# agwi-lab/renderformer

Measured on AMD Instinct MI355X. Metric: rendered frames/sec at 512×512, renderformer-v1.1-swin-large, 1/2/4/8 MI355X, higher is better.
Workload: dtype fp16+bf16

## Files before the change

include/rf.h:

```cpp
#ifndef RF_H
#define RF_H

#include <stdint.h>

#ifdef __cplusplus
extern "C" {
#endif

#define RF_OK 0
#define RF_ERR_INVALID 1
#define RF_ERR_LAUNCH 2
#define RF_ERR_UNSUPPORTED 3
#define RF_ERR_DEVICE 4

#define RF_ABI_VERSION 16

#define RF_EPI_BF16 0
#define RF_EPI_F32 1
#define RF_EPI_ADD_F32 2
#define RF_EPI_SWIGLU 3
#define RF_EPI_F16 4
#define RF_EPI_SWIGLU_F16 5

#define RF_DT_BF16 0
#define RF_DT_F16 1

const char* rf_last_error(void);
int rf_abi_version(void);
#define RF_BUILD_STUDY 1
int rf_build_flags(void);

int rf_device_error(void);
int rf_clear_device_error(void);
int rf_f16_range_flag(void);
int rf_clear_f16_range_flag(void);
int rf_range_word_new(void** handle);
int rf_range_word_bind(void* handle);
int rf_range_word_read(void* handle);
int rf_range_word_clear(void* handle);
int rf_range_word_free(void* handle);
int rf_debug_raise_device_error(int code, void* stream);

int rf_ktimer_arm(void);
int rf_ktimer_read(float* ms, int max_n);

int rf_gemm_bf16(const void* a, int64_t lda, const void* w, int64_t ldw, void* c, int64_t ldc,
                 const float* bias, int m, int n, int k, int epilogue, void* workspace, int64_t ws_bytes,
                 void* stream);
int64_t rf_gemm_workspace_bytes(void);
int rf_gemm_f16(const void* a, int64_t lda, const void* w, int64_t ldw, void* c, int64_t ldc,
                const float* bias, int m, int n, int k, int epilogue, void* workspace, int64_t ws_bytes,
                void* stream);
#define RF_PRENORM_SLOTS 8
int rf_prenorm(const float* x, int64_t ldx, const float* norm_w, void* xg, int64_t ldxg, float* ss, int rows,
               int dim, int operand_dtype, void* stream);
int rf_gemm_add_prenorm(const void* a, int64_t lda, const void* w, int64_t ldw, float* x, int64_t ldx, int m, int n,
                        int k, const float* norm_w, void* xg, int64_t ldxg, float* ss, int operand_dtype,
                        void* workspace, int64_t ws_bytes, void* stream);
int rf_gemm_rownorm(const void* a, int64_t lda, const void* w, int64_t ldw, void* c, int64_t ldc, int m, int n,
                    int k, int epilogue, const float* ss, int norm_dim, float eps, float* seg_ss, int seg_w,
                    int n_seg, int operand_dtype, void* workspace, int64_t ws_bytes, void* stream);
int rf_gemm_qk_rope(const void* a, int64_t lda, const void* w, int64_t ldw, void* c, int64_t ldc, int m, int n,
                    int k, const float* ss, int norm_dim, float eps, float* seg_ss, int seg_w, int n_seg,
                    const float* norm_w, const float* pos, int64_t ld_pos, int pos_div, const float* freqs,
                    int n_freqs, float q_scale, int operand_dtype, void* workspace, int64_t ws_bytes, void* stream);
int rf_row_rms_scale(void* x, int64_t ldx, int rows, int dim, const float* ss, int64_t ld_ss, float eps, float scale,
                     void* stream);
int rf_attn_fwd_qn(const void* q, int64_t ldq, const void* k, int64_t ldk, const void* v, int64_t ldv, void* o,
                   int64_t ldo, int o_dtype, const float* q_ss, int64_t ld_ss, int q_dim, float eps, float q_scale,
                   const int32_t* problems, int n_problems, int n_heads, int head_dim, void* workspace,
                   const int64_t* bounds, int grid, void* stream);
int rf_gemm_bf16_if(const int* flag, const void* a, int64_t lda, const void* w, int64_t ldw, void* c, int64_t ldc,
                    const float* bias, int m, int n, int k, int epilogue, void* workspace, int64_t ws_bytes,
                    void* stream);

int rf_gemm_mx8(const void* a, int64_t lda, const void* sa, int64_t ld_sa, const void* w, int64_t ldw, const void* sw,
                int64_t ld_sw, void* c, int64_t ldc, const float* bias, int m, int n, int k, int epilogue,
                void* stream);
int rf_quant_mx8(const void* x, int64_t ldx, int rows, int cols, void* q, int64_t ldq, void* scales, int64_t ld_s,
                 void* stream);

int rf_rmsnorm(const float* x, int64_t ldx, const float* weight, float eps, void* out, int64_t ldo,
               int rows, int dim, void* stream);
int rf_rmsnorm_f16(const float* x, int64_t ldx, const float* weight, float eps, void* out, int64_t ldo,
                   int rows, int dim, void* stream);

int rf_qk_norm_rope(const void* src, int64_t ld_src, void* dst, int64_t ld_dst, const int32_t* src_rows,
                    int rows, int dim, int n_heads, int n_seg, const float* norm_w, float eps, float seg0_scale,
                    const float* pos, int64_t ld_pos, int pos_div, const float* freqs, int n_freqs, void* stream);

int rf_qk_norm_rope_groups(const void* src, int64_t ld_src, int64_t src_gstride, void* dst, int64_t ld_dst,
                           int64_t dst_gstride, const int32_t* src_rows, int rows, int dim, int n_heads, int n_seg,
                           int n_groups, const float* norm_w, int64_t w_gstride, float eps, float seg0_scale,
                           const float* pos, int64_t ld_pos, int pos_div, const float* freqs, int n_freqs,
                           void* stream);
int rf_qk_norm_rope_groups_ilv(const void* src, int64_t ld_src, int64_t src_gstride, void* dst, int64_t ld_dst,
                               int64_t dst_gstride, const int32_t* src_rows, int rows, int dim, int n_heads, int n_seg,
                               int n_groups, const float* norm_w, int64_t w_gstride, float eps, float seg0_scale,
                               const float* pos, int64_t ld_pos, int pos_div, const float* freqs, int n_freqs,
                               void* stream);

int rf_attn_fwd(const void* q, int64_t ldq, const void* k, int64_t ldk, const void* v, int64_t ldv,
                void* o, int64_t ldo, const int32_t* problems, int n_problems, int max_q_len, int n_heads,
                int head_dim, float scale, int n_split, void* workspace, int64_t ws_rows, void* stream);
int64_t rf_attn_workspace_bytes(int64_t rows, int n_heads, int n_split);
int rf_attn_grid(void);
int rf_attn_schedule(const int32_t* problems_host, int n_problems, int n_heads, int grid, int64_t* bounds);
int rf_attn_fwd_sched(const void* q, int64_t ldq, const void* k, int64_t ldk, const void* v, int64_t ldv,
                      void* o, int64_t ldo, const int32_t* problems, int n_problems, int n_heads, int head_dim,
                      float scale, void* workspace, const int64_t* bounds, int grid, void* stream);
int rf_attn_combine(const void* workspace, int64_t ws_rows, int n_split, int n_heads, const int32_t* rows,
// ... 24 lines not shown
int rf_texture_scan(float* texture, int64_t n_rows, int channels, int patch_elems, int log_channels,
                    const int32_t* dst_row, float* coef, int64_t ldc, int* flag, void* stream);
int rf_texture_scan2(float* texture, int64_t n_rows, int channels, int patch_elems, int log_channels,
                     const int32_t* dst_row, float* coef, int64_t ldc, int* flag, int* flag_clear, void* stream);
int rf_texture_linear(const float* coef, int64_t ldc, int rows, int channels, const float* wsum,
                      const float* bias, float* out, int64_t ldo, int n, const int* flag, void* stream);

int rf_vn_encode(const float* vn, int64_t n_rows, const int32_t* dst_row, int n_freqs, void* out,
                 int64_t ldo, void* stream);
int rf_vn_encode_dt(const float* vn, int64_t n_rows, const int32_t* dst_row, int n_freqs, void* out,
                    int64_t ldo, int out_dtype, void* stream);

int rf_ray_tokens(const float* c2w, const float* fov_deg, int n_views, int res, int patch, void* out,
                  float* ray_pos, void* stream);
int rf_ray_tokens_dt(const float* c2w, const float* fov_deg, int n_views, int res, int patch, void* out,
                     float* ray_pos, int out_dtype, void* stream);

int rf_patchify_rays(const float* rays_d, int n_views, int res, int patch, void* out, void* stream);
int rf_patchify_rays_dt(const float* rays_d, int n_views, int res, int patch, void* out, int out_dtype,
                        void* stream);

int rf_scene_pos(const float* tris, const int32_t* valid_idx, const int32_t* scene_off, const float* c2w,
                 int n_scenes, int n_views, int n_reg, float* pos_out, const int32_t* set_off, int max_tris,
                 float* partials, int64_t partial_floats, void* stream);
int64_t rf_scene_pos_partials(int sets, int max_tris);

int rf_embed(float* out, int64_t ldo, const int32_t* out_rows, int rows, int dim, const float* base,
             int base_rows, const float* in0, int64_t ld0, const float* w0, float eps0, const float* in1,
             int64_t ld1, const float* w1, float eps1, void* stream);

int rf_hdr_output(const float* logits, float* out, int n, int c, int h, int w, float elu_alpha, int log_decode,
                  int channels_last, void* stream);

#define RF_CONV_PLANE_SILU 1
#define RF_CONV_SILU_OUT 2
#define RF_CONV_FINAL 4
#define RF_CONV_LOG_DECODE 8
#define RF_CONV_NCHW_OUT 16
#define RF_CONV_BORDER_BIAS 32
int rf_conv2d_bf16x3(const void* in_hi, const void* in_lo, int n_img, int hi, int wi, int cin_pad, const void* w_hi,
                     const void* w_lo, int cout, int cout_pad, int kh, int kw, int stride, int pad, const float* bias,
                     const float* res1, const float* res2, float* out, void* p_hi, void* p_lo, int p_ld, int flags,
                     const float* w_fin, const float* b_fin, int n_fin, float elu_alpha, void* workspace,
                     int64_t ws_bytes, void* stream);

int rf_deconv2d_bf16x3(const void* in_hi, const void* in_lo, int n_img, int hi, int wi, int cin_pad, const void* w_hi,
                       const void* w_lo, int cout, int k, const float* bias, float* out, void* p_hi, void* p_lo,
                       int p_ld, void* workspace, int64_t ws_bytes, void* stream);

int rf_conv2d_f16(const void* in, int n_img, int hi, int wi, int cin_pad, const void* w, int cout, int cout_pad, int kh,
                  int kw, int stride, int pad, const float* bias, const float* res1, const float* res2, float* out,
                  void* p_out, int p_ld, int flags, const float* w_fin, const float* b_fin, int n_fin, float elu_alpha,
                  void* workspace, int64_t ws_bytes, void* stream);
typedef struct {
    const void* in;
    const void* w;
    const float* bias;
    float* out;
    void* p_out;
    int n_img, hi, wi, cin_pad, cout, cout_pad, kh, kw, stride, pad, deconv_k, p_ld, flags;
} rf_conv_desc;
int rf_conv2d_f16_group(int n_conv, const rf_conv_desc* convs, void* stream);

int rf_conv1x1_f16_group(int n_conv, const void* const* in, const int* cin_pad, const void* const* w, const int* cout,
                         const int* cout_pad, const float* const* bias, void* const* p_out, const int* p_ld, int n_img,
                         int hi, int wi, void* stream);
int rf_deconv2d_f16(const void* in, int n_img, int hi, int wi, int cin_pad, const void* w, int cout, int k,
                    const float* bias, float* out, void* p_out, int p_ld, void* workspace, int64_t ws_bytes,
                    void* stream);

int rf_split_planes(const float* x, int64_t rows, int c, int64_t ldx, void* p_hi, void* p_lo, int p_ld, int silu_act,
                    void* stream);

int rf_upsample_bilinear(const float* in, int n_img, int hi, int wi, int c, float* out, int ho, int wo, void* p_hi,
                         void* p_lo, int p_ld, void* stream);

int rf_upsample_bilinear_h(const void* in, int in_ld, int n_img, int hi, int wi, int c, int ho, int wo, void* p_out,
                           int p_ld, void* stream);


typedef struct {
    const float* attn_norm;
    const void* w_qkv;
    const float* qk_norm;
    const void* w_out;
    const float* ffn_norm;
    const void* w13;
    const void* w2;
} rf_encoder_layer;

typedef struct {
    int n_layers, rows, dim, n_heads, ffn_dim;
    int operand_dtype;
    float eps;
    const rf_encoder_layer* layers;
    const float* pos;
    int64_t ld_pos;
    const float* freqs;
    int n_freqs;
    const int32_t* problems;
    int n_problems;
    const int64_t* bounds;
    int grid;
    void* workspace;
    void* gemm_ws;
    int64_t gemm_ws_bytes;
// ... 16 lines not shown
    const float* self_norm;
    const void* w_self_in;
    const float* self_qk_norm;
    const void* w_self_out;
    const float* ffn_norm;
    const void* w13;
    const void* w2;
} rf_decoder_layer;

typedef struct {
    int layer, p_ld;
    void* p_hi;
    void* p_lo;
} rf_decoder_tap;

typedef struct {
    int n_layers, rows, dim, n_heads, ffn_dim;
    int operand_dtype;
    float eps;
    const rf_decoder_layer* layers;
    const float* ctx;
    int64_t ld_ctx;
    int ctx_rows, ctx_dim;
    const float* ctx_norm;
    const void* w_kv_all;
    int kv_rows;
    const int32_t* kv_src_rows;
    const float* kv_pos;
    int64_t ld_kv_pos;
    int k_batch;
    const float* k_norm_all;
    const float* freqs;
    int n_freqs;
    const float* ray_pos;
    int64_t ld_ray_pos;
    int ray_pos_div;
    const int32_t* cross_problems;
    int n_cross;
    const int64_t* cross_bounds;
    int cross_grid;
    int swin, n_images, grid_h, grid_w, window, shift;
    const int32_t* self_problems;
    int n_self;
    const rf_decoder_tap* taps;
    int n_taps;
    void* workspace;
    void* gemm_ws;
    int64_t gemm_ws_bytes;
    void* attn_ws;
    int timer_cross;
    int qk_fused;
    const void* kv_all;
    int64_t ld_kv_all;
} rf_decoder_desc;

int rf_decoder_forward(float* x, int64_t ldx, const rf_decoder_desc* desc, void* stream);
int64_t rf_decoder_workspace_bytes(const rf_decoder_desc* desc);

int rf_scene_kv(const float* ctx, int64_t ld_ctx, int ctx_rows, int ctx_dim, const float* ctx_norm,
                const void* w_kv_all, int width, int operand_dtype, float eps, void* scratch, void* kv_all,
                int64_t ld_kv_all, void* gemm_ws, int64_t gemm_ws_bytes, void* stream);

#ifdef __cplusplus
}
#endif
#endif
```

renderformer_amd/_lib.py:

```python
from __future__ import annotations

import ctypes
import os
import threading

import torch

_HERE = os.path.dirname(os.path.abspath(__file__))
LIB_PATH = os.environ.get("RF_LIB", os.path.join(_HERE, "lib", "librfhip.so"))


def source_digest(*names: str) -> str:
    import hashlib
    h = hashlib.sha256()
    for n in names:
        with open(os.path.join(_HERE, "csrc", n), "rb") as f:
            h.update(f.read())
    return h.hexdigest()[:16]


ATTN_SOURCES = ("attention.hip", "common.h")

_P = ctypes.c_void_p
_I = ctypes.c_int
_L = ctypes.c_int64
_F = ctypes.c_float

SIGNATURES = {
    "rf_gemm_bf16": [_P, _L, _P, _L, _P, _L, _P, _I, _I, _I, _I, _P, _L, _P],
    "rf_gemm_f16": [_P, _L, _P, _L, _P, _L, _P, _I, _I, _I, _I, _P, _L, _P],
    "rf_rmsnorm_f16": [_P, _L, _P, _F, _P, _L, _I, _I, _P],
    "rf_attn_fwd_sk": [_P, _L, _P, _L, _P, _L, _P, _L, _I, _P, _I, _I, _I, _F, _P, _P, _I, _P],
    "rf_attn_fwd_dt": [_P, _L, _P, _L, _P, _L, _P, _L, _I, _I, _P, _I, _I, _I, _F, _P, _P, _I, _P],
    "rf_swin_attn_fwd_dt": [_P, _L, _P, _L, _P, _L, _P, _L, _I, _I, _I, _I, _I, _I, _I, _I, _F, _P],
    "rf_swin_attn_fwd_qkn": [_P, _L, _P, _L, _P, _L, _P, _L, _I, _I, _I, _I, _I, _I, _I, _I, _F, _P, _P, _F, _F, _P],
    "rf_rmsnorm": [_P, _L, _P, _F, _P, _L, _I, _I, _P],
    "rf_prenorm": [_P, _L, _P, _P, _L, _P, _I, _I, _I, _P],
    "rf_gemm_add_prenorm": [_P, _L, _P, _L, _P, _L, _I, _I, _I, _P, _P, _L, _P, _I, _P, _L, _P],
    "rf_gemm_rownorm": [_P, _L, _P, _L, _P, _L, _I, _I, _I, _I, _P, _I, _F, _P, _I, _I, _I, _P, _L, _P],
    "rf_gemm_qk_rope": [_P, _L, _P, _L, _P, _L, _I, _I, _I, _P, _I, _F, _P, _I, _I, _P, _P, _L, _I, _P, _I, _F, _I,
                        _P, _L, _P],
    "rf_row_rms_scale": [_P, _L, _I, _I, _P, _L, _F, _F, _P],
    "rf_attn_fwd_qn": [_P, _L, _P, _L, _P, _L, _P, _L, _I, _P, _L, _I, _F, _F, _P, _I, _I, _I, _P, _P, _I, _P],
    "rf_qk_norm_rope": [_P, _L, _P, _L, _P, _I, _I, _I, _I, _P, _F, _F, _P, _L, _I, _P, _I, _P],
    "rf_qk_norm_rope_groups": [_P, _L, _L, _P, _L, _L, _P, _I, _I, _I, _I, _I, _P, _L, _F, _F, _P, _L, _I, _P, _I,
                               _P],
    "rf_qk_norm_rope_groups_ilv": [_P, _L, _L, _P, _L, _L, _P, _I, _I, _I, _I, _I, _P, _L, _F, _F, _P, _L, _I, _P, _I,
                               _P],
    "rf_attn_fwd": [_P, _L, _P, _L, _P, _L, _P, _L, _P, _I, _I, _I, _I, _F, _I, _P, _L, _P],
    "rf_attn_fwd_sched": [_P, _L, _P, _L, _P, _L, _P, _L, _P, _I, _I, _I, _F, _P, _P, _I, _P],
    "rf_attn_schedule": [_P, _I, _I, _I, _P],
    "rf_attn_combine": [_P, _L, _I, _I, _P, _I, _P, _L, _P],
    "rf_swin_attn_fwd": [_P, _L, _P, _L, _P, _L, _P, _L, _I, _I, _I, _I, _I, _I, _I, _F, _P],
    "rf_texture_pack": [_P, _L, _I, _I, _I, _P, _P, _L, _P],
    "rf_texture_pack_if": [_P, _P, _L, _I, _I, _I, _P, _P, _L, _P],
    "rf_texture_scan": [_P, _L, _I, _I, _I, _P, _P, _L, _P, _P],
    "rf_texture_scan2": [_P, _L, _I, _I, _I, _P, _P, _L, _P, _P, _P],
    "rf_texture_linear": [_P, _L, _I, _I, _P, _P, _P, _L, _I, _P, _P],
    "rf_gemm_bf16_if": [_P, _P, _L, _P, _L, _P, _L, _P, _I, _I, _I, _I, _P, _L, _P],
    "rf_vn_encode": [_P, _L, _P, _I, _P, _L, _P],
    "rf_vn_encode_dt": [_P, _L, _P, _I, _P, _L, _I, _P],
    "rf_ray_tokens_dt": [_P, _P, _I, _I, _I, _P, _P, _I, _P],
    "rf_patchify_rays_dt": [_P, _I, _I, _I, _P, _I, _P],
    "rf_ray_tokens": [_P, _P, _I, _I, _I, _P, _P, _P],
    "rf_patchify_rays": [_P, _I, _I, _I, _P, _P],
    "rf_scene_pos": [_P, _P, _P, _P, _I, _I, _I, _P, _P, _I, _P, _L, _P],
    "rf_embed": [_P, _L, _P, _I, _I, _P, _I, _P, _L, _P, _F, _P, _L, _P, _F, _P],
    "rf_hdr_output": [_P, _P, _I, _I, _I, _I, _F, _I, _I, _P],
    "rf_conv2d_bf16x3": [_P, _P, _I, _I, _I, _I, _P, _P, _I, _I, _I, _I, _I, _I, _P, _P, _P, _P, _P, _P, _I, _I,
                         _P, _P, _I, _F, _P, _L, _P],
    "rf_deconv2d_bf16x3": [_P, _P, _I, _I, _I, _I, _P, _P, _I, _I, _P, _P, _P, _P, _I, _P, _L, _P],
    "rf_conv2d_f16": [_P, _I, _I, _I, _I, _P, _I, _I, _I, _I, _I, _I, _P, _P, _P, _P, _P, _I, _I, _P, _P, _I, _F,
                      _P, _L, _P],
    "rf_deconv2d_f16": [_P, _I, _I, _I, _I, _P, _I, _I, _P, _P, _P, _I, _P, _L, _P],
    "rf_split_planes": [_P, _L, _I, _L, _P, _P, _I, _I, _P],
    "rf_upsample_bilinear": [_P, _I, _I, _I, _I, _P, _I, _I, _P, _P, _I, _P],
    "rf_upsample_bilinear_h": [_P, _I, _I, _I, _I, _I, _I, _I, _P, _I, _P],
    "rf_conv1x1_f16_group": [_I, _P, _P, _P, _P, _P, _P, _P, _P, _I, _I, _I, _P],
    "rf_conv2d_f16_group": [_I, _P, _P],
    "rf_gemm_mx8": [_P, _L, _P, _L, _P, _L, _P, _L, _P, _L, _P, _I, _I, _I, _I, _P],
    "rf_quant_mx8": [_P, _L, _I, _I, _P, _L, _P, _L, _P],
    "rf_device_error": [],
    "rf_clear_device_error": [],
    "rf_f16_range_flag": [],
    "rf_clear_f16_range_flag": [],
    "rf_range_word_new": [_P],
    "rf_range_word_bind": [_P],
    "rf_range_word_read": [_P],
    "rf_range_word_clear": [_P],
    "rf_range_word_free": [_P],
    "rf_debug_raise_device_error": [_I, _P],
    "rf_ktimer_arm": [],
    "rf_ktimer_read": [_P, _I],
    "rf_encoder_forward": [_P, _L, _P, _P],
    "rf_decoder_forward": [_P, _L, _P, _P],
    "rf_scene_kv": [_P, _L, _I, _I, _P, _P, _I, _I, _F, _P, _P, _L, _P, _L, _P],
}
RF_ERR_DEVICE = 4

_lock = threading.Lock()
_lib = None


class EncoderLayer(ctypes.Structure):
    _fields_ = [(n, ctypes.c_void_p) for n in ("attn_norm", "w_qkv", "qk_norm", "w_out", "ffn_norm", "w13", "w2")]


class EncoderDesc(ctypes.Structure):
    _fields_ = [("n_layers", _I), ("rows", _I), ("dim", _I), ("n_heads", _I), ("ffn_dim", _I),
                ("operand_dtype", _I), ("eps", _F), ("layers", _P), ("pos", _P), ("ld_pos", _L), ("freqs", _P),
                ("n_freqs", _I), ("problems", _P), ("n_problems", _I), ("bounds", _P), ("grid", _I),
                ("workspace", _P), ("gemm_ws", _P), ("gemm_ws_bytes", _L), ("attn_ws", _P), ("timer_attn", _I),
                ("qk_fused", _I)]


class DecoderLayer(ctypes.Structure):
    _fields_ = [(n, ctypes.c_void_p) for n in ("query_norm", "w_q", "q_norm", "kv_norm", "w_kv", "k_norm", "w_out",
                                               "self_norm", "w_self_in", "self_qk_norm", "w_self_out", "ffn_norm",
                                               "w13", "w2")]


class DecoderTap(ctypes.Structure):
    _fields_ = [("layer", _I), ("p_ld", _I), ("p_hi", _P), ("p_lo", _P)]


class DecoderDesc(ctypes.Structure):
    _fields_ = [("n_layers", _I), ("rows", _I), ("dim", _I), ("n_heads", _I), ("ffn_dim", _I),
                ("operand_dtype", _I), ("eps", _F), ("layers", _P), ("ctx", _P), ("ld_ctx", _L), ("ctx_rows", _I),
                ("ctx_dim", _I), ("ctx_norm", _P), ("w_kv_all", _P), ("kv_rows", _I), ("kv_src_rows", _P),
                ("kv_pos", _P), ("ld_kv_pos", _L), ("k_batch", _I), ("k_norm_all", _P), ("freqs", _P),
                ("n_freqs", _I), ("ray_pos", _P), ("ld_ray_pos", _L), ("ray_pos_div", _I), ("cross_problems", _P),
                ("n_cross", _I), ("cross_bounds", _P), ("cross_grid", _I), ("swin", _I), ("n_images", _I),
                ("grid_h", _I), ("grid_w", _I), ("window", _I), ("shift", _I), ("self_problems", _P), ("n_self", _I),
                ("taps", _P), ("n_taps", _I), ("workspace", _P), ("gemm_ws", _P), ("gemm_ws_bytes", _L),
                ("attn_ws", _P), ("timer_cross", _I), ("qk_fused", _I), ("kv_all", _P), ("ld_kv_all", _L)]


class HipLibraryError(RuntimeError):
    pass


class DeviceError(RuntimeError):
    """A kernel reported a device-side failure (a stream-K hand-off that timed out, or a range table that does not
    fit its launch): the outputs of that launch are invalid.  ``renderformer_amd.ops.clear_device_error()``
    recovers (it drains the device, clears the error word and drops the stream-K workspaces).  Also raised by a
    deferred fp16 range check (``RenderFormer(range_check="deferred")``) that finds a frame whose fp16 operands
    overflowed."""


def load(require_device: bool = True):
    global _lib
    with _lock:
        if _lib is None:
            if not os.path.exists(LIB_PATH):
                raise HipLibraryError(
                    f"librfhip.so not found at {LIB_PATH}; build it with `python -c 'import __graft_entry__ as g; g.build()'`")
            lib = ctypes.CDLL(LIB_PATH)
            for name, args in SIGNATURES.items():
                fn = getattr(lib, name, None)
                if fn is None:
                    continue
                fn.argtypes = args
                fn.restype = ctypes.c_int
            for name, res, args in (("rf_last_error", ctypes.c_char_p, []), ("rf_abi_version", ctypes.c_int, None),
                                    ("rf_build_flags", ctypes.c_int, []),
                                    ("rf_attn_workspace_bytes", ctypes.c_int64, [_L, _I, _I]),
                                    ("rf_gemm_workspace_bytes", ctypes.c_int64, []),
                                    ("rf_scene_pos_partials", ctypes.c_int64, [_I, _I]), ("rf_attn_grid", None, []),
                                    ("rf_encoder_workspace_bytes", ctypes.c_int64, [_I, _I, _I, _I]),
                                    ("rf_decoder_workspace_bytes", ctypes.c_int64, [_P])):
                fn = getattr(lib, name, None)
                if fn is None:
                    continue
                if res is not None:
                    fn.restype = res
                if args is not None:
                    fn.argtypes = args
            _lib = lib
    if require_device and not torch.cuda.is_available():
        raise HipLibraryError("renderformer_amd needs a HIP device (MI355X); none is visible")
    return _lib


def study_build() -> bool:
    lib = load(require_device=False)
    if getattr(lib, "rf_build_flags", None) is None:
        return False
    return bool(lib.rf_build_flags() & 1)
# ... 21 lines not shown
```

renderformer_amd/csrc/common.h:

```cpp
#pragma once
#include <hip/hip_runtime.h>
#include <hip/hip_ext.h>
#include <stdint.h>

#include "../../include/rf.h"

#define RF_DEV __device__ __forceinline__

typedef uint16_t bf16_t;
typedef __attribute__((ext_vector_type(8))) __bf16 bf16x8;
typedef __attribute__((ext_vector_type(4))) __bf16 bf16x4;
typedef __attribute__((ext_vector_type(2))) _Float16 f16x2;
typedef __attribute__((ext_vector_type(8))) _Float16 f16x8;
typedef __attribute__((ext_vector_type(4))) short s16x4;
typedef __attribute__((ext_vector_type(4))) float f32x4;
typedef __attribute__((ext_vector_type(2))) float f32x2;
typedef __attribute__((ext_vector_type(16))) float f32x16;
typedef __attribute__((ext_vector_type(4))) unsigned u32x4;
typedef __attribute__((ext_vector_type(2))) unsigned u32x2;

#define LDS_PTR(T, p) ((__attribute__((address_space(3))) T*)(p))
#define GLB_PTR(T, p) ((const __attribute__((address_space(1))) T*)(p))

RF_DEV float bf16_to_f32(bf16_t v) { return __uint_as_float(((uint32_t)v) << 16); }

RF_DEV bf16_t f32_to_bf16(float f) {
    __bf16 b = (__bf16)f;
    return *reinterpret_cast<bf16_t*>(&b);
}

RF_DEV uint32_t pack_bf16x2(float lo, float hi) {
    return (uint32_t)f32_to_bf16(lo) | ((uint32_t)f32_to_bf16(hi) << 16);
}

RF_DEV uint16_t f32_to_16(float v, bool f16) {
    if (f16) {
        _Float16 h = (_Float16)v;
        return __builtin_bit_cast(uint16_t, h);
    }
    return f32_to_bf16(v);
}

RF_DEV uint32_t pack_f16x2(float lo, float hi) {
    _Float16 a = (_Float16)lo, b = (_Float16)hi;
    return (uint32_t)*reinterpret_cast<uint16_t*>(&a) | ((uint32_t)*reinterpret_cast<uint16_t*>(&b) << 16);
}

RF_DEV float f16_bits_to_f32(uint16_t b) { return (float)__builtin_bit_cast(_Float16, b); }

RF_DEV float wave_sum(float v) {
#pragma unroll
    for (int o = 32; o > 0; o >>= 1) v += __shfl_xor(v, o, 64);
    return v;
}

RF_DEV float wave_max(float v) {
#pragma unroll
    for (int o = 32; o > 0; o >>= 1) v = fmaxf(v, __shfl_xor(v, o, 64));
    return v;
}

RF_DEV void wait_vmcnt0() { asm volatile("s_waitcnt vmcnt(0)" ::: "memory"); }

RF_DEV float silu(float x) {
    return x * __builtin_amdgcn_rcpf(1.0f + __builtin_amdgcn_exp2f(x * -1.4426950408889634f));
}
RF_DEV float elu_fast(float y, float alpha) {
    return y > 0.f ? y : alpha * (__builtin_amdgcn_exp2f(y * 1.4426950408889634f) - 1.0f);
}
RF_DEV float pow10m1_fast(float y) { return __builtin_amdgcn_exp2f(y * 3.3219280948873623f) - 1.0f; }

RF_DEV void report_device_error(int* err, int code) {
    if (err) __hip_atomic_store(err, code, __ATOMIC_RELAXED, __HIP_MEMORY_SCOPE_SYSTEM);
}
RF_DEV void report_f16_range(int* w, int code) {
    if (w) __hip_atomic_store(w, code, __ATOMIC_RELAXED, __HIP_MEMORY_SCOPE_SYSTEM);
}
RF_DEV bool f16_in_range(float amax) { return amax <= 65504.0f; }
RF_DEV float amax3(float m, float a, float b) {
    return __builtin_fmaxf(__builtin_fmaxf(m, __builtin_fabsf(a)), __builtin_fabsf(b));
}
#define RF_RANGE_GEMM 1
#define RF_RANGE_RMSNORM 2
#define RF_RANGE_ATTN 4
#define RF_RANGE_CONV 8
#define RF_DEVERR_SK_GEMM 1
#define RF_DEVERR_SK_ATTN 2
#define RF_DEVERR_SK_SCHED 3
#define RF_DEVERR_SCENE_POS 4

#define RF_HD __host__ __device__ __forceinline__
struct SkLayout {
    int nwg, nx, G;
    RF_HD SkLayout(int nwg_, int64_t units) : nwg(nwg_), nx(nwg_ < 8 ? nwg_ : 8), G(1) {
        G = units < (int64_t)nx ? (int)(units > 0 ? units : 1) : nx;
    }
    RF_HD int cnt(int x) const { return (nwg - x + nx - 1) / nx; }
    RF_HD int xlo(int g) const { return (g * nx + G - 1) / G; }
    RF_HD int group_of(int x) const { return x * G / nx; }
    RF_HD int base(int g) const {
        int s = 0;
// ... 59 lines not shown
```

renderformer_amd/csrc/conv.hip:

```cpp
#include <math.h>

#include "common.h"

namespace {


RF_DEV float store_split4(bf16_t* p_hi, bf16_t* p_lo, int64_t off, float4 v, bool act) {
    float x[4] = {v.x, v.y, v.z, v.w};
    if (!p_lo) {
        if (act) {
#pragma unroll
            for (int e = 0; e < 4; ++e) x[e] = silu(x[e]);
        }
        *reinterpret_cast<uint2*>(p_hi + off) = make_uint2(pack_f16x2(x[0], x[1]), pack_f16x2(x[2], x[3]));
        return amax3(amax3(0.f, x[0], x[1]), x[2], x[3]);
    }
    uint32_t h[2], l[2];
#pragma unroll
    for (int e = 0; e < 2; ++e) {
        float a0 = x[2 * e], a1 = x[2 * e + 1];
        if (act) {
            a0 = silu(a0);
            a1 = silu(a1);
        }
// ... 9 lines not shown
__global__ __launch_bounds__(256) void split_kernel(const float* __restrict__ x, int rows, int c, int64_t ldx,
                                                    bf16_t* __restrict__ p_hi, bf16_t* __restrict__ p_lo, int p_ld,
                                                    int act, int* range) {
    const int c4 = c / 4;
    const int i = blockIdx.x * blockDim.x + threadIdx.x;
    if (i >= rows * c4) return;
    const int r32 = i / c4;
    const int64_t r = r32;
    const int cc = (i - r32 * c4) * 4;
    const float am = store_split4(p_hi, p_lo, r * p_ld + cc, *reinterpret_cast<const float4*>(x + r * ldx + cc), act);
    if (range && !f16_in_range(am)) report_f16_range(range, RF_RANGE_CONV);
}

__global__ __launch_bounds__(256) void upsample_kernel(const float* __restrict__ in, float* __restrict__ out,
                                                       bf16_t* __restrict__ p_hi, bf16_t* __restrict__ p_lo, int p_ld,
                                                       int hi, int wi, int c, int ho, int wo, float sh, float sw) {
    const int c4n = c >> 2;
    const int i = blockIdx.x * blockDim.x + threadIdx.x;
    if (i >= wo * c4n) return;
    const int row = blockIdx.y;
    const int img = row / ho, oy = row - img * ho;
    const int ox = i / c4n;
    const int cc = (i - ox * c4n) * 4;
    const float fy = sh * (float)oy, fx = sw * (float)ox;
    const int y0 = (int)fy, x0 = (int)fx;
    const int y1 = y0 + (y0 < hi - 1 ? 1 : 0), x1 = x0 + (x0 < wi - 1 ? 1 : 0);
    const float ly1 = fy - (float)y0, lx1 = fx - (float)x0;
    const float ly0 = 1.0f - ly1, lx0 = 1.0f - lx1;
    const float* base = in + (int64_t)img * hi * wi * c + cc;
    const float4 a = *reinterpret_cast<const float4*>(base + (int64_t)(y0 * wi + x0) * c);
    const float4 b = *reinterpret_cast<const float4*>(base + (int64_t)(y0 * wi + x1) * c);
    const float4 d = *reinterpret_cast<const float4*>(base + (int64_t)(y1 * wi + x0) * c);
    const float4 e = *reinterpret_cast<const float4*>(base + (int64_t)(y1 * wi + x1) * c);
    float4 r;
    r.x = ly0 * (lx0 * a.x + lx1 * b.x) + ly1 * (lx0 * d.x + lx1 * e.x);
    r.y = ly0 * (lx0 * a.y + lx1 * b.y) + ly1 * (lx0 * d.y + lx1 * e.y);
    r.z = ly0 * (lx0 * a.z + lx1 * b.z) + ly1 * (lx0 * d.z + lx1 * e.z);
    r.w = ly0 * (lx0 * a.w + lx1 * b.w) + ly1 * (lx0 * d.w + lx1 * e.w);
    const int64_t pix = (int64_t)row * wo + ox;
    if (out) *reinterpret_cast<float4*>(out + pix * c + cc) = r;
    if (p_hi) store_split4(p_hi, p_lo, pix * p_ld + cc, r, false);
}

__global__ __launch_bounds__(256) void upsample8_kernel(const float* __restrict__ in, float* __restrict__ out,
                                                        bf16_t* __restrict__ p_hi, bf16_t* __restrict__ p_lo, int p_ld,
                                                        int hi, int wi, int c, int ho, int wo, float sh, float sw) {
    const int c8n = c >> 3;
    const int i = blockIdx.x * blockDim.x + threadIdx.x;
    if (i >= wo * c8n) return;
    const int row = blockIdx.y;
    const int img = row / ho, oy = row - img * ho;
    const int ox = i / c8n;
    const int cc = (i - ox * c8n) * 8;
    const float fy = sh * (float)oy, fx = sw * (float)ox;
    const int y0 = (int)fy, x0 = (int)fx;
    const int y1 = y0 + (y0 < hi - 1 ? 1 : 0), x1 = x0 + (x0 < wi - 1 ? 1 : 0);
    const float ly1 = fy - (float)y0, lx1 = fx - (float)x0;
    const float ly0 = 1.0f - ly1, lx0 = 1.0f - lx1;
    const float* base = in + (int64_t)img * hi * wi * c + cc;
    const float4* pa = reinterpret_cast<const float4*>(base + (int64_t)(y0 * wi + x0) * c);
    const float4* pb = reinterpret_cast<const float4*>(base + (int64_t)(y0 * wi + x1) * c);
    const float4* pd = reinterpret_cast<const float4*>(base + (int64_t)(y1 * wi + x0) * c);
    const float4* pe = reinterpret_cast<const float4*>(base + (int64_t)(y1 * wi + x1) * c);
    float4 a[2], b[2], d[2], e[2], r[2];
#pragma unroll
    for (int h = 0; h < 2; ++h) {
        a[h] = pa[h];
        b[h] = pb[h];
        d[h] = pd[h];
        e[h] = pe[h];
    }
#pragma unroll
    for (int h = 0; h < 2; ++h) {
        r[h].x = ly0 * (lx0 * a[h].x + lx1 * b[h].x) + ly1 * (lx0 * d[h].x + lx1 * e[h].x);
        r[h].y = ly0 * (lx0 * a[h].y + lx1 * b[h].y) + ly1 * (lx0 * d[h].y + lx1 * e[h].y);
        r[h].z = ly0 * (lx0 * a[h].z + lx1 * b[h].z) + ly1 * (lx0 * d[h].z + lx1 * e[h].z);
        r[h].w = ly0 * (lx0 * a[h].w + lx1 * b[h].w) + ly1 * (lx0 * d[h].w + lx1 * e[h].w);
    }
    const int64_t pix = (int64_t)row * wo + ox;
    if (out) {
        float4* o = reinterpret_cast<float4*>(out + pix * c + cc);
        o[0] = r[0];
        o[1] = r[1];
    }
    if (p_hi && !p_lo) {
        *reinterpret_cast<uint4*>(p_hi + pix * p_ld + cc) =
            make_uint4(pack_f16x2(r[0].x, r[0].y), pack_f16x2(r[0].z, r[0].w), pack_f16x2(r[1].x, r[1].y),
                       pack_f16x2(r[1].z, r[1].w));
    } else if (p_hi) {
        store_split4(p_hi, p_lo, pix * p_ld + cc, r[0], false);
        store_split4(p_hi, p_lo, pix * p_ld + cc + 4, r[1], false);
    }
}

__global__ __launch_bounds__(256) void upsample8h_kernel(const uint16_t* __restrict__ in, int in_ld,
                                                         uint16_t* __restrict__ p_out, int p_ld, int hi, int wi, int c,
                                                         int ho, int wo, float sh, float sw) {
    const int c8n = c >> 3;
    const int i = blockIdx.x * blockDim.x + threadIdx.x;
    if (i >= wo * c8n) return;
    const int row = blockIdx.y;
    const int img = row / ho, oy = row - img * ho;
    const int ox = i / c8n;
    const int cc = (i - ox * c8n) * 8;
    const float fy = sh * (float)oy, fx = sw * (float)ox;
    const int y0 = (int)fy, x0 = (int)fx;
    const int y1 = y0 + (y0 < hi - 1 ? 1 : 0), x1 = x0 + (x0 < wi - 1 ? 1 : 0);
    const float ly1 = fy - (float)y0, lx1 = fx - (float)x0;
    const float ly0 = 1.0f - ly1, lx0 = 1.0f - lx1;
    const uint16_t* base = in + (int64_t)img * hi * wi * in_ld + cc;
    const uint4 qa = *reinterpret_cast<const uint4*>(base + (int64_t)(y0 * wi + x0) * in_ld);
    const uint4 qb = *reinterpret_cast<const uint4*>(base + (int64_t)(y0 * wi + x1) * in_ld);
    const uint4 qd = *reinterpret_cast<const uint4*>(base + (int64_t)(y1 * wi + x0) * in_ld);
    const uint4 qe = *reinterpret_cast<const uint4*>(base + (int64_t)(y1 * wi + x1) * in_ld);
    const uint32_t wa[4] = {qa.x, qa.y, qa.z, qa.w}, wb[4] = {qb.x, qb.y, qb.z, qb.w};
    const uint32_t wd[4] = {qd.x, qd.y, qd.z, qd.w}, we[4] = {qe.x, qe.y, qe.z, qe.w};
    uint32_t o[4];
#pragma unroll
    for (int k = 0; k < 4; ++k) {
        float r[2];
#pragma unroll
        for (int h = 0; h < 2; ++h) {
            const float a = f16_bits_to_f32((uint16_t)(wa[k] >> (16 * h))), b = f16_bits_to_f32((uint16_t)(wb[k] >> (16 * h)));
            const float d = f16_bits_to_f32((uint16_t)(wd[k] >> (16 * h))), e = f16_bits_to_f32((uint16_t)(we[k] >> (16 * h)));
            r[h] = ly0 * (lx0 * a + lx1 * b) + ly1 * (lx0 * d + lx1 * e);
        }
        o[k] = pack_f16x2(r[0], r[1]);
    }
    *reinterpret_cast<uint4*>(p_out + ((int64_t)row * wo + ox) * p_ld + cc) = make_uint4(o[0], o[1], o[2], o[3]);
}

// ... 54 lines not shown
```

renderformer_amd/csrc/gemm.hip:

```cpp
#include <algorithm>
#include <type_traits>
#include <cmath>
#include <math.h>
#include <stdio.h>
#include <stdlib.h>
#include <string.h>

#include "common.h"
#include "env.h"

namespace {

constexpr int BK = 32;
constexpr int P_F16 = 2;

enum Epi { E_BF16 = RF_EPI_BF16, E_F32 = RF_EPI_F32, E_ADD = RF_EPI_ADD_F32, E_SWIGLU = RF_EPI_SWIGLU, E_CONV = 16,
           E_ROPE = 17 };

template <int BM_, int BN_, int WGM_, int WGN_, int STAGES_, int KH_ = 1>
struct Tile {
    static constexpr int BM = BM_, BN = BN_, WGM = WGM_, WGN = WGN_, STAGES = STAGES_, KH = KH_;
    static constexpr int NWAVE = WGM * WGN, THREADS = NWAVE * 64;
    static constexpr int MW = BM / WGM, NWD = BN / WGN, TI = MW / 16, TJ = NWD / 16;
    static constexpr int APIECES = BM / 16;
    static constexpr bool ASHARE = APIECES < NWAVE;
    static constexpr int PA = ASHARE ? 1 : BM / 16 / NWAVE, PB = BN / 16 / NWAVE;
    static constexpr int A_BYTES = BM * BK * 2, B_BYTES = BN * BK * 2;
    static_assert(PA >= 1 && PB >= 1 && (ASHARE || PA * NWAVE * 16 == BM || BM == 288) && PB * NWAVE * 16 == BN,
                  "tile/wave mismatch");
    static_assert(TI >= 1 && TJ >= 2 && TJ % 2 == 0, "wave tile too small");
};

struct EngineArgs {
    const bf16_t* a;
    const bf16_t* a_lo;
    int64_t lda;
    const bf16_t* w;
    const bf16_t* w_lo;
    int64_t ldw;
    int m, n, k;
    int hi, wi, cin_pad, ho, wo, kw, stride, pad;
    uint64_t cin_m, kw_m;
    const bf16_t* zero;
    void* c;
    int64_t ldc;
    const float* bias;
    const float* res1;
    const float* res2;
    bf16_t* p_hi;
    bf16_t* p_lo;
    int p_ld;
    int cout, deconv, flags, n_fin;
    int plane_f16;
    const float* w_fin;
    const float* b_fin;
    float elu_alpha;
    float* sk_part;
    int* sk_flag;
    int sk_epoch;
    int group_m;
    const int* gate;
    int halo_lg;
    int* err;
    int spin;
    uint64_t* stamps;
    const uint8_t* sa;
    const uint8_t* sw;
    int ld_sa, ld_sw;
    int persist;
    int l2pf;
    int out_f16;
    int* range;
    bf16_t* xg;
    int64_t ldxg;
    const float* norm_g;
    float* ss_out;
    int xg_f16;
    const float* rs_part;
    float rs_n, rs_eps;
    float* seg_ss;
    int seg_w, seg_n;
    const float* rope_pos;
    int64_t rope_ld;
    int rope_div;
    const float* rope_freqs;
    int rope_nf;
    const float* rope_g;
    float rope_qscale;
};

constexpr int PN_SLOTS = RF_PRENORM_SLOTS;


RF_DEV uint32_t pack16(const EngineArgs& p, float lo, float hi) {
    return p.out_f16 ? pack_f16x2(lo, hi) : pack_bf16x2(lo, hi);
}

RF_DEV float unpack16(const EngineArgs& p, uint32_t h) {
    return p.out_f16 ? f16_bits_to_f32((uint16_t)h) : __uint_as_float(h << 16);
}

// ... 283 lines not shown
template <class C>
constexpr int ROPE_POS_BYTES = (C::BM * 9 + 63) / 64 * 256;
template <class C, int EPI>
constexpr bool RED_IN_ROWS = C::BM == 288 && (EPI == E_BF16 || EPI == E_ROPE) && C::WGN < PN_SLOTS;
template <class C, int EPI>
constexpr int PN_RED = RED_IN_ROWS<C, EPI> ? 0 : C::BM * C::WGN * 4;
template <class C, int EPI>
constexpr int PN_AREA = EPI == E_ADD      ? C::BN * 4 + C::BM * C::WGN * 4
                        : EPI == E_BF16   ? C::BM * PN_SLOTS * 4 + PN_RED<C, EPI>
                        : EPI == E_ROPE   ? C::BM * PN_SLOTS * 4 + PN_RED<C, EPI> + C::BN * 4 + ROPE_POS_BYTES<C> + 64 * 4
                        : EPI == E_SWIGLU ? C::BM * PN_SLOTS * 4
                                          : 0;

template <class C, int EPI>
RF_DEV void pn_issue(const EngineArgs& p, char* area, int m0, int n0) {
    const int lane = threadIdx.x & 63;
    const int wave = __builtin_amdgcn_readfirstlane(threadIdx.x >> 6);
    if constexpr (EPI == E_ADD) {
        if (p.xg && wave == 0 && n0 + 4 * lane < p.n && 4 * lane < C::BN)
            __builtin_amdgcn_global_load_lds(GLB_PTR(void, p.norm_g + n0 + 4 * lane), LDS_PTR(void, area), 16, 0, 0);
    } else if constexpr (EPI == E_BF16 || EPI == E_SWIGLU || EPI == E_ROPE) {
        if (p.rs_part) {
            static_assert(C::BM % 32 == 0, "1-KiB pieces of 32 rows");
            for (int c = wave; c < C::BM / 32; c += C::NWAVE) {
                const int row = min(m0 + 32 * c + (lane >> 1), p.m - 1);
                __builtin_amdgcn_global_load_lds(GLB_PTR(void, p.rs_part + (int64_t)row * PN_SLOTS + 4 * (lane & 1)),
                                                 LDS_PTR(void, area + c * 1024), 16, 0, 0);
            }
        }
        if constexpr (EPI == E_ROPE) {
            if (n0 / p.seg_w < p.seg_n) {
                char* const gl = area + C::BM * PN_SLOTS * 4 + PN_RED<C, EPI>;
                char* const pl = gl + C::BN * 4;
                char* const fl = pl + ROPE_POS_BYTES<C>;
                if (wave == 0 && p.rope_g && 4 * lane < C::BN)
                    __builtin_amdgcn_global_load_lds(GLB_PTR(void, p.rope_g + n0 + 4 * lane), LDS_PTR(void, gl), 16, 0, 0);
                if (p.rope_pos) {
                    if (wave == C::NWAVE - 1)
                        __builtin_amdgcn_global_load_lds(GLB_PTR(void, p.rope_freqs + min(lane, p.rope_nf - 1)),
                                                         LDS_PTR(void, fl), 4, 0, 0);
                    for (int c = wave; c * 64 < C::BM * 9; c += C::NWAVE) {
                        const int e = c * 64 + lane;
                        const int r = e / 9, col = e - r * 9;
                        const int row = min(m0 + min(r, C::BM - 1), p.m - 1) / p.rope_div;
                        __builtin_amdgcn_global_load_lds(GLB_PTR(void, p.rope_pos + (int64_t)row * p.rope_ld + col),
                                                         LDS_PTR(void, pl + c * 256), 4, 0, 0);
                    }
                }
            }
        }
    }
}

template <class C, int EPI, int TW2D = 0, bool FINAL = true>
RF_DEV void engine_epilogue(const EngineArgs& p, int m0, int n0, const f32x4 (&acc)[C::TI][C::TJ],
                            char* area = nullptr) {
    constexpr int TI = C::TI, TJ = C::TJ;
    const int lane = threadIdx.x & 63;
    const int wave = threadIdx.x >> 6;
    const int wm = wave / C::WGN, wn = wave % C::WGN;
    static_assert(TW2D == 0 || (EPI == E_CONV && TW2D % 16 == 0 && C::MW % TW2D == 0), "2-D conv tile");
    const int rl = lane & 15, cq = 4 * (lane >> 4);
    const int rbase = m0 + wm * C::MW, cbase = n0 + wn * C::NWD;
    auto frow = [&](int i) -> int {
        if constexpr (TW2D == 0) return rbase + i * 16 + rl;
        else return m0 + (wm * (C::MW / TW2D) + (i * 16) / TW2D) * p.wo + (i * 16) % TW2D + rl;
    };
    float amax = 0.f;
    const bool rsc = (EPI == E_SWIGLU || EPI == E_BF16 || EPI == E_ROPE) && p.rs_part && area;
    if constexpr (EPI == E_SWIGLU || EPI == E_BF16 || EPI == E_ROPE) {
        if (rsc) {
            lds_sync();
            for (int t = threadIdx.x; t < C::BM; t += C::THREADS) {
                char* q = area + t * (PN_SLOTS * 4);
                const f32x4 a = lds_ld_f4(q), b = lds_ld_f4(q + 16);
                const float sum = ((a[0] + a[1]) + (a[2] + a[3])) + ((b[0] + b[1]) + (b[2] + b[3]));
                lds_st_f32(q, 1.0f / sqrtf(sum / p.rs_n + p.rs_eps));
            }
            lds_sync();
        }
    }
    auto row_scale = [&](int i) -> float {
        return rsc ? lds_ld_f32(area + (wm * C::MW + i * 16 + rl) * (PN_SLOTS * 4)) : 1.f;
    };
    if constexpr (EPI == E_SWIGLU) {
        bf16_t* c = reinterpret_cast<bf16_t*>(p.c);
#pragma unroll
        for (int i = 0; i < TI; ++i) {
            const float rsi = row_scale(i);
#pragma unroll
            for (int pair = 0; pair < TJ / 2; ++pair) {
                const int gcol = cbase + pair * 32;
                const int ocol = (gcol >> 5) * 16 + cq;
                const int row = rbase + i * 16 + rl;
                if (row < p.m) {
                    float o[4];
#pragma unroll
                    for (int e = 0; e < 4; ++e) {
                        float g = acc[i][2 * pair][e] * rsi, u = acc[i][2 * pair + 1][e] * rsi;
                        if (p.bias) {
                            g += p.bias[gcol + cq + e];
                            u += p.bias[gcol + 16 + cq + e];
                        }
                        o[e] = silu(g) * u;
                    }
                    amax = amax3(amax3(amax, o[0], o[1]), o[2], o[3]);
                    *reinterpret_cast<uint2*>(c + (int64_t)row * p.ldc + ocol) =
                        make_uint2(pack16(p, o[0], o[1]), pack16(p, o[2], o[3]));
                }
            }
        }
        if (p.range && !f16_in_range(amax)) report_f16_range(p.range, RF_RANGE_GEMM);
        return;
    } else if constexpr (EPI == E_CONV) {
        if (FINAL && (p.flags & RF_CONV_FINAL)) {
            float bsum[TJ][4];
#pragma unroll
            for (int j = 0; j < TJ; ++j)
#pragma unroll
                for (int e = 0; e < 4; ++e) {
                    const int col = cbase + j * 16 + cq + e;
                    bsum[j][e] = (p.bias && col < p.cout) ? p.bias[col] : 0.f;
                }
            for (int f = 0; f < p.n_fin; ++f) {
                const float bfin = p.b_fin[f];
                float wf[TJ][4];
#pragma unroll
                for (int j = 0; j < TJ; ++j)
#pragma unroll
                    for (int e = 0; e < 4; ++e) {
                        const int col = cbase + j * 16 + cq + e;
                        wf[j][e] = col < p.cout ? p.w_fin[f * p.cout + col] : 0.f;
                    }
#pragma unroll
                for (int i = 0; i < TI; ++i) {
                    float s = 0.f;
#pragma unroll
                    for (int j = 0; j < TJ; ++j)
#pragma unroll
                        for (int e = 0; e < 4; ++e) s += silu(acc[i][j][e] + bsum[j][e]) * wf[j][e];
                    s += __shfl_xor(s, 16, 64);
                    s += __shfl_xor(s, 32, 64);
                    const int m = frow(i);
                    if (lane < 16 && wn == 0 && m < p.m) {
                        float y = elu_fast(s + bfin, p.elu_alpha);
                        if (p.flags & RF_CONV_LOG_DECODE) y = pow10m1_fast(y);
                        const int hwp = p.ho * p.wo;
                        const int64_t o = (p.flags & RF_CONV_NCHW_OUT) ? ((int64_t)(m / hwp) * p.n_fin + f) * hwp + (m % hwp)
                                                                      : (int64_t)m * p.n_fin + f;
                        reinterpret_cast<float*>(p.c)[o] = y;
                    }
                }
            }
            return;
        }
        const int kk = p.deconv;
        const int nreal = kk ? p.cout * kk * kk : p.cout;
        const bool border = (p.flags & RF_CONV_BORDER_BIAS) && !kk;
        float* __restrict__ outp = reinterpret_cast<float*>(p.c);
        const float* __restrict__ res1 = p.res1;
        const float* __restrict__ res2 = p.res2;
        const float* __restrict__ bias = p.bias;
        struct PixOp {
            float4 r1[TJ], r2[TJ], b[TJ];
            int64_t pix[TJ];
            int co[TJ];
        };
        float4 bconst[TJ];
#pragma unroll
        for (int j = 0; j < TJ; ++j) {
            const int col = cbase + j * 16 + cq;
            bconst[j] = float4{0.f, 0.f, 0.f, 0.f};
            if (bias && !border && !kk && col < nreal) bconst[j] = *reinterpret_cast<const float4*>(bias + col);
        }
        auto fetch = [&](int i, PixOp& o) {
            const int m = frow(i);
            int img = 0, y = 0, x = 0;
            if (kk || border) {
                x = m % p.wo;
                const int t = m / p.wo;
                y = t % p.ho;
                img = t / p.ho;
            }
            const float* brow = bias;
            if (border && brow)
                brow += (3 * (y == 0 ? 0 : y == p.ho - 1 ? 2 : 1) + (x == 0 ? 0 : x == p.wo - 1 ? 2 : 1)) * p.cout;
#pragma unroll
            for (int j = 0; j < TJ; ++j) {
                const int col = cbase + j * 16 + cq;
                int64_t pix = m;
                int co = col;
                if (kk) {
                    const int tap = col / p.cout, dy = tap / kk, dx = tap % kk;
                    co = col - tap * p.cout;
                    pix = ((int64_t)img * p.ho * kk + y * kk + dy) * (p.wo * kk) + x * kk + dx;
                }
                o.pix[j] = pix;
                o.co[j] = co;
                o.r1[j] = float4{0.f, 0.f, 0.f, 0.f};
                o.r2[j] = float4{0.f, 0.f, 0.f, 0.f};
                o.b[j] = bconst[j];
                if (m < p.m && col < nreal) {
                    if (res1) o.r1[j] = *reinterpret_cast<const float4*>(res1 + pix * p.cout + co);
                    if (res2) o.r2[j] = *reinterpret_cast<const float4*>(res2 + pix * p.cout + co);
                    if (brow && (border || kk)) o.b[j] = *reinterpret_cast<const float4*>(brow + co);
                }
            }
        };
        constexpr bool PF = TJ <= 2;
        PixOp ops[PF ? 2 : 1];
        if constexpr (PF) fetch(0, ops[0]);
#pragma unroll
        for (int i = 0; i < TI; ++i) {
            if constexpr (PF) {
                if (i + 1 < TI) fetch(i + 1, ops[(i + 1) & 1]);
            } else {
                fetch(i, ops[0]);
            }
            const PixOp& o = ops[PF ? (i & 1) : 0];
            if (frow(i) >= p.m) continue;
#pragma unroll
            for (int j = 0; j < TJ; ++j) {
                const int col = cbase + j * 16 + cq;
                if (col >= nreal) continue;
                const int64_t pix = o.pix[j];
                const int co = o.co[j];
                const float bb[4] = {o.b[j].x, o.b[j].y, o.b[j].z, o.b[j].w};
                const float rr1[4] = {o.r1[j].x, o.r1[j].y, o.r1[j].z, o.r1[j].w};
                const float rr2[4] = {o.r2[j].x, o.r2[j].y, o.r2[j].z, o.r2[j].w};
                float v[4] = {acc[i][j][0], acc[i][j][1], acc[i][j][2], acc[i][j][3]};
#pragma unroll
                for (int e = 0; e < 4; ++e) {
                    v[e] = ((v[e] + bb[e]) + rr1[e]) + rr2[e];
                    if (p.flags & RF_CONV_SILU_OUT) v[e] = silu(v[e]);
                }
                if (outp)
                    *reinterpret_cast<float4*>(outp + pix * p.cout + co) = make_float4(v[0], v[1], v[2], v[3]);
                if (p.p_hi && p.plane_f16) {
                    float a[4] = {v[0], v[1], v[2], v[3]};
                    if (p.flags & RF_CONV_PLANE_SILU) {
#pragma unroll
                        for (int e = 0; e < 4; ++e) a[e] = silu(a[e]);
                    }
                    amax = amax3(amax3(amax, a[0], a[1]), a[2], a[3]);
                    *reinterpret_cast<uint2*>(p.p_hi + pix * p.p_ld + co) = make_uint2(pack_f16x2(a[0], a[1]),
                                                                                       pack_f16x2(a[2], a[3]));
                } else if (p.p_hi) {
                    uint32_t h[2], l[2];
#pragma unroll
                    for (int e = 0; e < 2; ++e) {
                        float a0 = v[2 * e], a1 = v[2 * e + 1];
                        if (p.flags & RF_CONV_PLANE_SILU) {
                            a0 = silu(a0);
                            a1 = silu(a1);
                        }
                        const bf16_t h0 = f32_to_bf16(a0), h1 = f32_to_bf16(a1);
                        h[e] = (uint32_t)h0 | ((uint32_t)h1 << 16);
                        l[e] = pack_bf16x2(a0 - bf16_to_f32(h0), a1 - bf16_to_f32(h1));
                    }
                    *reinterpret_cast<uint2*>(p.p_hi + pix * p.p_ld + co) = make_uint2(h[0], h[1]);
                    *reinterpret_cast<uint2*>(p.p_lo + pix * p.p_ld + co) = make_uint2(l[0], l[1]);
                }
            }
        }
        if (p.range && !f16_in_range(amax)) report_f16_range(p.range, RF_RANGE_CONV);
        return;
    } else {
        const bool pre = EPI == E_ADD && p.xg && area;
        const bool qkseg = EPI == E_ROPE && n0 / p.seg_w < p.seg_n;
        const bool segq = (EPI == E_BF16 || (EPI == E_ROPE && qkseg)) && p.seg_ss && area && n0 / p.seg_w < p.seg_n;
        char* const red = area + (EPI == E_ADD ? C::BN * 4 : C::BM * PN_SLOTS * 4);
        auto red_at = [&](int w, int t) -> char* {
            if constexpr (RED_IN_ROWS<C, EPI>) return area + t * (PN_SLOTS * 4) + (1 + w) * 4;
            else return red + (w * C::BM + t) * 4;
        };
        if (pre) lds_sync();
        float ssr[TI];
#pragma unroll
        for (int i = 0; i < TI; ++i) ssr[i] = 0.f;
        const char* const gl = area + C::BM * PN_SLOTS * 4 + PN_RED<C, EPI>;
        const float* const pl = reinterpret_cast<const float*>(gl + C::BN * 4);
        float frq[EPI == E_ROPE ? TJ : 1][2];
        int pcol[EPI == E_ROPE ? TJ : 1][2];
        float sscale = 1.f;
        if constexpr (EPI == E_ROPE) {
            if (qkseg) {
                if (!rsc) lds_sync();
                sscale = n0 / p.seg_w == 0 ? p.rope_qscale : 1.f;
                const int lim = 9 * p.rope_nf;
                const float* fl = pl + ROPE_POS_BYTES<C> / 4;
#pragma unroll
                for (int j = 0; j < TJ; ++j) {
                    const int col = cbase + j * 16 + cq;
#pragma unroll
                    for (int t = 0; t < 2; ++t) {
                        const int m = ((col & 127) >> 1) + t;
                        const bool on = p.rope_pos && m < lim;
                        const int pc = on ? m / p.rope_nf : 0;
                        frq[j][t] = on ? fl[m - pc * p.rope_nf] : 0.f;
                        pcol[j][t] = pc;
                    }
                }
            }
        }
#pragma unroll
        for (int i = 0; i < TI; ++i) {
            const int row = rbase + i * 16 + rl;
            if (row >= p.m) continue;
            const float rsi = row_scale(i);
#pragma unroll
            for (int j = 0; j < TJ; ++j) {
                const int col = cbase + j * 16 + cq;
                if (col >= p.n) continue;
                float v[4] = {acc[i][j][0] * rsi, acc[i][j][1] * rsi, acc[i][j][2] * rsi, acc[i][j][3] * rsi};
                if (p.bias) {
                    const float4 b = *reinterpret_cast<const float4*>(p.bias + col);
                    v[0] += b.x;
                    v[1] += b.y;
                    v[2] += b.z;
                    v[3] += b.w;
                }
                const int64_t o = (int64_t)row * p.ldc + col;
                if constexpr (EPI == E_ROPE) {
                    if (qkseg) {
                        if (segq) ssr[i] += v[0] * v[0] + v[1] * v[1] + v[2] * v[2] + v[3] * v[3];
                        const f32x4 g = p.rope_g ? *reinterpret_cast<const f32x4*>(gl + (col - n0) * 4)
                                                 : f32x4{1.f, 1.f, 1.f, 1.f};
                        const float z0 = v[0] * g[0], z1 = v[1] * g[1], z2 = v[2] * g[2], z3 = v[3] * g[3];
                        const float* prow = pl + (wm * C::MW + i * 16 + rl) * 9;
                        float s0, c0, s1, c1;
                        __sincosf(prow[pcol[j][0]] * frq[j][0], &s0, &c0);
                        __sincosf(prow[pcol[j][1]] * frq[j][1], &s1, &c1);
                        v[0] = (z0 * c0 - z1 * s0) * sscale;
                        v[1] = (z1 * c0 + z0 * s0) * sscale;
                        v[2] = (z2 * c1 - z3 * s1) * sscale;
                        v[3] = (z3 * c1 + z2 * s1) * sscale;
                    }
                    *reinterpret_cast<uint2*>(reinterpret_cast<bf16_t*>(p.c) + o) =
                        make_uint2(pack_bf16x2(v[0], v[1]), pack_bf16x2(v[2], v[3]));
                } else if constexpr (EPI == E_BF16) {
                    amax = amax3(amax3(amax, v[0], v[1]), v[2], v[3]);
                    const uint32_t lo = pack16(p, v[0], v[1]), hi = pack16(p, v[2], v[3]);
                    *reinterpret_cast<uint2*>(reinterpret_cast<bf16_t*>(p.c) + o) = make_uint2(lo, hi);
                    if (segq) {
                        const float r0 = unpack16(p, lo & 0xffffu), r1 = unpack16(p, lo >> 16);
                        const float r2 = unpack16(p, hi & 0xffffu), r3 = unpack16(p, hi >> 16);
                        ssr[i] += r0 * r0 + r1 * r1 + r2 * r2 + r3 * r3;
                    }
                } else {
                    *reinterpret_cast<float4*>(reinterpret_cast<float*>(p.c) + o) = make_float4(v[0], v[1], v[2], v[3]);
                    if (pre) {
                        const f32x4 g = lds_ld_f4(area + (col - n0) * 4);
                        const float y0 = v[0] * g[0], y1 = v[1] * g[1], y2 = v[2] * g[2], y3 = v[3] * g[3];
                        amax = amax3(amax3(amax, y0, y1), y2, y3);
                        const uint32_t lo = p.xg_f16 ? pack_f16x2(y0, y1) : pack_bf16x2(y0, y1);
                        const uint32_t hi = p.xg_f16 ? pack_f16x2(y2, y3) : pack_bf16x2(y2, y3);
                        *reinterpret_cast<uint2*>(p.xg + (int64_t)row * p.ldxg + col) = make_uint2(lo, hi);
                        ssr[i] += v[0] * v[0] + v[1] * v[1] + v[2] * v[2] + v[3] * v[3];
                    }
                }
            }
        }
        if constexpr (EPI == E_BF16)
            if (p.range && !f16_in_range(amax)) report_f16_range(p.range, RF_RANGE_GEMM);
        if constexpr (EPI == E_ADD || EPI == E_BF16 || EPI == E_ROPE) {
            if (pre && p.xg_f16 && p.range && !f16_in_range(amax)) report_f16_range(p.range, RF_RANGE_RMSNORM);
            if (pre || segq) {
#pragma unroll
                for (int i = 0; i < TI; ++i) {
                    ssr[i] += __shfl_xor(ssr[i], 16, 64);
                    ssr[i] += __shfl_xor(ssr[i], 32, 64);
                }
                if (lane < 16) {
#pragma unroll
                    for (int i = 0; i < TI; ++i) lds_st_f32(red_at(wn, wm * C::MW + i * 16 + rl), ssr[i]);
                }
                lds_sync();
                int slot, nslots, ld;
                float* base;
                if (pre) {
                    slot = n0 / C::BN;
                    nslots = (p.n + C::BN - 1) / C::BN;
                    ld = PN_SLOTS;
                    base = p.ss_out;
                } else {
                    slot = (n0 % p.seg_w) / C::BN;
                    nslots = p.seg_w / C::BN;
                    ld = p.seg_n * PN_SLOTS;
                    base = p.seg_ss + (n0 / p.seg_w) * PN_SLOTS;
                }
                for (int t = threadIdx.x; t < C::BM; t += C::THREADS) {
                    const int row = m0 + t;
                    if (row < p.m) {
                        float s = 0.f;
#pragma unroll
                        for (int w = 0; w < C::WGN; ++w) s += lds_ld_f32(red_at(w, t));
                        float* dst = base + (int64_t)row * ld;
                        dst[slot] = s;
                        if (slot == 0)
                            for (int z = nslots; z < PN_SLOTS; ++z) dst[z] = 0.f;
                    }
                }
            }
        }
    }
}



namespace ph {
constexpr int BN = 256, BK2 = 64;
constexpr int REGION = 16384;
template <int BM>
struct Cfg {
    static constexpr int NREG = BM >= 256 ? 4 : 3;
    static constexpr int NA = BM >= 256 ? 2 : 1;
    static constexpr int NX = BM == 288 ? 1 : 0;
// ... 923 lines not shown
        __syncthreads();
        if constexpr (STG == 1) quad_mainloop_reg<WM, WN, NTERM, EPI == E_ADD>(p, smem, m0, n0, 2 * kf, 2 * kl, acc);
        else quad_mainloop<WM, WN, NTERM, EPI == E_ADD>(p, smem, m0, n0, 2 * kf, 2 * kl, acc);
        if (kf != 0) {
            const __amdgpu_buffer_rsrc_t rs =
                __builtin_amdgcn_make_buffer_rsrc(p.sk_part + (int64_t)L * TS, 0, TS * 4, qd::RSRC_CFG);
#pragma unroll
            for (int i = 0; i < TI; ++i)
#pragma unroll
                for (int j = 0; j < TJ; ++j) {
                    const int off = (((wave * TI + i) * TJ + j) * 64 + lane) * 16;
                    __builtin_amdgcn_raw_buffer_store_b128(__builtin_bit_cast(u32x4, acc[i][j]), rs, off, 0, 16);
                }
            asm volatile("s_waitcnt vmcnt(0)" ::: "memory");
            __syncthreads();
            if (threadIdx.x == 0) __hip_atomic_store(p.sk_flag + L, p.sk_epoch, __ATOMIC_RELAXED, __HIP_MEMORY_SCOPE_AGENT);
        } else {
            if (kl < iters2) {
                const int64_t tile_end = (int64_t)(tile + 1) * iters2;
                for (int c = L + 1; c < gend; ++c) {
                    int64_t cb, ce;
                    lay.equal_range(c, grp, ntiles64, iters2, cb, ce);
                    if (cb >= tile_end) break;
                    if (ce == cb) continue;
                    if (threadIdx.x == 0) {
                        int spins = 0;
                        while (__hip_atomic_load(p.sk_flag + c, __ATOMIC_RELAXED, __HIP_MEMORY_SCOPE_AGENT) != p.sk_epoch &&
                               ++spins < p.spin)
                            __builtin_amdgcn_s_sleep(1);
                        if (spins >= p.spin) report_device_error(p.err, RF_DEVERR_SK_GEMM);
                        __builtin_amdgcn_fence(__ATOMIC_ACQUIRE, "agent");
                        asm volatile("s_waitcnt vmcnt(0)" ::: "memory");
                    }
                    __syncthreads();
                    const float4* src = reinterpret_cast<const float4*>(p.sk_part + (int64_t)c * TS) + wave * TI * TJ * 64 + lane;
#pragma unroll
                    for (int i = 0; i < TI; ++i)
#pragma unroll
                        for (int j = 0; j < TJ; ++j) {
                            const float4 v = src[(i * TJ + j) * 64];
                            acc[i][j][0] += v.x;
                            acc[i][j][1] += v.y;
                            acc[i][j][2] += v.z;
                            acc[i][j][3] += v.w;
                        }
                }
            }
            engine_epilogue<G, EPI>(p, m0, n0, acc);
        }
        it += kl - kf;
    }
}

template <class C, int EPI, int NTERM, bool GATHER, bool SK>
__global__ __launch_bounds__(C::THREADS, 2) void engine_kernel(EngineArgs p) {
    constexpr int BM = C::BM, BN = C::BN, TI = C::TI, TJ = C::TJ;
    constexpr int MAIN = C::STAGES * stage_bytes<C, NTERM>();
    __shared__ __attribute__((aligned(16))) char smem[MAIN + PN_AREA<C, EPI>];
    char* const area = smem + MAIN;
    if (gated_off(p)) return;

    const int tiles_m = (p.m + BM - 1) / BM;
    const int nwg = gridDim.x;
    const int hw = blockIdx.x;
    const int xcd = hw & 7, q = nwg >> 3, r = nwg & 7;
    const int wg = (xcd < r ? xcd * (q + 1) : r * (q + 1) + (xcd - r) * q) + (hw >> 3);
    f32x4 acc[TI][TJ];
    if constexpr (!SK) {
        int tm, tn;
        tile_coords(wg, tiles_m, p.n / BN, p.group_m, tm, tn);
        const int m0 = tm * BM, n0 = tn * BN;
        pn_issue<C, EPI>(p, area, m0, n0);
        engine_mainloop<C, NTERM, GATHER, EPI == E_ADD>(p, smem, m0, n0, 0, p.k / (BK * C::KH), acc);
        engine_epilogue<C, EPI>(p, m0, n0, acc, area);
    } else {
        const int iters = p.k / (BK * C::KH);
        const int64_t ntiles64 = (int64_t)tiles_m * (p.n / BN);
        const SkLayout lay(nwg, ntiles64);
        int grp = 0;
        const int L = lay.logical(hw, &grp);
        const int gend = lay.base(grp) + lay.size(grp);
        int64_t it, it_end;
        lay.equal_range(L, grp, ntiles64, iters, it, it_end);
        const int lane = threadIdx.x & 63, wave = threadIdx.x >> 6;
        while (it < it_end) {
            const int tile = (int)(it / iters), kf = (int)(it % iters);
            const int kl = (int)min((int64_t)iters, kf + (it_end - it));
            int tm, tn;
            tile_coords(tile, tiles_m, p.n / BN, p.group_m, tm, tn);
            const int m0 = tm * BM, n0 = tn * BN;
            wait_vm<0>();
            __syncthreads();
            if (kf == 0) pn_issue<C, EPI>(p, area, m0, n0);
            engine_mainloop<C, NTERM, GATHER, EPI == E_ADD>(p, smem, m0, n0, kf, kl, acc);
            if (kf != 0) {
                const __amdgpu_buffer_rsrc_t rs = __builtin_amdgcn_make_buffer_rsrc(
                    p.sk_part + (int64_t)L * (BM * BN), 0, BM * BN * 4, 0x00020000);
#pragma unroll
                for (int i = 0; i < TI; ++i)
#pragma unroll
                    for (int j = 0; j < TJ; ++j) {
                        const int off = (((wave * TI + i) * TJ + j) * 64 + lane) * 16;
                        __builtin_amdgcn_raw_buffer_store_b128(__builtin_bit_cast(u32x4, acc[i][j]), rs, off, 0, 16);
                    }
                asm volatile("s_waitcnt vmcnt(0)" ::: "memory");
                __syncthreads();
                if (threadIdx.x == 0) __hip_atomic_store(p.sk_flag + L, p.sk_epoch, __ATOMIC_RELAXED, __HIP_MEMORY_SCOPE_AGENT);
            } else {
                if (kl < iters) {
                    const int64_t tile_end = (int64_t)(tile + 1) * iters;
                    for (int c = L + 1; c < gend; ++c) {
                        int64_t cb, ce;
                        lay.equal_range(c, grp, ntiles64, iters, cb, ce);
                        if (cb >= tile_end) break;
                        if (ce == cb) continue;
                        if (threadIdx.x == 0) {
                            int spins = 0;
                            while (__hip_atomic_load(p.sk_flag + c, __ATOMIC_RELAXED, __HIP_MEMORY_SCOPE_AGENT) != p.sk_epoch &&
                                   ++spins < p.spin)
                                __builtin_amdgcn_s_sleep(1);
                            if (spins >= p.spin) report_device_error(p.err, RF_DEVERR_SK_GEMM);
                            __builtin_amdgcn_fence(__ATOMIC_ACQUIRE, "agent");
                            asm volatile("s_waitcnt vmcnt(0)" ::: "memory");
                        }
                        __syncthreads();
                        const float4* src =
                            reinterpret_cast<const float4*>(p.sk_part + (int64_t)c * (BM * BN)) + wave * TI * TJ * 64 + lane;
#pragma unroll
                        for (int i = 0; i < TI; ++i)
#pragma unroll
                            for (int j = 0; j < TJ; ++j) {
                                const float4 v = src[(i * TJ + j) * 64];
                                acc[i][j][0] += v.x;
                                acc[i][j][1] += v.y;
                                acc[i][j][2] += v.z;
                                acc[i][j][3] += v.w;
                            }
                    }
                }
                engine_epilogue<C, EPI>(p, m0, n0, acc, area);
            }
            it += kl - kf;
        }
    }
}

constexpr int GROUP_MAX = 4;
struct GroupArgs {
    EngineArgs p[GROUP_MAX];
    int first[GROUP_MAX + 1];
    int n;
};

template <class C, int EPI, int NTERM, bool GATHER>
__global__ __launch_bounds__(C::THREADS, 2) void engine_group_kernel(GroupArgs g) {
    constexpr int BM = C::BM, BN = C::BN, TI = C::TI, TJ = C::TJ;
    __shared__ __attribute__((aligned(16))) char smem[C::STAGES * stage_bytes<C, NTERM>()];
    const int nwg = gridDim.x, hw = blockIdx.x;
    const int xcd = hw & 7, qd = nwg >> 3, rd = nwg & 7;
    const int wg = (xcd < rd ? xcd * (qd + 1) : rd * (qd + 1) + (xcd - rd) * qd) + (hw >> 3);
    int q = 0;
#pragma unroll
    for (int i = 1; i < GROUP_MAX; ++i) q += (i < g.n && wg >= g.first[i]) ? 1 : 0;
    const EngineArgs& p = g.p[q];
    const int local = wg - g.first[q];
    const int tiles_m = (p.m + BM - 1) / BM;
    int tm, tn;
    tile_coords(local, tiles_m, p.n / BN, p.group_m, tm, tn);
    f32x4 acc[TI][TJ];
    engine_mainloop<C, NTERM, GATHER, EPI == E_ADD>(p, smem, tm * BM, tn * BN, 0, p.k / (BK * C::KH), acc);
    engine_epilogue<C, EPI>(p, tm * BM, tn * BN, acc);
}

template <class C>
struct Halo {
    static constexpr int ROWS = (3 * (C::BM + 2) + 15) / 16 * 16;
    static constexpr int BYTES = ROWS * 64;
    static constexpr int PIECES = ROWS / 16;
    static constexpr int PPW = (PIECES + C::NWAVE - 1) / C::NWAVE;
    static constexpr int BST = 3;
    static constexpr int LDS = 2 * BYTES + BST * C::B_BYTES;
};

template <class C>
RF_DEV void halo_mainloop(const EngineArgs& p, char* smem, int m0, int n0, f32x4 (&acc)[C::TI][C::TJ]) {
    using H = Halo<C>;
    constexpr int TI = C::TI, TJ = C::TJ, PB = C::PB, S = H::BST;
    const int lane = threadIdx.x & 63;
    const int wave = threadIdx.x >> 6;
    const int wm = wave / C::WGN, wn = wave % C::WGN;
    const int lg = p.halo_lg, tw = 1 << lg, hw2 = tw + 2;
    const int hr_n = ((C::BM >> lg) + 2) * hw2;
    const int per_img = p.ho * p.wo;
// ... 279 lines not shown
            const int kt = 9 * c + t;
            if constexpr (DBG == 8) __builtin_amdgcn_s_setprio(1);
            read_b(kt % S);
            read_a(t);
            if (DBG != 2 && t < PPW && !last) issue_halo(c + 1, t);
            if (DBG != 2 && kt + S - 1 < nk) issue_w(kt + S - 1);
            if (has_w) {
                if (t < 8 || !last) {
                    if (last) wait_vm_rt<4>(wait_count(t, S - 1, true));
                    else wait_vm_rt<8>(wait_count(t, S - 1, false));
                }
            } else if (t == 8 && !last) {
                wait_vm<0>();
            }
            if constexpr (DBG == 8) __builtin_amdgcn_s_setprio(0);
            sync_in();
            mma();
            sync_out();
        }
        const uint32_t step = (c & 1) ? (uint32_t)-HBYTES : (uint32_t)HBYTES;
#pragma unroll
        for (int h = 0; h < 2; ++h)
#pragma unroll
            for (int tx = 0; tx < 3; ++tx) hadr[h][tx] += step;
    }
    if (!late) __builtin_amdgcn_s_barrier();
}

template <int S, int BN, int DBG = 0>
__global__ __launch_bounds__(512, 1) void halo2_kernel(EngineArgs p) {
    __shared__ __attribute__((aligned(16))) char smem[H2Cfg<S, BN>::LDS];
    const int nwg = gridDim.x, hw = blockIdx.x;
    const int xcd = hw & 7, q = nwg >> 3, r = nwg & 7;
    const int wg = (xcd < r ? xcd * (q + 1) : r * (q + 1) + (xcd - r) * q) + (hw >> 3);
    const int tiles_n = p.n / BN, tx_n = p.wo / h2::TW, ty_n = p.ho / h2::TH;
    const int tn = wg % tiles_n, pt = wg / tiles_n;
    const int tx = pt % tx_n, rest = pt / tx_n;
    const int ty = rest % ty_n, img = rest / ty_n;
    const int y0 = ty * h2::TH, x0 = tx * h2::TW;
    f32x4 acc[H2Cfg<S, BN>::TI][4];
    halo2_mainloop<S, BN, DBG>(p, smem, img, y0, x0, tn * BN, acc);
    engine_epilogue<H2Tile<BN>, E_CONV, h2::TW, BN == 64>(p, (img * p.ho + y0) * p.wo + x0, tn * BN, acc);
}

namespace h3 {
constexpr int WGN = 4, WGM = 2, RW = h2::TH / WGM, TI = 2 * RW, TJ = 2;
constexpr int LDS = 2 * h2::HBYTES;
}
struct H3Tile {
    static constexpr int WGN = h3::WGN, WGM = h3::WGM, MW = 512 / h3::WGM, NWD = 128 / h3::WGN, TI = h3::TI,
                         TJ = h3::TJ;
};

template <int DBG = 0>
__global__ __launch_bounds__(512, 1) void halo3_kernel(EngineArgs p) {
    using namespace h2;
    __shared__ __attribute__((aligned(16))) char smem[h3::LDS];
    constexpr int TI = h3::TI;
    const int nwg = gridDim.x, hw = blockIdx.x;
    const int xcd = hw & 7, q = nwg >> 3, r = nwg & 7;
    const int wg = (xcd < r ? xcd * (q + 1) : r * (q + 1) + (xcd - r) * q) + (hw >> 3);
    const int tiles_n = p.n / 128, tx_n = p.wo / TW, ty_n = p.ho / TH;
    const int tn = wg % tiles_n, pt = wg / tiles_n;
    const int tx = pt % tx_n, rest = pt / tx_n;
    const int ty = rest % ty_n, img = rest / ty_n;
    const int y0 = ty * TH, x0 = tx * TW, n0 = tn * 128;

    const int lane = threadIdx.x & 63;
    const int wave = threadIdx.x >> 6;
    const int wm = wave / h3::WGN, wn = wave % h3::WGN;
    const int nch = p.cin_pad / 32, nk = 9 * nch;
    char* hbuf = smem;

    int hpix[PPW], hch[PPW];
#pragma unroll
    for (int t = 0; t < PPW; ++t) {
        const int hp = (wave + 8 * t) * 16 + (lane >> 2);
        hch[t] = (lane & 3) ^ h2::hkey(hp % HWID);
        int pix = -1;
        if (hp < HPIX) {
            const int hy = hp / HWID, hx = hp - hy * HWID;
            const int iy = y0 + hy - 1, ix = x0 + hx - 1;
            if (iy >= 0 && iy < p.hi && ix >= 0 && ix < p.wi) pix = (img * p.hi + iy) * p.wi + ix;
        }
        hpix[t] = pix;
    }
    const uint32_t hbase = __builtin_amdgcn_readfirstlane((uint32_t)(uintptr_t)LDS_PTR(char, hbuf) + wave * 1024);
    auto issue_halo = [&](int chunk, int buf, int t) {
        const bf16_t* src = hpix[t] >= 0 ? p.a + (int64_t)hpix[t] * p.cin_pad + hch[t] * 8 + chunk * 32 : p.zero;
        const uint32_t lds = hbase + buf * HBYTES + t * 8 * 1024;
        asm volatile("s_mov_b32 m0, %1\n\ts_nop 0\n\tglobal_load_lds_dwordx4 %0, off" ::"v"(src), "s"(lds)
                     : "memory", "m0");
    };

    const int frow = lane & 15, fch = lane >> 4;
    const __amdgpu_buffer_rsrc_t rw = __builtin_amdgcn_make_buffer_rsrc(
        (void*)(p.w + (int64_t)n0 * p.ldw), 0, (int)((int64_t)128 * p.ldw * 2), qd::RSRC_CFG);
    const int wv0 = ((wn * 32 + frow) * (int)p.ldw + fch * 8) * 2, wv1 = wv0 + 16 * (int)p.ldw * 2;
    u32x4 fb[3][2];
    auto load_b = [&](int kt, int slot) {
        const int chunk = kt / 9, tap = kt - 9 * chunk;
        const int so = (tap * p.cin_pad + chunk * 32) * 2;
        fb[slot][0] = __builtin_amdgcn_raw_buffer_load_b128(rw, wv0, so, 0);
        fb[slot][1] = __builtin_amdgcn_raw_buffer_load_b128(rw, wv1, so, 0);
    };

    f32x4 acc[TI][2];
// ... 19 lines not shown
    wait_vm<0>();
    __builtin_amdgcn_s_barrier();
    __builtin_amdgcn_sched_barrier(0);

    for (int c = 0; c < ((DBG & 32) ? 0 : nch); ++c) {
        const bool last = c + 1 == nch;
#pragma unroll
        for (int t = 0; t < 9; ++t) {
            const int kt = 9 * c + t;
            bf16x8 fa[TI];
#pragma unroll
            for (int i = 0; i < TI; ++i) {
                if constexpr (DBG & 16) {
                    fa[i] = __builtin_bit_cast(bf16x8, u32x4{(uint32_t)(lane + i), (uint32_t)t, 0u, (uint32_t)c});
                } else {
                    fa[i] = *LDS_PTR(const bf16x8, (uintptr_t)(hadr[i & 1][t % 3] + ((i >> 1) + t / 3) * HWID * 64));
                }
            }
            if (!(DBG & 4) && t < PPW) issue_halo(last ? c : c + 1, (c + 1) & 1, t);
            if (!(DBG & 2)) load_b(min(kt + 2, nk - 1), (t + 2) % 3);
            __builtin_amdgcn_s_setprio(1);
#pragma unroll
            for (int i = 0; i < TI; ++i)
#pragma unroll
                for (int j = 0; j < 2; ++j) {
                    if constexpr (DBG & 1) {
                        if (j == 0) asm volatile("" ::"v"(fa[i]));
                    } else {
                        acc[i][j] = __builtin_amdgcn_mfma_f32_16x16x32_f16(__builtin_bit_cast(f16x8, fb[t % 3][j]),
                                                                           __builtin_bit_cast(f16x8, fa[i]), acc[i][j], 0, 0, 0);
                    }
                }
            __builtin_amdgcn_s_setprio(0);
        }
        if (!(DBG & 8) && !last) {
            wait_vm<0>();
            __builtin_amdgcn_s_waitcnt(0xC07F);
            __builtin_amdgcn_sched_barrier(0);
            __builtin_amdgcn_s_barrier();
            __builtin_amdgcn_sched_barrier(0);
            const uint32_t step = (c & 1) ? (uint32_t)-HBYTES : (uint32_t)HBYTES;
#pragma unroll
            for (int h = 0; h < 2; ++h)
#pragma unroll
                for (int tx3 = 0; tx3 < 3; ++tx3) hadr[h][tx3] += step;
        }
    }
    wait_vm<0>();
    if constexpr ((DBG & 64) != 0) {
#pragma unroll
        for (int i = 0; i < TI; ++i) asm volatile("" ::"v"(acc[i][0]), "v"(acc[i][1]));
        return;
    }
    engine_epilogue<H3Tile, E_CONV, TW, false>(p, (img * p.ho + y0) * p.wo + x0, n0, acc);
}

namespace c32 {
constexpr int TH = 16, TW = 32, HWID = TW + 2, HPIX = (TH + 2) * HWID;
constexpr int HPIECES = 40, WPIECES = 18;
constexpr int HBYTES = HPIECES * 1024, WBYTES = WPIECES * 1024, BUF = HBYTES + WBYTES;
constexpr int NWAVE = 4, HPW = HPIECES / NWAVE;
constexpr int LDS = 2 * BUF;
constexpr int NFIN = 4;
}

__global__ __launch_bounds__(256, 1) void conv3x3_c32_kernel(EngineArgs p) {
    using namespace c32;
    __shared__ __attribute__((aligned(16))) char smem[LDS];
    const int lane = threadIdx.x & 63;
    const int wave = __builtin_amdgcn_readfirstlane(threadIdx.x >> 6);
    const int nwg = gridDim.x, hw = blockIdx.x;
    const int xcd = hw & 7, q = nwg >> 3, r = nwg & 7;
    const int wg = (xcd < r ? xcd * (q + 1) : r * (q + 1) + (xcd - r) * q) + (hw >> 3);
    const int tx_n = p.wo / TW, ty_n = p.ho / TH;
    const int tx = wg % tx_n, rest = wg / tx_n;
    const int ty = rest % ty_n, img = rest / ty_n;
    const int y0 = ty * TH, x0 = tx * TW;
    const int nch = p.cin_pad / 32;

    int hpix[HPW], hch[HPW];
#pragma unroll
    for (int t = 0; t < HPW; ++t) {
        const int hp = (wave + NWAVE * t) * 16 + (lane >> 2);
        hch[t] = (lane & 3) ^ h2::hkey(hp % HWID);
        int pix = -1;
        if (hp < HPIX) {
            const int hy = hp / HWID, hx = hp - hy * HWID;
            const int iy = y0 + hy - 1, ix = x0 + hx - 1;
            if (iy >= 0 && iy < p.hi && ix >= 0 && ix < p.wi) pix = (img * p.hi + iy) * p.wi + ix;
        }
        hpix[t] = pix;
    }
    const int wr = lane >> 2;
    auto issue = [&](int chunk, int buf) {
        char* b = smem + buf * BUF;
#pragma unroll
        for (int t = 0; t < HPW; ++t) {
            const bf16_t* src = hpix[t] >= 0 ? p.a + (int64_t)hpix[t] * p.cin_pad + hch[t] * 8 + chunk * 32 : p.zero;
            __builtin_amdgcn_global_load_lds(GLB_PTR(void, src), LDS_PTR(void, b + (wave + NWAVE * t) * 1024), 16, 0, 0);
        }
        for (int v = wave; v < WPIECES; v += NWAVE) {
            const int tap = v >> 1, row = 16 * (v & 1) + wr;
            const bf16_t* src = p.w + (int64_t)row * p.ldw + tap * p.cin_pad + chunk * 32 + (((lane & 3) ^ ((row >> 1) & 3)) * 8);
            __builtin_amdgcn_global_load_lds(GLB_PTR(void, src), LDS_PTR(void, b + HBYTES + v * 1024), 16, 0, 0);
        }
    };
    const int n_issue = HPW + (WPIECES - wave + NWAVE - 1) / NWAVE;
// ... 212 lines not shown
        rd(0, 0);
#pragma unroll
        for (int tap = 0; tap < 9; ++tap) {
            const int s = tap & 1;
            if (tap + 1 < 9) rd(tap + 1, s ^ 1);
            __builtin_amdgcn_sched_barrier(0);
#pragma unroll
            for (int i = 0; i < 8; ++i)
#pragma unroll
                for (int j = 0; j < 4; ++j)
                    acc[i][j] = __builtin_amdgcn_mfma_f32_16x16x32_f16(__builtin_bit_cast(f16x8, fb[s][j]),
                                                                       __builtin_bit_cast(f16x8, fa[s][i]), acc[i][j], 0, 0, 0);
            __builtin_amdgcn_sched_barrier(0);
        }
        __builtin_amdgcn_sched_barrier(0);
        __builtin_amdgcn_s_barrier();
    }
    engine_epilogue<HkTile, E_CONV, TW, false>(p, (img * p.ho + y0) * p.wo + x0, n0, acc);
}
#endif

using T128 = Tile<128, 128, 2, 2, 3>;
using T128w8 = Tile<128, 128, 2, 4, 3>;
using T256 = Tile<256, 256, 2, 4, 4>;
using T256x128 = Tile<256, 128, 4, 2, 3>;
using T256x64 = Tile<256, 64, 4, 1, 4>;
using T96x256 = Tile<96, 256, 2, 4, 3>;
using T64x256 = Tile<64, 256, 2, 4, 3>;
using T64x256w4 = Tile<64, 256, 1, 4, 3>;
using T96x256s5 = Tile<96, 256, 2, 4, 5>;
using T96x256s6 = Tile<96, 256, 2, 4, 6>;
using T64x256s6 = Tile<64, 256, 2, 4, 6>;
using T128s6 = Tile<128, 128, 2, 2, 6>;
using T128w8s6 = Tile<128, 128, 2, 4, 6>;
using T128k2s3 = Tile<128, 128, 2, 2, 3, 2>;
using T128k2s4 = Tile<128, 128, 2, 2, 4, 2>;
using T128w8k2s4 = Tile<128, 128, 2, 4, 4, 2>;
using T96x256k2 = Tile<96, 256, 2, 4, 3, 2>;
using T64x256k2 = Tile<64, 256, 2, 4, 3, 2>;
using T64x256w4k2 = Tile<64, 256, 1, 4, 3, 2>;
using T64c = Tile<64, 64, 2, 2, 8>;
using T64x128c = Tile<64, 128, 2, 2, 6>;

int pick_group_m(int tiles_m, int tiles_n, int bm, int bn, int64_t per_xcd, int64_t a_bytes = 0) {
    if (rf::env_set("RF_GEMM_GROUP_M")) return std::max(1, std::min(tiles_m, rf::env_int("RF_GEMM_GROUP_M", 0)));
    if (RF_ENV_ONCE("RF_GEMM_STREAM_RASTER", 1) != 0 && a_bytes > (192ll << 20) && tiles_n <= 8) return std::max(1, std::min(tiles_m, 32 / tiles_n));
    const double g = std::sqrt((double)per_xcd * bn / bm);
    int gm = (int)(g + 0.5);
    gm = std::max(1, std::min(gm, tiles_m));
    if ((int64_t)gm * tiles_n < per_xcd / 2) gm = std::min<int64_t>(tiles_m, (per_xcd + tiles_n - 1) / tiles_n);
    return gm;
}

template <class C, int EPI, int NTERM, bool GATHER = false>
int launch(EngineArgs a, void* stream, const char* what) {
    const int tiles_m = (a.m + C::BM - 1) / C::BM, tiles_n = a.n / C::BN;
    const int nwg = tiles_n * tiles_m;
    a.group_m = pick_group_m(tiles_m, tiles_n, C::BM, C::BN, (nwg + 7) / 8, GATHER ? 0 : (int64_t)a.m * a.k * 2);
    RF_LAUNCH((engine_kernel<C, EPI, NTERM, GATHER, false>), dim3(nwg), dim3(C::THREADS), 0, (hipStream_t)stream,
                       a);
    return rf::check_launch(what);
}

template <class C>
bool halo_ok(EngineArgs& a) {
    if (a.kw != 3 || a.k != 9 * a.cin_pad || a.stride != 1 || a.pad != 1 || a.ho != a.hi || a.wo != a.wi) return false;
    if (a.cin_pad % BK || a.m % C::BM || (a.ho * a.wo) % C::BM) return false;
    const int tw = std::min(C::BM, a.wo);
    if (tw < 16 || (tw & (tw - 1)) || a.wo % tw || C::BM % tw) return false;
    const int th = C::BM / tw;
    if (a.ho % th || (th + 2) * (tw + 2) > Halo<C>::ROWS) return false;
    a.halo_lg = __builtin_ctz(tw);
    return true;
}

template <class C, int EPI>
int launch_halo(EngineArgs a, void* stream, const char* what) {
    const int tiles_m = a.m / C::BM, tiles_n = a.n / C::BN;
    const int nwg = tiles_n * tiles_m;
    a.group_m = pick_group_m(tiles_m, tiles_n, C::BM, C::BN, (nwg + 7) / 8);
    RF_LAUNCH((halo_kernel<C, EPI>), dim3(nwg), dim3(C::THREADS), 0, (hipStream_t)stream, a);
    return rf::check_launch(what);
}

template <class C, int NTERM, bool GATHER>
int launch_conv(EngineArgs& a, void* stream, const char* what) {
    if constexpr (GATHER && NTERM == P_F16) {
        const bool want = rf::env_int("RF_CONV_HALO", C::BM == 128 && C::NWAVE == 4) != 0;
        if (want && halo_ok<C>(a)) return launch_halo<C, E_CONV>(a, stream, what);
    }
    return launch<C, E_CONV, NTERM, GATHER>(a, stream, what);
}

constexpr int SK_MAX_GRID = 768;
constexpr int64_t SK_PART_FLOATS = (int64_t)256 * 256 * 256;
constexpr int64_t SK_WS_BYTES = SK_PART_FLOATS * 4 + SK_MAX_GRID * 4;

template <class C, int EPI, int NTERM = 1, bool GATHER = false>
int launch_sk(EngineArgs a, int grid, void* stream, const char* what) {
    const int tiles_m = (a.m + C::BM - 1) / C::BM, tiles_n = a.n / C::BN;
    a.group_m = pick_group_m(tiles_m, tiles_n, C::BM, C::BN, ((int64_t)tiles_m * tiles_n + 7) / 8);
    RF_LAUNCH((engine_kernel<C, EPI, NTERM, GATHER, true>), dim3(grid), dim3(C::THREADS), 0,
                       (hipStream_t)stream, a);
    return rf::check_launch(what);
}

int sk_setup(EngineArgs& p, void* workspace, void* stream) {
    p.sk_part = (float*)workspace;
    p.sk_flag = (int*)(p.sk_part + SK_PART_FLOATS);
    p.sk_epoch = rf::next_epoch(p.sk_flag, SK_MAX_GRID * sizeof(int), (hipStream_t)stream);
    if (p.sk_epoch == 0) return RF_ERR_LAUNCH;
    p.err = rf::device_error_word();
    p.spin = rf::spin_limit();
    p.stamps = RF_ENV_ONCE("RF_GEMM_STAMPS", 0) != 0 ? (uint64_t*)(p.sk_part + SK_PART_FLOATS - 65536) : nullptr;
    return RF_OK;
}

template <class F>
int with_epi(int epilogue, F&& f) {
    switch (epilogue) {
        case RF_EPI_BF16: return f(std::integral_constant<int, E_BF16>{});
        case RF_EPI_F32: return f(std::integral_constant<int, E_F32>{});
        case RF_EPI_ADD_F32: return f(std::integral_constant<int, E_ADD>{});
        default: return f(std::integral_constant<int, E_SWIGLU>{});
    }
}

inline void dense_args(EngineArgs& p, const void* a, int64_t lda, const void* w, int64_t ldw, int m, int n, int k,
                       void* c, int64_t ldc) {
    p.a = (const bf16_t*)a;
    p.lda = lda;
    p.w = (const bf16_t*)w;
    p.ldw = ldw;
    p.m = m;
    p.n = n;
    p.k = k;
    p.c = c;
    p.ldc = ldc;
}


int sk_grid(int m, int n, int k) {
    const bool env = rf::env_set("RF_GEMM_SK");
    int grid = 2 * 256;
    if (!env) return 0;
    if (env) {
        grid = rf::env_int("RF_GEMM_SK", 0);
        if (grid <= 0) return 0;
        grid = grid > SK_MAX_GRID ? SK_MAX_GRID : grid;
    }
    const int64_t tiles = (int64_t)((m + 127) / 128) * (n / 128);
    const int64_t rounds = (tiles + 511) / 512;
    const double eff = (double)tiles / (rounds * 512);
    if (!env && (eff >= 0.9 || tiles * (k / BK) < 8LL * grid)) return 0;
    return grid;
// ... 555 lines not shown
    if (mode == 2 && workspace && ws_bytes >= SK_WS_BYTES) {
        if (const int rc = sk_setup(a, workspace, stream)) return rc;
        RF_LAUNCH((quad_kernel<WM, WN, EPI, NT, STG>), dim3(256), dim3(256), 0, (hipStream_t)stream, a);
    } else {
        a.sk_flag = nullptr;
        RF_LAUNCH((quad_kernel<WM, WN, EPI, NT, STG>), dim3(grid), dim3(256), 0, (hipStream_t)stream, a);
    }
    return rf::check_launch(what);
}

template <int WM, int WN, int NT>
static int run_quad_t(const EngineArgs& p, int epilogue, int mode, void* workspace, int64_t ws_bytes, void* stream,
                      const char* what) {
    return with_epi(epilogue, [&](auto e) {
        return launch_quad<WM, WN, decltype(e)::value, NT>(p, mode, workspace, ws_bytes, stream, what);
    });
}

template <int NT>
static int run_quad(const EngineArgs& p, int epilogue, int mode, void* workspace, int64_t ws_bytes, void* stream,
                    const char* what) {
    switch (quad_tile()) {
        case 192256: return run_quad_t<96, 128, NT>(p, epilogue, mode, workspace, ws_bytes, stream, what);
        case 160256: return run_quad_t<80, 128, NT>(p, epilogue, mode, workspace, ws_bytes, stream, what);
        case 128192: return run_quad_t<64, 96, NT>(p, epilogue, mode, workspace, ws_bytes, stream, what);
        case 128128: return run_quad_t<64, 64, NT>(p, epilogue, mode, workspace, ws_bytes, stream, what);
        default: return run_quad_t<128, 128, NT>(p, epilogue, mode, workspace, ws_bytes, stream, what);
    }
}
#endif

static int gemm_bf16(const void* a, int64_t lda, const void* w, int64_t ldw, void* c, int64_t ldc,
                     const float* bias, int m, int n, int k, int epilogue, void* workspace, int64_t ws_bytes,
                     void* stream, const int* gate, bool f16 = false, const EngineArgs* norm = nullptr) {
    RF_REQUIRE(a && w && c, "rf_gemm_bf16: null pointer");
    int out_f16 = 0;
    if (epilogue == RF_EPI_F16 || epilogue == RF_EPI_SWIGLU_F16) {
        out_f16 = 1;
        epilogue = epilogue == RF_EPI_F16 ? RF_EPI_BF16 : RF_EPI_SWIGLU;
    }
    RF_REQUIRE(m > 0 && n > 0 && k > 0, "rf_gemm_bf16: empty problem m=%d n=%d k=%d", m, n, k);
    RF_REQUIRE(k % BK == 0, "rf_gemm_bf16: K=%d must be a multiple of %d", k, BK);
    RF_REQUIRE(n % 128 == 0, "rf_gemm_bf16: N=%d must be a multiple of 128", n);
    RF_REQUIRE(lda % 8 == 0 && ldw % 8 == 0 && lda >= k && ldw >= k, "rf_gemm_bf16: lda/ldw must be >=K and 16-B aligned");
    RF_REQUIRE(((uintptr_t)a & 15) == 0 && ((uintptr_t)w & 15) == 0, "rf_gemm_bf16: operands must be 16-B aligned");
    RF_REQUIRE(epilogue >= RF_EPI_BF16 && epilogue <= RF_EPI_SWIGLU, "rf_gemm_bf16: bad epilogue %d", epilogue);
    RF_REQUIRE(ldc >= (epilogue == RF_EPI_SWIGLU ? n / 2 : n) && ldc % 4 == 0, "rf_gemm_bf16: ldc too small/unaligned");
    RF_REQUIRE(((uintptr_t)c & 7) == 0, "rf_gemm_bf16: output must be 8-B aligned");
    EngineArgs p = norm ? *norm : EngineArgs{};
    dense_args(p, a, lda, w, ldw, m, n, k, c, ldc);
    p.bias = bias;
    p.gate = gate;
    p.out_f16 = out_f16;
    p.range = (out_f16 || (p.xg && p.xg_f16)) ? rf::range_word() : nullptr;
    const char* what = f16 ? "rf_gemm_f16" : "rf_gemm_bf16";
    const bool ws_ok = workspace && ws_bytes >= SK_WS_BYTES;
#ifdef RF_STUDY
    if (const int qm = norm ? 0 : quad_mode(m, n, k, lda, ldw, epilogue)) {
        return f16 ? run_quad<P_F16>(p, epilogue, qm, workspace, ws_bytes, stream, what)
                   : run_quad<1>(p, epilogue, qm, workspace, ws_bytes, stream, what);
    }
#else
    if (rf::env_int("RF_GEMM_QUAD", 0) > 0) return rf::study_only("rf_gemm: RF_GEMM_QUAD");
#endif
    if (ws_ok && skph(m, n, k)) {
        if (const int rc = sk_setup(p, workspace, stream)) return rc;
        const int64_t tiles = (int64_t)((m + 255) / 256) * (n / 256);
        p.persist = tiles % 256 == 0 && persist_on();
        return with_epi(epilogue, [&](auto e) {
            return f16 ? launch_phased_sk<decltype(e)::value, P_F16>(p, 256, stream, what)
                       : launch_phased_sk<decltype(e)::value>(p, 256, stream, what);
        });
    }
    const int cfg = pick_cfg(m, n, k, epilogue);
    if (f16) return run_dp<P_F16>(TileTable{}, cfg, p, epilogue, stream);
    const bool big = cfg != TC_R128;
    const int grid = (!big && ws_ok) ? sk_grid(m, n, k) : 0;
    if (grid) {
        if (const int rc = sk_setup(p, workspace, stream)) return rc;
        return with_epi(epilogue, [&](auto e) { return launch_sk<T128, decltype(e)::value>(p, grid, stream, what); });
    }
    if (ws_ok && n % 256 == 0 && sk256(m, n, k)) {
        if (const int rc = sk_setup(p, workspace, stream)) return rc;
        return with_epi(epilogue, [&](auto e) { return launch_sk<T256, decltype(e)::value>(p, 256, stream, what); });
    }
    return run_dp<1>(TileTable{}, cfg, p, epilogue, stream);
}

extern "C" int rf_gemm_bf16(const void* a, int64_t lda, const void* w, int64_t ldw, void* c, int64_t ldc,
                            const float* bias, int m, int n, int k, int epilogue, void* workspace, int64_t ws_bytes,
                            void* stream) {
    return gemm_bf16(a, lda, w, ldw, c, ldc, bias, m, n, k, epilogue, workspace, ws_bytes, stream, nullptr);
}

extern "C" int rf_gemm_f16(const void* a, int64_t lda, const void* w, int64_t ldw, void* c, int64_t ldc,
                           const float* bias, int m, int n, int k, int epilogue, void* workspace, int64_t ws_bytes,
                           void* stream) {
    return gemm_bf16(a, lda, w, ldw, c, ldc, bias, m, n, k, epilogue, workspace, ws_bytes, stream, nullptr, true);
}

extern "C" int rf_gemm_add_prenorm(const void* a, int64_t lda, const void* w, int64_t ldw, float* x, int64_t ldx,
                                   int m, int n, int k, const float* norm_w, void* xg, int64_t ldxg, float* ss,
                                   int operand_dtype, void* workspace, int64_t ws_bytes, void* stream) {
    RF_REQUIRE(x && norm_w && xg && ss, "rf_gemm_add_prenorm: null pointer");
    RF_REQUIRE(operand_dtype == RF_DT_F16 || operand_dtype == RF_DT_BF16, "rf_gemm_add_prenorm: operand_dtype");
    RF_REQUIRE(ldxg >= n && ldxg % 4 == 0 && ((uintptr_t)xg & 7) == 0, "rf_gemm_add_prenorm: xg rows (ldxg >= N, 8-B)");
    RF_REQUIRE(((uintptr_t)ss & 15) == 0 && ((uintptr_t)norm_w & 15) == 0, "rf_gemm_add_prenorm: ss / norm_w 16-B aligned");
    const bool f16 = operand_dtype == RF_DT_F16;
    if (n > PN_SLOTS * 128) {
        const int rc = gemm_bf16(a, lda, w, ldw, x, ldx, nullptr, m, n, k, RF_EPI_ADD_F32, workspace, ws_bytes, stream,
                                 nullptr, f16);
        if (rc != RF_OK) return rc;
        return rf_prenorm(x, ldx, norm_w, xg, ldxg, ss, m, n, operand_dtype, stream);
    }
    EngineArgs nio{};
    nio.xg = (bf16_t*)xg;
    nio.ldxg = ldxg;
    nio.norm_g = norm_w;
    nio.ss_out = ss;
    nio.xg_f16 = f16;
    return gemm_bf16(a, lda, w, ldw, x, ldx, nullptr, m, n, k, RF_EPI_ADD_F32, workspace, ws_bytes, stream, nullptr,
                     f16, &nio);
}

extern "C" int rf_gemm_rownorm(const void* a, int64_t lda, const void* w, int64_t ldw, void* c, int64_t ldc, int m,
                               int n, int k, int epilogue, const float* ss, int norm_dim, float eps, float* seg_ss,
                               int seg_w, int n_seg, int operand_dtype, void* workspace, int64_t ws_bytes,
                               void* stream) {
    RF_REQUIRE(ss && ((uintptr_t)ss & 15) == 0, "rf_gemm_rownorm: ss must be 16-B aligned");
    RF_REQUIRE(norm_dim > 0, "rf_gemm_rownorm: norm_dim must be positive");
    RF_REQUIRE(epilogue == RF_EPI_BF16 || epilogue == RF_EPI_F16 || epilogue == RF_EPI_SWIGLU ||
                   epilogue == RF_EPI_SWIGLU_F16,
               "rf_gemm_rownorm: epilogue must be RF_EPI_BF16 / F16 / SWIGLU / SWIGLU_F16 (got %d)", epilogue);
    RF_REQUIRE(operand_dtype == RF_DT_F16 || operand_dtype == RF_DT_BF16, "rf_gemm_rownorm: operand_dtype");
    RF_REQUIRE(!seg_ss || ((epilogue == RF_EPI_BF16 || epilogue == RF_EPI_F16) && ((uintptr_t)seg_ss & 15) == 0 &&
                           seg_w > 0 && seg_w % 256 == 0 && seg_w <= PN_SLOTS * 128 && n_seg >= 1 &&
                           (int64_t)seg_w * n_seg <= n),
               "rf_gemm_rownorm: seg_ss needs a 16-bit (non-SwiGLU) epilogue, 16-B alignment, seg_w %% 256 == 0 and "
               "<= %d, n_seg >= 1 segments inside N", PN_SLOTS * 128);
    EngineArgs nio{};
    nio.rs_part = ss;
    nio.rs_n = (float)norm_dim;
    nio.rs_eps = eps;
    nio.seg_ss = seg_ss;
    nio.seg_w = seg_w;
    nio.seg_n = seg_ss ? n_seg : 0;
    return gemm_bf16(a, lda, w, ldw, c, ldc, nullptr, m, n, k, epilogue, workspace, ws_bytes, stream, nullptr,
                     operand_dtype == RF_DT_F16, &nio);
}

template <class C, int NT>
static int launch_rope(EngineArgs p, void* stream) {
    return launch<C, E_ROPE, NT>(p, stream, "rf_gemm_qk_rope");
}

extern "C" int rf_gemm_qk_rope(const void* a, int64_t lda, const void* w, int64_t ldw, void* c, int64_t ldc, int m,
                               int n, int k, const float* ss, int norm_dim, float eps, float* seg_ss, int seg_w,
                               int n_seg, const float* norm_w, const float* pos, int64_t ld_pos, int pos_div,
                               const float* freqs, int n_freqs, float q_scale, int operand_dtype, void* workspace,
                               int64_t ws_bytes, void* stream) {
    (void)workspace;
    (void)ws_bytes;
    RF_REQUIRE(a && w && c, "rf_gemm_qk_rope: null pointer");
    RF_REQUIRE(m > 0 && n > 0 && k > 0, "rf_gemm_qk_rope: empty problem m=%d n=%d k=%d", m, n, k);
    RF_REQUIRE(operand_dtype == RF_DT_F16 || operand_dtype == RF_DT_BF16, "rf_gemm_qk_rope: operand_dtype");
    RF_REQUIRE(k % 64 == 0 && n % 128 == 0, "rf_gemm_qk_rope: needs K %% 64 == 0 and N %% 128 == 0");
    RF_REQUIRE(lda % 8 == 0 && ldw % 8 == 0 && lda >= k && ldw >= k && ((uintptr_t)a & 15) == 0 &&
                   ((uintptr_t)w & 15) == 0, "rf_gemm_qk_rope: operands must be 16-B aligned with lda/ldw >= K");
    RF_REQUIRE(ldc >= n && ldc % 4 == 0 && ((uintptr_t)c & 7) == 0, "rf_gemm_qk_rope: ldc too small/unaligned");
    RF_REQUIRE(seg_w > 0 && seg_w % 256 == 0 && seg_w % 128 == 0 && n_seg >= 1 && (int64_t)seg_w * n_seg <= n,
               "rf_gemm_qk_rope: the q/k segments must be whole 256-column tiles inside N");
    RF_REQUIRE(!seg_ss || (((uintptr_t)seg_ss & 15) == 0 && seg_w <= PN_SLOTS * 128),
               "rf_gemm_qk_rope: seg_ss must be 16-B aligned and seg_w <= %d", PN_SLOTS * 128);
    RF_REQUIRE(!ss || (((uintptr_t)ss & 15) == 0 && norm_dim > 0), "rf_gemm_qk_rope: ss must be 16-B aligned");
    RF_REQUIRE(!norm_w || ((uintptr_t)norm_w & 15) == 0, "rf_gemm_qk_rope: norm_w must be 16-B aligned");
// ... 83 lines not shown
    RF_LAUNCH(quant_mx8_kernel, dim3((unsigned)((n + 255) / 256)), dim3(256), 0, (hipStream_t)stream,
                       (const bf16_t*)x, ldx, rows, cols, (uint8_t*)q, ldq, (uint8_t*)scales, ld_s);
    return rf::check_launch("rf_quant_mx8");
}

static bool halo2_ok(const EngineArgs& a) {
    const int env = rf::env_int("RF_CONV_HALO2", -1);
    if (env == 0) return false;
    if (!rf::env_set("RF_CONV_HALO2") && rf::env_set("RF_CONV_TILE")) return false;
    if (a.kw != 3 || a.k != 9 * a.cin_pad || a.stride != 1 || a.pad != 1 || a.ho != a.hi || a.wo != a.wi) return false;
    if (a.cin_pad % 32 || (a.n % 128 && a.n != 64) || a.ho % h2::TH || a.wo % h2::TW || a.m % 512) return false;
    const int64_t blocks = (int64_t)(a.m / 512) * (a.n == 64 ? 1 : a.n / 128);
    return env == 1 || blocks >= 256;
}

static int launch_halo2(EngineArgs a, void* stream, const char* what) {
    const bool n64 = a.n == 64;
    const int nwg = (a.m / 512) * (n64 ? 1 : a.n / 128);
    const int ring = rf::env_int("RF_CONV_H2S", 4);
    const hipStream_t st = (hipStream_t)stream;
    const int dbg = rf::env_int("RF_H2_DBG", 0);
#ifndef RF_STUDY
    if (dbg) return rf::study_only("rf_conv: RF_H2_DBG (halo2 ablation builds)");
#else
    if (!n64 && ring == 4 && dbg >= 1 && dbg <= 8) {
        if (dbg == 1) RF_LAUNCH((halo2_kernel<4, 128, 1>), dim3(nwg), dim3(512), 0, st, a);
        if (dbg == 2) RF_LAUNCH((halo2_kernel<4, 128, 2>), dim3(nwg), dim3(512), 0, st, a);
        if (dbg == 3) RF_LAUNCH((halo2_kernel<4, 128, 3>), dim3(nwg), dim3(512), 0, st, a);
        if (dbg == 4) RF_LAUNCH((halo2_kernel<4, 128, 4>), dim3(nwg), dim3(512), 0, st, a);
        if (dbg == 8) RF_LAUNCH((halo2_kernel<4, 128, 8>), dim3(nwg), dim3(512), 0, st, a);
        return rf::check_launch(what);
    }
#endif
    if (n64) {
        if (ring == 3) RF_LAUNCH((halo2_kernel<3, 64>), dim3(nwg), dim3(512), 0, st, a);
        else if (ring == 5) RF_LAUNCH((halo2_kernel<5, 64>), dim3(nwg), dim3(512), 0, st, a);
        else RF_LAUNCH((halo2_kernel<4, 64>), dim3(nwg), dim3(512), 0, st, a);
    } else {
        if (ring == 3) RF_LAUNCH((halo2_kernel<3, 128>), dim3(nwg), dim3(512), 0, st, a);
        else if (ring == 5) RF_LAUNCH((halo2_kernel<5, 128>), dim3(nwg), dim3(512), 0, st, a);
        else RF_LAUNCH((halo2_kernel<4, 128>), dim3(nwg), dim3(512), 0, st, a);
    }
    return rf::check_launch(what);
}

static bool halo3_ok(const EngineArgs& a) {
    if (rf::env_int("RF_CONV_HALO3", 1) == 0 || (a.flags & RF_CONV_FINAL) || a.n % 128 || a.deconv) return false;
    if ((int64_t)128 * a.ldw * 2 >= 0x7fffffff) return false;
    return halo2_ok(a);
}

static int launch_halo3(EngineArgs a, void* stream, const char* what) {
    const int nwg = (a.m / 512) * (a.n / 128);
    const int dbg = rf::env_int("RF_H3_DBG", 0);
#ifndef RF_STUDY
    if (dbg) return rf::study_only("rf_conv: RF_H3_DBG (halo3 ablation builds, garbage results)");
    RF_LAUNCH(halo3_kernel<0>, dim3(nwg), dim3(512), 0, (hipStream_t)stream, a);
#else
    if (dbg == 1) RF_LAUNCH(halo3_kernel<1>, dim3(nwg), dim3(512), 0, (hipStream_t)stream, a);
    else if (dbg == 2) RF_LAUNCH(halo3_kernel<2>, dim3(nwg), dim3(512), 0, (hipStream_t)stream, a);
    else if (dbg == 4) RF_LAUNCH(halo3_kernel<4>, dim3(nwg), dim3(512), 0, (hipStream_t)stream, a);
    else if (dbg == 6) RF_LAUNCH(halo3_kernel<6>, dim3(nwg), dim3(512), 0, (hipStream_t)stream, a);
    else if (dbg == 8) RF_LAUNCH(halo3_kernel<8>, dim3(nwg), dim3(512), 0, (hipStream_t)stream, a);
    else if (dbg == 14) RF_LAUNCH(halo3_kernel<14>, dim3(nwg), dim3(512), 0, (hipStream_t)stream, a);
    else if (dbg == 15) RF_LAUNCH(halo3_kernel<15>, dim3(nwg), dim3(512), 0, (hipStream_t)stream, a);
    else if (dbg == 30) RF_LAUNCH(halo3_kernel<30>, dim3(nwg), dim3(512), 0, (hipStream_t)stream, a);
    else if (dbg == 16) RF_LAUNCH(halo3_kernel<16>, dim3(nwg), dim3(512), 0, (hipStream_t)stream, a);
    else if (dbg == 32) RF_LAUNCH(halo3_kernel<32>, dim3(nwg), dim3(512), 0, (hipStream_t)stream, a);
    else if (dbg == 64) RF_LAUNCH(halo3_kernel<64>, dim3(nwg), dim3(512), 0, (hipStream_t)stream, a);
    else if (dbg == 96) RF_LAUNCH(halo3_kernel<96>, dim3(nwg), dim3(512), 0, (hipStream_t)stream, a);
    else RF_LAUNCH(halo3_kernel<0>, dim3(nwg), dim3(512), 0, (hipStream_t)stream, a);
#endif
    return rf::check_launch(what);
}

static bool c32_ok(const EngineArgs& a) {
    if (rf::env_int("RF_CONV_C32", 1) == 0 || !(a.flags & RF_CONV_FINAL) || a.cout > 32 || a.n < 32) return false;
    if (a.kw != 3 || a.k != 9 * a.cin_pad || a.stride != 1 || a.pad != 1 || a.ho != a.hi || a.wo != a.wi) return false;
    return a.cin_pad % 32 == 0 && a.ho % c32::TH == 0 && a.wo % c32::TW == 0 && a.m > 0 && a.n_fin <= c32::NFIN;
}

static int launch_c32(EngineArgs a, void* stream, const char* what) {
    const int nwg = a.m / (c32::TH * c32::TW);
    RF_LAUNCH(conv3x3_c32_kernel, dim3(nwg), dim3(256), 0, (hipStream_t)stream, a);
    return rf::check_launch(what);
}

static bool hk_ok(const EngineArgs& a) {
    const int env = rf::env_int("RF_CONV_HK", 0);
    if (env == 0 || (a.flags & RF_CONV_FINAL) || a.deconv) return false;
#ifndef RF_STUDY
    return true;
#else
    if (a.kw != 3 || a.k != 9 * a.cin_pad || a.stride != 1 || a.pad != 1 || a.ho != a.hi || a.wo != a.wi) return false;
    if (a.cin_pad % 32 || a.n % hk::NCO || a.ho % hk::TH || a.wo % hk::TW || a.m <= 0) return false;
    return env == 1 || (int64_t)(a.m / (hk::TH * hk::TW)) * (a.n / hk::NCO) >= 256;
#endif
}

static int launch_hk(EngineArgs a, void* stream, const char* what) {
#ifdef RF_STUDY
    const int nwg = (a.m / (hk::TH * hk::TW)) * (a.n / hk::NCO);
    RF_LAUNCH(conv3x3_hk_kernel, dim3(nwg), dim3(256), 0, (hipStream_t)stream, a);
    return rf::check_launch(what);
#else
    (void)a, (void)stream, (void)what;
// ... 5 lines not shown
    CT_AUTO = 0,
    CT_64 = 64,
    CT_128 = 128,
    CT_256 = 256,
    CT_128w8 = 1288,
    CT_256x128 = 2561,
    CT_64x128 = 6412,
    CT_64SK = 6464,
};
static int conv_tile_env() { return rf::env_int("RF_CONV_TILE", CT_AUTO); }

template <bool GATHER>
static int conv_f16_dp(EngineArgs& p, void* stream, const char* what, int tile = 0) {
    if (GATHER && c32_ok(p)) return launch_c32(p, stream, what);
    if (GATHER && hk_ok(p)) return launch_hk(p, stream, what);
    if (GATHER && halo3_ok(p)) return launch_halo3(p, stream, what);
    if (GATHER && halo2_ok(p)) return launch_halo2(p, stream, what);
    const int t = tile ? tile : conv_tile_env();
    if (p.n == 64) return launch_conv<T256x64, P_F16, GATHER>(p, stream, what);
    if (t == CT_64 || t == CT_64SK) return launch_conv<T64c, P_F16, GATHER>(p, stream, what);
    if (t == CT_64x128) return launch_conv<T64x128c, P_F16, GATHER>(p, stream, what);
    if (t == CT_128) return launch_conv<T128, P_F16, GATHER>(p, stream, what);
    if (t == CT_128w8) return launch_conv<T128w8, P_F16, GATHER>(p, stream, what);
    if (t == CT_256x128) return launch<T256x128, E_CONV, P_F16, GATHER>(p, stream, what);
    if (p.n % 256 == 0 && (t == CT_256 || (t == CT_AUTO && ((p.m + 255) / 256) * (p.n / 256) >= 256)))
        return (rf::env_int("RF_CONV_PHASED", 0) != 0 && use_phased(p.n, p.k))
                   ? launch_phased<E_CONV, P_F16, GATHER, 256>(p, stream, what)
                   : launch_conv<T256, P_F16, GATHER>(p, stream, what);
    const int64_t tiles = (int64_t)((p.m + 127) / 128) * (p.n / 128);
    if (tiles <= 512) return launch_conv<T128w8, P_F16, GATHER>(p, stream, what);
    return launch_conv<T128, P_F16, GATHER>(p, stream, what);
}

template <int NT>
static int conv_dispatch(EngineArgs& p, bool gather, bool big, int64_t sk_grid_n, void* workspace, void* stream,
                         const char* what, int tile = 0) {
    if constexpr (NT == P_F16) {
        if (!sk_grid_n)
            return gather ? conv_f16_dp<true>(p, stream, what, tile) : conv_f16_dp<false>(p, stream, what, tile);
    }
    if (sk_grid_n) {
        if (const int rc = sk_setup(p, workspace, stream)) return rc;
        if (NT == P_F16 && rf::env_int("RF_CONV_SKW8", 1) != 0)
            return gather ? launch_sk<T128w8, E_CONV, NT, true>(p, (int)sk_grid_n, stream, what)
                          : launch_sk<T128w8, E_CONV, NT, false>(p, (int)sk_grid_n, stream, what);
        return gather ? launch_sk<T128, E_CONV, NT, true>(p, (int)sk_grid_n, stream, what)
                      : launch_sk<T128, E_CONV, NT, false>(p, (int)sk_grid_n, stream, what);
    }
    if (gather)
        return big ? launch<T256x128, E_CONV, NT, true>(p, stream, what) : launch<T128, E_CONV, NT, true>(p, stream, what);
    return big ? launch<T256x128, E_CONV, NT, false>(p, stream, what) : launch<T128, E_CONV, NT, false>(p, stream, what);
}

static int conv_common(EngineArgs& p, int nterm, bool gather, const void* w_hi, const void* w_lo, int cout, int cout_pad, float* out,
                       const float* bias, const float* res1, const float* res2, void* p_hi, void* p_lo, int p_ld,
                       int flags, const float* w_fin, const float* b_fin, int n_fin, float elu_alpha, void* workspace,
                       int64_t ws_bytes, void* stream, const char* what) {
    RF_REQUIRE(w_hi && (w_lo || nterm == P_F16), "%s: null weights", what);
    RF_REQUIRE(cout % 4 == 0, "%s: cout must be a multiple of 4", what);
    RF_REQUIRE(out || p_hi, "%s: no output", what);
    RF_REQUIRE(!p_hi || ((p_lo || nterm == P_F16) && p_ld % 4 == 0 && p_ld >= cout), "%s: bad plane output", what);
    RF_REQUIRE(!(flags & RF_CONV_FINAL) || (cout <= 64 && w_fin && b_fin && n_fin > 0 && out),
               "%s: final head needs cout <= 64 and w_fin/b_fin", what);
    RF_REQUIRE(!(flags & RF_CONV_BORDER_BIAS) ||
                   (bias && !(flags & RF_CONV_FINAL) && p.kw == 3 && p.k == 9 * p.cin_pad && p.stride == 1 &&
                    p.pad == 1 && p.ho == p.hi && p.wo == p.wi && p.deconv == 0 && p.ho >= 2 && p.wo >= 2),
               "%s: RF_CONV_BORDER_BIAS needs a 3x3 stride-1 pad-1 convolution of an image of at least 2 x 2 pixels "
               "with its 9-row bias", what);
    static void* z = nullptr;
    if (!z && hipGetSymbolAddress(&z, HIP_SYMBOL(g_zero_row)) != hipSuccess) {
        z = nullptr;
        rf::set_error("%s: zero row symbol", what);
        return RF_ERR_LAUNCH;
    }
    p.zero = (const bf16_t*)z;
    p.w = (const bf16_t*)w_hi;
    p.w_lo = (const bf16_t*)w_lo;
    p.n = cout_pad;
    p.c = out;
    p.bias = bias;
    p.res1 = res1;
    p.res2 = res2;
    p.p_hi = (bf16_t*)p_hi;
    p.p_lo = (bf16_t*)p_lo;
    p.p_ld = p_ld;
    p.plane_f16 = nterm == P_F16;
    p.range = (p_hi && nterm == P_F16) ? rf::range_word() : nullptr;
    p.cout = cout;
    p.flags = flags;
    p.w_fin = w_fin;
    p.b_fin = b_fin;
    p.n_fin = n_fin;
    p.elu_alpha = elu_alpha;
    if (p.m <= 0) return RF_OK;
    const bool big = rf::env_set("RF_CONV_TILE") ? conv_tile_env() == CT_256 : ((p.m + 255) / 256) * (p.n / 128) >= 256;
    int64_t skg = 0;
    int ct = conv_tile_env();
    if (!ct && RF_ENV_ONCE("RF_CONV_SMALL", 1) != 0 && nterm == P_F16 && gather && p.kw == 3 && p.n % 64 == 0 && p.m <= 4096 &&
        (p.k <= 2304 || p.m <= 1024))
        ct = p.k <= 2304 ? CT_64 : CT_64SK;
    if (nterm == P_F16 && ct == CT_64SK && p.n % 64 == 0 && workspace && ws_bytes >= SK_WS_BYTES) {
        const int64_t tiles = (int64_t)((p.m + 63) / 64) * (p.n / 64);
        const int64_t grid = std::min<int64_t>(512, tiles * (p.k / BK) / 12);
        if (grid > tiles) {
            if (const int rc = sk_setup(p, workspace, stream)) return rc;
            return gather ? launch_sk<T64c, E_CONV, P_F16, true>(p, (int)grid, stream, what)
                          : launch_sk<T64c, E_CONV, P_F16, false>(p, (int)grid, stream, what);
        }
    }
    if (!big && p.n % 128 == 0 && workspace && ws_bytes >= SK_WS_BYTES && rf::env_int("RF_CONV_SK", 1) != 0 &&
        !(nterm == P_F16 && (ct == CT_64 || ct == CT_64x128 || ct == CT_64SK))) {
        const int64_t tiles = (int64_t)((p.m + 127) / 128) * (p.n / 128);
        const int64_t work = tiles * (p.k / BK);
        const int64_t grid = std::min<int64_t>(256, work / 8);
        if (tiles < 192 && grid > tiles) skg = grid;
    }
    return nterm == P_F16 ? conv_dispatch<P_F16>(p, gather, big, skg, workspace, stream, what, ct == CT_64 ? CT_64 : CT_AUTO)
                          : conv_dispatch<3>(p, gather, big, skg, workspace, stream, what);
}

extern "C" int rf_conv2d_bf16x3(const void* in_hi, const void* in_lo, int n_img, int hi, int wi, int cin_pad,
                                const void* w_hi, const void* w_lo, int cout, int cout_pad, int kh, int kw, int stride,
                                int pad, const float* bias, const float* res1, const float* res2, float* out,
                                void* p_hi, void* p_lo, int p_ld, int flags, const float* w_fin, const float* b_fin,
                                int n_fin, float elu_alpha, void* workspace, int64_t ws_bytes, void* stream) {
    RF_REQUIRE(in_hi && in_lo, "rf_conv2d_bf16x3: null input");
    RF_REQUIRE(cin_pad % BK == 0, "rf_conv2d_bf16x3: cin_pad %d must be a multiple of %d", cin_pad, BK);
    RF_REQUIRE(cout_pad % 128 == 0 && cout_pad >= cout, "rf_conv2d_bf16x3: cout_pad %d must be a multiple of 128",
               cout_pad);
    EngineArgs p{};
    p.a = (const bf16_t*)in_hi;
    p.a_lo = (const bf16_t*)in_lo;
    p.hi = hi;
    p.wi = wi;
    p.cin_pad = cin_pad;
    p.cin_m = udiv_magic(cin_pad);
    p.ho = (hi + 2 * pad - kh) / stride + 1;
    p.wo = (wi + 2 * pad - kw) / stride + 1;
    p.kw = kw;
    p.kw_m = udiv_magic(kw);
    p.stride = stride;
    p.pad = pad;
    p.m = n_img * p.ho * p.wo;
    p.k = kh * kw * cin_pad;
    RF_REQUIRE(p.k < 65536, "conv: kh*kw*cin_pad = %d must be < 65536", p.k);
    p.ldw = p.k;
    return conv_common(p, 3, true, w_hi, w_lo, cout, cout_pad, out, bias, res1, res2, p_hi, p_lo, p_ld, flags, w_fin,
                       b_fin, n_fin, elu_alpha, workspace, ws_bytes, stream, "rf_conv2d_bf16x3");
}

extern "C" int rf_conv2d_f16(const void* in, int n_img, int hi, int wi, int cin_pad, const void* w, int cout,
                             int cout_pad, int kh, int kw, int stride, int pad, const float* bias, const float* res1,
                             const float* res2, float* out, void* p_out, int p_ld, int flags, const float* w_fin,
                             const float* b_fin, int n_fin, float elu_alpha, void* workspace, int64_t ws_bytes,
                             void* stream) {
    RF_REQUIRE(in, "rf_conv2d_f16: null input");
    RF_REQUIRE(cin_pad % BK == 0, "rf_conv2d_f16: cin_pad %d must be a multiple of %d", cin_pad, BK);
    RF_REQUIRE((cout_pad % 128 == 0 || cout_pad == 64) && cout_pad >= cout,
               "rf_conv2d_f16: cout_pad %d must be 64 or a multiple of 128", cout_pad);
    EngineArgs p{};
    p.a = (const bf16_t*)in;
    p.hi = hi;
    p.wi = wi;
    p.cin_pad = cin_pad;
    p.cin_m = udiv_magic(cin_pad);
    p.ho = (hi + 2 * pad - kh) / stride + 1;
    p.wo = (wi + 2 * pad - kw) / stride + 1;
    p.kw = kw;
    p.kw_m = udiv_magic(kw);
    p.stride = stride;
    p.pad = pad;
    p.m = n_img * p.ho * p.wo;
    p.k = kh * kw * cin_pad;
    RF_REQUIRE(p.k < 65536, "conv: kh*kw*cin_pad = %d must be < 65536", p.k);
    p.ldw = p.k;
    return conv_common(p, P_F16, true, w, nullptr, cout, cout_pad, out, bias, res1, res2, p_out, nullptr, p_ld, flags,
                       w_fin, b_fin, n_fin, elu_alpha, workspace, ws_bytes, stream, "rf_conv2d_f16");
}

static const char* group_member(EngineArgs& p, const rf_conv_desc& d, const void* zero) {
    if (!d.in || !d.w || !(d.out || d.p_out)) return "null pointer";
    if (d.cin_pad % BK) return "cin_pad must be a multiple of 32";
    if (d.cout % 4) return "cout must be a multiple of 4";
    if (d.p_out && (d.p_ld % 4 || d.p_ld < d.cout)) return "bad p_ld";
    if (d.flags & RF_CONV_FINAL) return "the fused final head runs on its own launch";
    p = EngineArgs{};
    p.a = (const bf16_t*)d.in;
    p.cin_pad = d.cin_pad;
    p.cin_m = udiv_magic(d.cin_pad);
    p.zero = (const bf16_t*)zero;
    if (d.deconv_k > 0) {
        p.hi = p.ho = d.hi;
        p.wi = p.wo = d.wi;
        p.kw = 1;
        p.stride = 1;
        p.pad = 0;
        p.deconv = d.deconv_k;
        p.n = d.deconv_k * d.deconv_k * d.cout;
        if (d.flags) return "a deconvolution takes no flags";
    } else {
        p.hi = d.hi;
        p.wi = d.wi;
        p.ho = (d.hi + 2 * d.pad - d.kh) / d.stride + 1;
        p.wo = (d.wi + 2 * d.pad - d.kw) / d.stride + 1;
        p.kw = d.kw;
        p.stride = d.stride;
        p.pad = d.pad;
        p.n = d.cout_pad;
        if (d.cout_pad < d.cout) return "cout_pad < cout";
        if ((d.flags & RF_CONV_BORDER_BIAS) &&
            !(d.bias && d.kh == 3 && d.kw == 3 && d.stride == 1 && d.pad == 1 && d.hi >= 2 && d.wi >= 2))
            return "RF_CONV_BORDER_BIAS needs a 3x3 stride-1 pad-1 convolution of an image of at least 2 x 2 pixels "
                   "with its 9-row bias";
    }
    p.kw_m = udiv_magic(p.kw);
    p.m = d.n_img * p.ho * p.wo;
    p.k = (d.deconv_k > 0 ? 1 : d.kh * d.kw) * d.cin_pad;
    if (p.k >= 65536) return "kh*kw*cin_pad must be < 65536";
    if (p.n % T128w8::BN) return "output channels (k*k*cout for a deconvolution) must be a multiple of 128";
    p.ldw = p.k;
    p.w = (const bf16_t*)d.w;
    p.c = d.out;
    p.bias = d.bias;
    p.p_hi = (bf16_t*)d.p_out;
    p.p_ld = d.p_ld;
    p.plane_f16 = 1;
    p.range = d.p_out ? rf::range_word() : nullptr;
    p.cout = d.cout;
    p.flags = d.flags;
    return nullptr;
// ... 106 lines not shown
```

renderformer_amd/csrc/stage.cpp:

```cpp
#include <hip/hip_runtime.h>

#include <cmath>

#include "common.h"

namespace {
constexpr int64_t kAlign = 256;
int64_t align_up(int64_t b) { return (b + kAlign - 1) / kAlign * kAlign; }

struct EncBufs {
    int64_t h, qkv, att, g, ss, qkss, total;
};
EncBufs enc_layout(int rows, int dim, int ffn) {
    EncBufs b;
    const int64_t r = rows;
    b.h = 0;
    b.qkv = b.h + align_up(r * dim * 2);
    b.att = b.qkv + align_up(r * 3 * dim * 2);
    b.g = b.att + align_up(r * dim * 2);
    b.ss = b.g + align_up(r * (int64_t)ffn * 2);
    b.qkss = b.ss + align_up(r * RF_PRENORM_SLOTS * 4);
    b.total = b.qkss + align_up(r * 2 * RF_PRENORM_SLOTS * 4);
    return b;
}
// ... 242 lines not shown
        else
            RF_CALL(rf_gemm_rownorm(h, D, L.w_q, D, q2, D, T2, D, D, RF_EPI_BF16, ss, D, d->eps, nullptr, 0, 0, dt, gws,
                                    gwb, stream));
        const uint16_t* kvi = kv_batch ? kv + (int64_t)2 * D * i : kv;
        if (!kv_batch) {
            RF_CALL(rmsnorm(d->ctx, d->ld_ctx, L.kv_norm, d->eps, hc, d->ctx_dim, T1, d->ctx_dim, stream));
            RF_CALL(gemm(hc, d->ctx_dim, L.w_kv, d->ctx_dim, kv, ld_kv, nullptr, T1, 2 * D, d->ctx_dim, RF_EPI_BF16,
                         gws, gwb, stream));
        }
        const uint16_t* ki = k_batch ? kview + (int64_t)D * i : kview;
        if (!qf)
            RF_CALL(rf_qk_norm_rope(q2, D, q2, D, nullptr, T2, D, H, 1, L.q_norm, d->eps, kQLog2Scale, d->ray_pos,
                                    d->ld_ray_pos, d->ray_pos ? d->ray_pos_div : 1, d->freqs, d->ray_pos ? nf : 0,
                                    stream));
        if (!k_batch)
            RF_CALL(k_rope(kvi, ld_kv, 0, kview, ld_kview, 0, d->kv_src_rows, d->kv_rows, D, H, 1, 1, L.k_norm, 0, d->eps,
                           1.0f, d->kv_pos, d->ld_kv_pos, 1, d->freqs, d->kv_pos ? nf : 0, stream));
        if (d->timer_cross) RF_CALL(rf_ktimer_arm());
        if (qn)
            RF_CALL(rf_attn_fwd_qn(q2, D, ki, ld_kview, kvi + D, ld_kv, att, D, o_dt, qkss, RF_PRENORM_SLOTS, D, d->eps,
                                   kQLog2Scale, d->cross_problems, d->n_cross, H, 128, d->attn_ws, d->cross_bounds,
                                   d->cross_bounds ? d->cross_grid : 0, stream));
        else
            RF_CALL(rf_attn_fwd_dt(q2, D, ki, ld_kview, kvi + D, ld_kv, att, D, RF_DT_BF16, o_dt, d->cross_problems,
                                   d->n_cross, H, 128, kLn2, d->attn_ws, d->cross_bounds,
                                   d->cross_bounds ? d->cross_grid : 0, stream));
        RF_CALL(rf_gemm_add_prenorm(att, D, L.w_out, D, x, ldx, T2, D, D, self_attn ? L.self_norm : L.ffn_norm, h, D,
                                    ss, dt, gws, gwb, stream));
        if (self_attn) {
            const bool qkn = d->swin && L.self_qk_norm && D % 256 == 0 && D <= RF_PRENORM_SLOTS * 128;
            RF_CALL(rf_gemm_rownorm(h, D, L.w_self_in, D, qkv, 3 * D, T2, 3 * D, D, RF_EPI_BF16, ss, D, d->eps,
                                    qkn ? qkss : nullptr, D, 2, dt, gws, gwb, stream));
            if (qkn) {
                RF_CALL(rf_swin_attn_fwd_qkn(qkv, 3 * D, qkv + D, 3 * D, qkv + 2 * D, 3 * D, att, D, o_dt, d->n_images,
                                             d->grid_h, d->grid_w, d->window, i % 2 == 0 ? 0 : d->shift, H, 128, kLn2,
                                             qkss, L.self_qk_norm, d->eps, kQLog2Scale, stream));
            } else if (d->swin) {
                RF_CALL(rf_qk_norm_rope(qkv, 3 * D, qkv, 3 * D, nullptr, T2, D, H, 2, L.self_qk_norm, d->eps,
                                        kQLog2Scale, nullptr, 0, 1, nullptr, 0, stream));
                RF_CALL(rf_swin_attn_fwd_dt(qkv, 3 * D, qkv + D, 3 * D, qkv + 2 * D, 3 * D, att, D, o_dt, d->n_images,
                                            d->grid_h, d->grid_w, d->window, i % 2 == 0 ? 0 : d->shift, H, 128, kLn2,
                                            stream));
            } else {
                RF_CALL(rf_qk_norm_rope(qkv, 3 * D, qkv, 3 * D, nullptr, T2, D, H, 2, L.self_qk_norm, d->eps,
                                        kQLog2Scale, d->ray_pos, d->ld_ray_pos, d->ray_pos ? d->ray_pos_div : 1,
                                        d->freqs, d->ray_pos ? nf : 0, stream));
                RF_CALL(rf_attn_fwd_dt(qkv, 3 * D, qkv + D, 3 * D, qkv + 2 * D, 3 * D, att, D, RF_DT_BF16, o_dt,
                                       d->self_problems, d->n_self, H, 128, kLn2, d->attn_ws, nullptr, 0, stream));
            }
            RF_CALL(rf_gemm_add_prenorm(att, D, L.w_self_out, D, x, ldx, T2, D, D, L.ffn_norm, h, D, ss, dt, gws, gwb,
                                        stream));
        }
        RF_CALL(rf_gemm_rownorm(h, D, L.w13, D, g, F, T2, 2 * F, D, epi_swiglu, ss, D, d->eps, nullptr, 0, 0, dt, gws, gwb, stream));
        if (i + 1 < NL)
            RF_CALL(rf_gemm_add_prenorm(g, F, L.w2, F, x, ldx, T2, D, F, d->layers[i + 1].query_norm, h, D, ss, dt, gws,
                                        gwb, stream));
        else
            RF_CALL(gemm(g, F, L.w2, F, x, ldx, nullptr, T2, D, F, RF_EPI_ADD_F32, gws, gwb, stream));
        if (tap < d->n_taps && d->taps[tap].layer == i) {
            const rf_decoder_tap& t = d->taps[tap++];
            RF_CALL(rf_split_planes(x, T2, D, ldx, t.p_hi, t.p_lo, t.p_ld, 0, stream));
        }
    }
    return RF_OK;
}
```

renderformer_amd/dpt.py:

```python
from __future__ import annotations

import os
from dataclasses import dataclass
from typing import Dict, List, Optional

import torch

import ctypes

from ._lib import call, ptr, stream

PLANE_SILU, SILU_OUT, FINAL, LOG_DECODE, NCHW_OUT, BORDER_BIAS = 1, 2, 4, 8, 16, 32
BK, BN = 32, 128


def _pad(c: int, m: int) -> int:
    return -(-c // m) * m


def _split(w: torch.Tensor):
    hi = w.to(torch.bfloat16)
    lo = (w - hi.float()).to(torch.bfloat16)
    return hi.contiguous(), lo.contiguous()

# ... 94 lines not shown
        d.n_img, d.hi, d.wi, d.cin_pad, d.cout, d.cout_pad = n, h, w, c.cin_pad, c.cout, c.cout_pad
        d.kh, d.kw, d.stride, d.pad, d.deconv_k = c.kh, c.kw, stride, pad, c.k
        d.p_ld = ld_out or 0
        d.flags = PLANE_SILU if j.get("planes_silu") else 0
        results.append((out, pl))
    call("rf_conv2d_f16_group", len(jobs), ctypes.cast(descs, ctypes.c_void_p), stream())
    return results


def fold_affine_1x1(w3: torch.Tensor, b3: torch.Tensor, w1: torch.Tensor, b1: torch.Tensor):
    w3 = w3.detach().double().cpu()
    w1 = w1.detach().double().cpu().reshape(w1.shape[0], w1.shape[1])
    w = torch.einsum("ocyx,ci->oiyx", w3, w1)
    tap = torch.einsum("ocyx,c->oyx", w3, b1.detach().double().cpu())
    keep = {0: [1, 2], 1: [0, 1, 2], 2: [0, 1]}
    b = torch.empty(9, w3.shape[0], dtype=torch.float64)
    b3 = b3.detach().double().cpu()
    for ry in range(3):
        for rx in range(3):
            b[3 * ry + rx] = b3 + tap[:, keep[ry]][:, :, keep[rx]].sum((1, 2))
    return w, b


class _Conv:

    def __init__(self, w: torch.Tensor, b, device, deconv: bool = False, f16: bool = False):
        self.f16 = f16
        w = w.detach().float().cpu()
        if deconv:
            cin, cout, k, _ = w.shape
            self.k, self.kh, self.kw = k, 1, 1
            self.cin_pad = _pad(cin, BK)
            mat = torch.zeros(k * k * cout, self.cin_pad)
            mat[:, :cin] = w.permute(2, 3, 1, 0).reshape(k * k * cout, cin)
            self.cout_pad = k * k * cout
        else:
            cout, cin, kh, kw = w.shape
            self.k, self.kh, self.kw = 0, kh, kw
            self.cin_pad = _pad(cin, BK)
            self.cout_pad = 64 if (f16 and cout <= 64) else _pad(cout, BN)
            mat = torch.zeros(self.cout_pad, kh, kw, self.cin_pad)
            mat[:cout, :, :, :cin] = w.permute(0, 2, 3, 1)
            mat = mat.reshape(self.cout_pad, -1)
        self.cin, self.cout = cin, cout
        if f16:
            self.w_hi, self.w_lo = mat.to(torch.float16).contiguous().to(device), None
        else:
            hi, lo = _split(mat)
            self.w_hi, self.w_lo = hi.to(device), lo.to(device)
        self.b = None if b is None else b.detach().float().to(device).contiguous()

    def __call__(self, x: Planes, stride=1, pad=None, res1=None, res2=None, out_f32=False,
                 planes_ld: Optional[int] = None, planes_silu=False, final=None, final_flags=0,
                 border_bias: Optional[torch.Tensor] = None):
        n, h, w, ld = x.shape
        if ld != self.cin_pad or x.c != self.cin:
            raise ValueError(f"conv input planes must have {self.cin} channels padded to {self.cin_pad}, got "
                             f"{x.c}/{ld}")
        if x.f16 != self.f16:
            raise ValueError("conv input planes and weights must use the same operand precision")
        dev = x.hi.device
        from .ops import _gemm_workspace
        ws = _gemm_workspace(dev)
        if self.k:
            ho, wo = h * self.k, w * self.k
        else:
            pad = self.kh // 2 if pad is None else pad
            ho = (h + 2 * pad - self.kh) // stride + 1
            wo = (w + 2 * pad - self.kw) // stride + 1
        if final is not None:
            w_fin, b_fin, alpha = final
            nf = w_fin.shape[0]
            shape = (n, nf, ho, wo) if final_flags & NCHW_OUT else (n, ho, wo, nf)
            out = torch.empty(shape, device=dev)
            if self.f16:
                call("rf_conv2d_f16", ptr(x.hi), n, h, w, ld, ptr(self.w_hi), self.cout, self.cout_pad, self.kh,
                     self.kw, stride, pad, ptr(self.b), 0, 0, ptr(out), 0, 0, FINAL | final_flags, ptr(w_fin),
                     ptr(b_fin), nf, alpha, ptr(ws), ws.numel(), stream())
            else:
                call("rf_conv2d_bf16x3", ptr(x.hi), ptr(x.lo), n, h, w, ld, ptr(self.w_hi), ptr(self.w_lo), self.cout,
                     self.cout_pad, self.kh, self.kw, stride, pad, ptr(self.b), 0, 0, ptr(out), 0, 0, 0,
                     FINAL | final_flags, ptr(w_fin), ptr(b_fin), nf, alpha, ptr(ws), ws.numel(), stream())
            return out
        out = torch.empty(n, ho, wo, self.cout, device=dev) if out_f32 else None
        pl = Planes.empty(n, ho, wo, self.cout, planes_ld, dev, self.f16) if planes_ld else None
        for r in (res1, res2):
            if r is not None and (tuple(r.shape) != (n, ho, wo, self.cout) or not r.is_contiguous()):
                raise ValueError("residual must match the conv output")
        flags = PLANE_SILU if planes_silu else 0
        bias = self.b
        if border_bias is not None:
            if not (self.f16 and not self.k and self.kh == 3 and stride == 1 and pad == 1):
                raise ValueError("border_bias needs an fp16 3x3 stride-1 pad-1 convolution")
            bias, flags = border_bias, flags | BORDER_BIAS
        if self.f16 and self.k:
            call("rf_deconv2d_f16", ptr(x.hi), n, h, w, ld, ptr(self.w_hi), self.cout, self.k, ptr(self.b), ptr(out),
                 ptr(pl.hi if pl else None), planes_ld or 0, ptr(ws), ws.numel(), stream())
        elif self.f16:
            call("rf_conv2d_f16", ptr(x.hi), n, h, w, ld, ptr(self.w_hi), self.cout, self.cout_pad, self.kh, self.kw,
                 stride, pad, ptr(bias), ptr(res1), ptr(res2), ptr(out), ptr(pl.hi if pl else None), planes_ld or 0,
                 flags, 0, 0, 0, 0.0, ptr(ws), ws.numel(), stream())
        elif self.k:
            call("rf_deconv2d_bf16x3", ptr(x.hi), ptr(x.lo), n, h, w, ld, ptr(self.w_hi), ptr(self.w_lo), self.cout,
                 self.k, ptr(self.b), ptr(out), ptr(pl.hi if pl else None), ptr(pl.lo if pl else None),
                 planes_ld or 0, ptr(ws), ws.numel(), stream())
        else:
            call("rf_conv2d_bf16x3", ptr(x.hi), ptr(x.lo), n, h, w, ld, ptr(self.w_hi), ptr(self.w_lo), self.cout,
                 self.cout_pad, self.kh, self.kw, stride, pad, ptr(self.b), ptr(res1), ptr(res2), ptr(out),
                 ptr(pl.hi if pl else None), ptr(pl.lo if pl else None), planes_ld or 0, flags, 0, 0, 0, 0.0,
                 ptr(ws), ws.numel(), stream())
        return out, pl


PRECISIONS = ("f16", "bf16x3")


class DPTHead:
    def __init__(self, sd: Dict[str, torch.Tensor], prefix: str, device, precision: str = "f16"):
        if precision not in PRECISIONS:
            raise ValueError(f"DPT precision must be one of {PRECISIONS}, got {precision!r}")
        self.precision = precision
        f16 = self.f16 = precision == "f16"
        g = lambda n: sd.get(f"{prefix}.{n}")
        C = lambda w, b, **kw: _Conv(w, b, device, f16=f16, **kw)
        self.projects = [C(g(f"projects.{i}.weight"), g(f"projects.{i}.bias")) for i in range(4)]
        self.resize = {0: C(g("resize_layers.0.weight"), g("resize_layers.0.bias"), deconv=True),
                       1: C(g("resize_layers.1.weight"), g("resize_layers.1.bias"), deconv=True),
                       3: C(g("resize_layers.3.weight"), g("resize_layers.3.bias"))}
        self.rn = [C(g(f"scratch.layer{i + 1}_rn.weight"), None) for i in range(4)]
        self.refine = {}
        for r in (1, 2, 3, 4):
            p = f"scratch.refinenet{r}"
            units = {}
            for u in ((1, 2) if r != 4 else (2,)):
                units[u] = [C(g(f"{p}.resConvUnit{u}.conv{c}.weight"), g(f"{p}.resConvUnit{u}.conv{c}.bias"))
                            for c in (1, 2)]
            self.refine[r] = (units, C(g(f"{p}.out_conv.weight"), g(f"{p}.out_conv.bias")))
        self.out1 = C(g("scratch.output_conv1.weight"), g("scratch.output_conv1.bias"))
        self.out2 = C(g("scratch.output_conv2.0.weight"), g("scratch.output_conv2.0.bias"))
        wf = g("scratch.output_conv2.2.weight")
        self.w_fin = wf.detach().float().reshape(wf.shape[0], -1).to(device).contiguous()
        self.b_fin = g("scratch.output_conv2.2.bias").detach().float().to(device).contiguous()
        if self.out2.cout > 64:
            raise ValueError("output_conv2 must have <= 64 channels for the fused head")
        self.feat_ld = self.refine[1][0][2][0].cin_pad
        self.group_proj = (f16 and os.environ.get("RF_DPT_GROUP", "1") != "0" and len(self.projects) <= 4 and
                           all(c.kh == 1 and c.kw == 1 and not c.k and c.cout_pad % 128 == 0 for c in self.projects))
        self.fold = f16 and os.environ.get("RF_DPT_FOLD", "1") != "0"
        if self.fold:
            w, b = fold_affine_1x1(g("scratch.output_conv1.weight"), g("scratch.output_conv1.bias"),
                                   g("scratch.refinenet1.out_conv.weight"), g("scratch.refinenet1.out_conv.bias"))
            self.out1_fold = C(w.float(), None)
            self.out1_fold_bias = b.float().to(device).contiguous()

    def _rcu(self, convs, x32, xs: Planes, extra=None, want_f32=False, next_silu=True, next_ld=None):
        _, t = convs[0](xs, planes_ld=convs[1].cin_pad, planes_silu=True)
        return convs[1](t, res1=x32, res2=extra, out_f32=want_f32, planes_ld=next_ld, planes_silu=next_silu)

    def _fuse(self, r, x0, x1, x1s, size, last=False):
        units, out_conv = self.refine[r]
        if x1 is None:
            out, outs = x0, split_planes(x0, self.feat_ld, silu=True, f16=self.f16)
        else:
            out, outs = self._rcu(units[1], x1, x1s, extra=x0, want_f32=True, next_ld=self.feat_ld)
        _, y = self._rcu(units[2], out, outs, next_silu=False, next_ld=out_conv.cin_pad)
        if last and self.fold:
            return upsample_planes(y, *size, planes_ld=self.out1_fold.cin_pad)
        y32, _ = out_conv(y, out_f32=True)
        if last:
            return upsample(y32, *size, out_f32=False, planes_ld=self.out1.cin_pad, f16=self.f16)[1]
        return upsample(y32, *size)[0]

    def tap_planes(self, i: int, t: torch.Tensor, n_img: int, hp: int, wp: int) -> Planes:
        return split_planes(t.view(n_img, hp, wp, t.shape[-1]), self.projects[i].cin_pad, f16=self.f16)

    def empty_tap_planes(self, i: int, n_img: int, hp: int, wp: int, c: int, device) -> Planes:
        return Planes.empty(n_img, hp, wp, c, self.projects[i].cin_pad, device, self.f16)

    @torch.no_grad()
    def __call__(self, taps: List, n_img: int, hp: int, wp: int, patch: int, elu_alpha: float,
                 log_decode: bool, channels_last: bool) -> torch.Tensor:
        layers = []
        xs = [t if isinstance(t, Planes) else self.tap_planes(i, t, n_img, hp, wp) for i, t in enumerate(taps)]
        nxt_ld = [(self.resize[i] if i in self.resize else self.rn[i]).cin_pad for i in range(len(xs))]
        if self.group_proj:
            xs = conv1x1_group(self.projects[:len(xs)], xs, nxt_ld)
        for i, x in enumerate(xs):
            if not self.group_proj:
                _, x = self.projects[i](x, planes_ld=nxt_ld[i])
            if i in self.resize:
                _, x = self.resize[i](x, stride=2 if i == 3 else 1, pad=1 if i == 3 else None,
                                      planes_ld=self.rn[i].cin_pad)
            layers.append(x)
        rn, rns = [], []
        for i in range(4):
            o, s = self.rn[i](layers[i], out_f32=True, planes_ld=self.feat_ld, planes_silu=True)
            rn.append(o)
            rns.append(s)
        size = lambda t: (t.shape[1], t.shape[2])
        units4, oc4 = self.refine[4]
        _, y = self._rcu(units4[2], rn[3], rns[3], next_silu=False, next_ld=oc4.cin_pad)
        y32, _ = oc4(y, out_f32=True)
        p4 = upsample(y32, *size(rn[2]))[0]
        p3 = self._fuse(3, p4, rn[2], rns[2], size(rn[1]))
        p2 = self._fuse(2, p3, rn[1], rns[1], size(rn[0]))
        p1 = self._fuse(1, p2, rn[0], rns[0], (2 * rn[0].shape[1], 2 * rn[0].shape[2]), last=True)
        if (p1.shape[1], p1.shape[2]) != (hp * patch, wp * patch):
            raise ValueError("DPT output size mismatch (patch size must be 8)")
        if self.fold:
            _, o1 = self.out1_fold(p1, planes_ld=self.out2.cin_pad, border_bias=self.out1_fold_bias)
        else:
            _, o1 = self.out1(p1, planes_ld=self.out2.cin_pad)
        flags = (LOG_DECODE if log_decode else 0) | (0 if channels_last else NCHW_OUT)
        return self.out2(o1, final=(self.w_fin, self.b_fin, elu_alpha), final_flags=flags)
```

renderformer_amd/model.py:

```python
from __future__ import annotations

import ctypes
import math
import os
import threading
from dataclasses import dataclass
from typing import Dict, List, Optional

import torch

from . import ops
from ._lib import load as _load_lib
from .config import RenderFormerConfig, named_config
from .dpt import PRECISIONS as DPT_PRECISIONS
from .dpt import DPTHead
from .weights import check_state_dict, load_snapshot, synthetic_state_dict

EPS = 1e-6
FP8_PROJECTIONS = ("q", "out", "self_in", "self_out", "w13", "w2")
FP8_DEFAULT = ("q", "w2")
SWIN_WINDOW, SWIN_SHIFT = 8, 4


def _bf16(t, device):
# ... 587 lines not shown
                ops.gemm_add_prenorm(inp, w_half, x, next_norm, h, ss, tag=tag)
            else:
                proj(inp, w_half, w_fp8, x, ops.EPI_ADD_F32, tag=tag, name=name)

        if defer:
            ops.prenorm(x, W.dec[0].query_norm, h, ss)
        for i, L in enumerate(W.dec):
            if qfuse:
                ops.gemm_qk_rope(h, L.wq, q2, ss, EPS, D, 1, L.q_norm if qk else None, q2ss, ray_pos, W.dec_freqs,
                                 q_scale=1.0 if qk else ops.Q_LOG2_SCALE, pos_div=R)
            else:
                norm_proj(L.query_norm, L.wq, getattr(L, "wq8", None), q2, name="q")
            if kv_batch:
                kv = kv_all[:, 2 * D * i:2 * D * (i + 1)]
            else:
                ops.rmsnorm(ctx, L.kv_norm, EPS, hc)
                ops.gemm(hc, L.wkv, kv)
            if k_batch:
                kview = kview_all[:, D * i:D * (i + 1)]
            if not qfuse:
                ops.qk_norm_rope(q2, q2, H, L.q_norm if qk else None, EPS, ray_pos, W.dec_freqs, pos_div=R,
                                 q_scale=ops.Q_LOG2_SCALE, ilv=W.qk_fused)
            if not k_batch:
                ops.qk_norm_rope_groups(kv[:, :D], 0, kview, 0, 1, H, L.k_norm if qk else None, EPS, pos2, W.dec_freqs,
                                        src_rows=plan.kv_src_rows, ilv=W.qk_fused)
            if q2ss is not None:
                ops.attention(q2, kview, kv[:, D:], att, plan.prob2, R, H, tag="attn_cross", max_k_len=plan.max_s,
                              schedule=plan.sched2, q_ss=q2ss[:, 0], q_eps=EPS)
            else:
                ops.attention(q2, kview, kv[:, D:], att, plan.prob2, R, H, tag="attn_cross", max_k_len=plan.max_s,
                              q_prescaled=True, schedule=plan.sched2)
            add_proj(att, L.wo, getattr(L, "wo8", None), L.self_norm if qkv is not None else L.ffn_norm, name="out")
            if qkv is not None:
                qs, ks, vs = qkv[:, :D], qkv[:, D:2 * D], qkv[:, 2 * D:]
                qks = qkv[:, :2 * D]
                qkn = swin and defer and qk and D % 256 == 0 and D <= ops.PRENORM_SLOTS * 128
                if qkn:
                    ops.gemm_rownorm(h, L.ws_in, qkv, ss, EPS, seg_ss=qkss, seg_w=D)
                else:
                    norm_proj(L.self_norm, L.ws_in, getattr(L, "ws_in8", None), qkv, name="self_in")
                if qkn:
                    ops.swin_attention(qs, ks, vs, att, P, plan.hp, plan.wp, 0 if i % 2 == 0 else SWIN_SHIFT, H,
                                       SWIN_WINDOW, qk_norm=(qkss, L.sqk_norm, EPS))
                elif swin:
                    ops.qk_norm_rope(qks, qks, H, L.sqk_norm if qk else None, EPS, n_seg=2, q_scale=ops.Q_LOG2_SCALE)
                    ops.swin_attention(qs, ks, vs, att, P, plan.hp, plan.wp, 0 if i % 2 == 0 else SWIN_SHIFT, H,
                                       SWIN_WINDOW, q_prescaled=True)
                else:
                    ops.qk_norm_rope(qks, qks, H, L.sqk_norm if qk else None, EPS, ray_pos, W.dec_freqs, pos_div=R,
                                     n_seg=2, q_scale=ops.Q_LOG2_SCALE)
                    ops.attention(qs, ks, vs, att, plan.prob_self, R, H, max_k_len=R, q_prescaled=True)
                add_proj(att, L.ws_out, getattr(L, "ws_out8", None), L.ffn_norm, name="self_out")
            norm_proj(L.ffn_norm, L.w13, getattr(L, "w13_8", None), g, ops.EPI_SWIGLU, tag="gemm_w13_stage2", name="w13")
            add_proj(g, L.w2, getattr(L, "w2_8", None), W.dec[i + 1].query_norm if i + 1 < n_dec else None,
                     tag="gemm_w2_stage2", name="w2")
            if i in outl:
                taps.append(W.dpt.tap_planes(len(taps), x, P, plan.hp, plan.wp))
            cap = self._capture
            if cap is not None and cap["dec"] is not None:
                rows = torch.cat([v * R + cap["dec"] for v in cap["views"]])
                cap["out"].setdefault("dec_rows", []).append(
                    x.index_select(0, rows).view(len(cap["views"]), -1, D).clone())
        if self._capture is not None:
            if "dec_rows" in self._capture["out"]:
                self._capture["out"]["dec_rows"] = torch.stack(self._capture["out"]["dec_rows"])
            self._capture = None
        return taps

    def _ray_embed(self, plan: _Plan, ray_in: torch.Tensor):
        cfg, W, dev = self.config, self._w, self._device
        D = cfg.view_transformer_latent_dim
        T2 = ray_in.shape[0]
        ray_lin = torch.empty(T2, D, dtype=torch.float32, device=dev)
        ops.gemm(ray_in, W.ray_w, ray_lin, W.ray_b, ops.EPI_F32)
        x2 = torch.empty(T2, D, dtype=torch.float32, device=dev)
        ops.embed(x2, None, T2, W.patch_token, 1, ray_lin, W.ray_norm, ops.FLT_EPS)
        return x2

    def _decode(self, plan: _Plan, taps, log_decode: bool, channels_last: bool):
        return self._w.dpt(taps, plan.B * plan.V, plan.hp, plan.wp, self.config.patch_size, 1e-3, log_decode,
                           channels_last)

    @torch.no_grad()
    def render_views(self, triangles, texture, mask, vn, c2w, fov, resolution: int, log_encode: bool = True,
                     timings: Optional[dict] = None) -> torch.Tensor:
        self._require()
        with torch.cuda.device(self._device):
            return self._guarded(
                lambda: self._render_views(triangles, texture, mask, vn, c2w, fov, resolution, log_encode),
                lambda: self._render_views(triangles, texture, mask, vn, c2w, fov, resolution, False),
                (triangles, texture, mask, vn, c2w, fov))

    @torch.no_grad()
    def encode_scene(self, triangles, texture, mask, vn, log_encode: bool = True) -> EncodedScene:
        self._require()
        dev = self._device
        with torch.cuda.device(dev):
            for t, n in ((triangles, "triangles"), (texture, "texture"), (mask, "mask"), (vn, "vn")):
                if t.device != dev:
                    raise ValueError(f"{n} must be on {dev} (got {t.device})")
            sc = EncodedScene(self, self._generation, dev, self._mask_host(mask), (triangles, texture, mask, vn))
            with sc.lock:
                self._encode_checked(sc, log_encode)
            return sc

    def _encode(self, sc: EncodedScene, log_encode: bool):
        cfg, dev = self.config, self._device
        triangles, texture, _, vn = sc.inputs
        B = sc.batch_size
        res0 = cfg.patch_size * (SWIN_WINDOW if cfg.view_transformer_use_swin_attn else 1)
# ... 378 lines not shown
```

renderformer_amd/ops.py:

```python
from __future__ import annotations

import math
import os
from typing import Optional

import torch

from ._lib import call, load, ptr, stream

EPI_BF16, EPI_F32, EPI_ADD_F32, EPI_SWIGLU = 0, 1, 2, 3
_EPI_F16, _EPI_SWIGLU_F16 = 4, 5
DT_BF16, DT_F16 = 0, 1
HALF = (torch.bfloat16, torch.float16)
FLT_EPS = float(torch.finfo(torch.float32).eps)
CUS = 256


class KernelTimer:

    def __init__(self, tag: str):
        self.tag = tag
        self.n = 0

    def start(self, tag):
# ... 157 lines not shown
    m, ex = torch.frexp(amax)
    e = ex - 9 + (m > 0.875).to(ex.dtype)
    e = torch.where(amax > 0, e, torch.full_like(e, -127)).clamp(-127, 127)
    q = (xb * torch.pow(2.0, -e.float())[:, :, None]).to(torch.float8_e4m3fn).view(rows, cols)
    return q.view(torch.uint8), (e + 127).to(torch.uint8)


def rmsnorm(x: torch.Tensor, w: torch.Tensor, eps: float, out: torch.Tensor) -> torch.Tensor:
    _dev(x, torch.float32, "x")
    _check(out.dtype in HALF, "rmsnorm: out must be bf16 or fp16")
    _dev(out, out.dtype, "out")
    _check(x.shape == out.shape and w.numel() == x.shape[1], "rmsnorm: shape mismatch")
    call("rf_rmsnorm_f16" if out.dtype == torch.float16 else "rf_rmsnorm", ptr(x), x.stride(0), ptr(w), eps, ptr(out),
         out.stride(0), x.shape[0], x.shape[1], stream())
    return out


PRENORM_SLOTS = 8


def _dt(t: torch.Tensor) -> int:
    return 1 if t.dtype == torch.float16 else 0


def prenorm(x: torch.Tensor, w: torch.Tensor, xg: torch.Tensor, ss: torch.Tensor) -> torch.Tensor:
    _dev(x, torch.float32, "x")
    _check(xg.dtype in HALF, "prenorm: xg must be bf16 or fp16")
    _dev(xg, xg.dtype, "xg")
    _dev(ss, torch.float32, "ss")
    _check(xg.shape == x.shape and w.numel() == x.shape[1], "prenorm: shape mismatch")
    _check(ss.shape[0] >= x.shape[0] and ss.shape[1] == PRENORM_SLOTS and ss.is_contiguous(), "prenorm: ss shape")
    call("rf_prenorm", ptr(x), x.stride(0), ptr(w), ptr(xg), xg.stride(0), ptr(ss), x.shape[0], x.shape[1], _dt(xg),
         stream())
    return xg


def gemm_add_prenorm(a: torch.Tensor, w: torch.Tensor, x: torch.Tensor, norm_w: torch.Tensor, xg: torch.Tensor,
                     ss: torch.Tensor, tag: Optional[str] = None) -> torch.Tensor:
    _check(a.dtype in HALF and w.dtype == a.dtype and xg.dtype == a.dtype,
           f"gemm_add_prenorm: a / w / xg must share bf16 or fp16 ({a.dtype}, {w.dtype}, {xg.dtype})")
    for t, n in ((a, "a"), (w, "w"), (xg, "xg")):
        _dev(t, t.dtype, n)
    _dev(x, torch.float32, "x")
    _dev(ss, torch.float32, "ss")
    m, k = a.shape
    n, k2 = w.shape
    _check(k == k2 and x.shape == (m, n) and xg.shape == (m, n) and norm_w.numel() == n,
           "gemm_add_prenorm: shape mismatch")
    _check(ss.shape[0] >= m and ss.shape[1] == PRENORM_SLOTS and ss.is_contiguous(), "gemm_add_prenorm: ss shape")
    ws = _gemm_workspace(a.device)
    _t0(tag)
    call("rf_gemm_add_prenorm", ptr(a), a.stride(0), ptr(w), w.stride(0), ptr(x), x.stride(0), m, n, k, ptr(norm_w),
         ptr(xg), xg.stride(0), ptr(ss), _dt(a), ptr(ws), ws.numel(), stream())
    return x


def gemm_rownorm(xg: torch.Tensor, w: torch.Tensor, out: torch.Tensor, ss: torch.Tensor, eps: float,
                 epilogue: int = EPI_BF16, tag: Optional[str] = None, seg_ss: Optional[torch.Tensor] = None,
                 seg_w: int = 0) -> torch.Tensor:
    _check(xg.dtype in HALF and w.dtype == xg.dtype, "gemm_rownorm: xg / w must both be bf16 or both fp16")
    _check(epilogue in (EPI_BF16, EPI_SWIGLU), "gemm_rownorm: epilogue must be EPI_BF16 or EPI_SWIGLU")
    _dev(xg, xg.dtype, "xg")
    _dev(w, w.dtype, "w")
    _dev(ss, torch.float32, "ss")
    _check(out.dtype in HALF, "gemm_rownorm: out must be bf16 or fp16")
    _dev(out, out.dtype, "out")
    m, k = xg.shape
    n, k2 = w.shape
    ncols = n // 2 if epilogue == EPI_SWIGLU else n
    _check(k == k2 and out.shape == (m, ncols), "gemm_rownorm: shape mismatch")
    _check(ss.shape[0] >= m and ss.shape[1] == PRENORM_SLOTS and ss.is_contiguous(), "gemm_rownorm: ss shape")
    epi = epilogue
    if out.dtype == torch.float16:
        epi = _EPI_F16 if epilogue == EPI_BF16 else _EPI_SWIGLU_F16
    ws = _gemm_workspace(xg.device)
    _t0(tag)
    n_seg = 0
    if seg_ss is not None:
        _dev(seg_ss, torch.float32, "seg_ss")
        _check(epilogue == EPI_BF16 and seg_ss.is_contiguous() and seg_ss.dim() == 3 and seg_ss.shape[0] >= m
               and seg_ss.shape[2] == PRENORM_SLOTS and seg_w > 0, "gemm_rownorm: seg_ss [M, n_seg, 8] with EPI_BF16")
        n_seg = seg_ss.shape[1]
    call("rf_gemm_rownorm", ptr(xg), xg.stride(0), ptr(w), w.stride(0), ptr(out), out.stride(0), m, n, k, epi, ptr(ss),
         k, eps, ptr(seg_ss), seg_w, n_seg, _dt(xg), ptr(ws), ws.numel(), stream())
    return out


def qk_norm_rope(src: torch.Tensor, dst: torch.Tensor, n_heads: int, norm_w: Optional[torch.Tensor], eps: float,
                 pos: Optional[torch.Tensor] = None, freqs: Optional[torch.Tensor] = None, pos_div: int = 1,
                 src_rows: Optional[torch.Tensor] = None, n_seg: int = 1, q_scale: float = 1.0,
                 ilv: bool = False) -> torch.Tensor:
    _dev(src, torch.bfloat16, "src")
    _dev(dst, torch.bfloat16, "dst")
    rows, width = dst.shape
    dim = n_heads * 128
    _check(width == n_seg * dim and src.shape[1] == width, "qk_norm_rope: width mismatch")
    if src_rows is None:
        _check(src.shape[0] == rows, "qk_norm_rope: row mismatch")
    else:
        _dev(src_rows, torch.int32, "src_rows")
    if norm_w is not None:
        _check(norm_w.numel() == n_seg * dim, "qk_norm_rope: norm weight size")
    if pos is not None:
        _dev(pos, torch.float32, "pos")
        _check(pos.shape[1] == 9 and freqs is not None, "qk_norm_rope: pos must be [*, 9] with freqs")
    if ilv:
# ... 268 lines not shown
def decoder_forward(x: torch.Tensor, layers, n_layers: int, n_heads: int, ffn_dim: int, operands: torch.dtype,
                    eps: float, ctx: torch.Tensor, kv: dict, cross: dict, self_attn: dict, taps=(),
                    tag: Optional[str] = None) -> torch.Tensor:
    from ._lib import DecoderDesc, DecoderTap
    import ctypes
    _dev(x, torch.float32, "x")
    _dev(ctx, torch.float32, "ctx")
    _check(operands in HALF, "decoder_forward: operands must be bf16 or fp16")
    rows, dim = x.shape
    _check(dim == n_heads * 128, "decoder_forward: dim must be n_heads * 128")
    _dev(cross["problems"], torch.int32, "cross problems")
    _dev(kv["kv_src_rows"], torch.int32, "kv_src_rows")
    for key in ("kv_pos", "freqs"):
        if kv.get(key) is not None:
            _dev(kv[key], torch.float32, key)
    if cross.get("ray_pos") is not None:
        _dev(cross["ray_pos"], torch.float32, "ray_pos")
    if cross.get("schedule") is not None:
        _dev(cross["schedule"], torch.int64, "schedule")
    kv_all = kv.get("kv_all")
    if kv_all is not None:
        _dev(kv_all, torch.bfloat16, "kv_all")
        _check(kv_all.dim() == 2 and kv_all.shape[0] == ctx.shape[0] and kv_all.shape[1] >= n_layers * 2 * dim,
               f"decoder_forward: kv_all must be [{ctx.shape[0]}, >= {n_layers * 2 * dim}], got {tuple(kv_all.shape)}")
    tarr = (DecoderTap * max(1, len(taps)))()
    for e, (layer, hi, lo, ld) in zip(tarr, taps):
        e.layer, e.p_hi, e.p_lo, e.p_ld = layer, ptr(hi), ptr(lo), ld
    gws = _gemm_workspace(x.device)
    sch = cross.get("schedule")
    pos, rpos, freqs = kv.get("kv_pos"), cross.get("ray_pos"), kv.get("freqs")
    sp = self_attn.get("problems")
    d = DecoderDesc(n_layers=n_layers, rows=rows, dim=dim, n_heads=n_heads, ffn_dim=ffn_dim,
                    operand_dtype=DT_F16 if operands == torch.float16 else DT_BF16, eps=eps,
                    layers=ctypes.addressof(layers), ctx=ptr(ctx), ld_ctx=ctx.stride(0), ctx_rows=ctx.shape[0],
                    ctx_dim=ctx.shape[1], ctx_norm=ptr(kv.get("ctx_norm")), w_kv_all=ptr(kv.get("w_kv_all")),
                    kv_rows=kv["kv_src_rows"].numel(), kv_src_rows=ptr(kv["kv_src_rows"]), kv_pos=ptr(pos),
                    ld_kv_pos=pos.stride(0) if pos is not None else 0, k_batch=int(bool(kv.get("k_batch"))),
                    k_norm_all=ptr(kv.get("k_norm_all")), freqs=ptr(freqs),
                    n_freqs=freqs.numel() if freqs is not None else 0, ray_pos=ptr(rpos),
                    ld_ray_pos=rpos.stride(0) if rpos is not None else 0, ray_pos_div=cross.get("ray_pos_div", 1),
                    cross_problems=ptr(cross["problems"]), n_cross=cross["problems"].shape[0], cross_bounds=ptr(sch),
                    cross_grid=sch.numel() - 1 if sch is not None else 0, swin=int(bool(self_attn.get("swin"))),
                    n_images=self_attn.get("n_images", 0), grid_h=self_attn.get("grid_h", 0),
                    grid_w=self_attn.get("grid_w", 0), window=self_attn.get("window", 0),
                    shift=self_attn.get("shift", 0), self_problems=ptr(sp), n_self=sp.shape[0] if sp is not None else 0,
                    taps=ctypes.addressof(tarr), n_taps=len(taps), gemm_ws=ptr(gws), gemm_ws_bytes=gws.numel(),
                    attn_ws=ptr(_attn_workspace(x.device)), kv_all=ptr(kv_all),
                    ld_kv_all=kv_all.stride(0) if kv_all is not None else 0)
    lib = load()
    ws = torch.empty(int(lib.rf_decoder_workspace_bytes(ctypes.addressof(d))), dtype=torch.uint8, device=x.device)
    d.workspace = ptr(ws)
    d.timer_cross = int(_timer_takes(tag, n_layers))
    d.qk_fused = int(bool(cross.get("qk_fused")))
    call("rf_decoder_forward", ptr(x), x.stride(0), ctypes.addressof(d), stream())
    return x


def swin_attention(q, k, v, out, n_images: int, grid_h: int, grid_w: int, shift: int, n_heads: int,
                   window: int = 8, q_prescaled: bool = False, qk_norm=None) -> torch.Tensor:
    for t, nme in ((q, "q"), (k, "k"), (v, "v")):
        _dev(t, torch.bfloat16, nme)
    _check(out.dtype in HALF, "swin_attention: out must be bf16 or fp16")
    _dev(out, out.dtype, "out")
    hd = q.shape[1] // n_heads
    odt = DT_F16 if out.dtype == torch.float16 else DT_BF16
    if qk_norm is None:
        call("rf_swin_attn_fwd_dt", ptr(q), q.stride(0), ptr(k), k.stride(0), ptr(v), v.stride(0), ptr(out),
             out.stride(0), odt, n_images, grid_h, grid_w, window, shift, n_heads, hd,
             LN2 if q_prescaled else 1.0 / math.sqrt(hd), stream())
        return out
    qk_ss, norm_w, eps = qk_norm
    _dev(qk_ss, torch.float32, "qk_ss")
    _check(qk_ss.is_contiguous() and qk_ss.shape[1:] == (2, PRENORM_SLOTS), "swin_attention: qk_ss [rows, 2, 8]")
    call("rf_swin_attn_fwd_qkn", ptr(q), q.stride(0), ptr(k), k.stride(0), ptr(v), v.stride(0), ptr(out),
         out.stride(0), odt, n_images, grid_h, grid_w, window, shift, n_heads, hd, LN2, ptr(qk_ss), ptr(norm_w), eps,
         Q_LOG2_SCALE, stream())
    return out


def texture_pack(texture: torch.Tensor, log_channels: int, dst_row: torch.Tensor, out: torch.Tensor):
    _dev(texture, torch.float32, "texture")
    _check(texture.is_contiguous(), "texture must be contiguous")
    b, n, c = texture.shape[:3]
    pe = texture[0, 0, 0].numel() if texture.dim() > 3 else 1
    call("rf_texture_pack", ptr(texture), b * n, c, pe, log_channels, ptr(dst_row), ptr(out), out.stride(0), stream())
    return out


def texture_pack_if(flag: torch.Tensor, texture: torch.Tensor, log_channels: int, dst_row: torch.Tensor,
                    out: torch.Tensor):
    _dev(flag, torch.int32, "flag")
    _dev(texture, torch.float32, "texture")
    _check(texture.is_contiguous(), "texture must be contiguous")
    b, n, c = texture.shape[:3]
    pe = texture[0, 0, 0].numel() if texture.dim() > 3 else 1
    call("rf_texture_pack_if", ptr(flag), ptr(texture), b * n, c, pe, log_channels, ptr(dst_row), ptr(out),
         out.stride(0), stream())
    return out


def texture_scan(texture: torch.Tensor, log_channels: int, dst_row: torch.Tensor, coef: torch.Tensor,
                 flag: torch.Tensor, flag_clear: Optional[torch.Tensor] = None):
    _dev(texture, torch.float32, "texture")
    _dev(coef, torch.float32, "coef")
    _dev(flag, torch.int32, "flag")
    _check(texture.is_contiguous() and texture.dim() == 5 and tuple(texture.shape[3:]) == (32, 32),
# ... 90 lines not shown
```

Baseline: 93.40.

## Fuse DPT tap plane writes into w2 GEMM and upsample into conv residual

The w2 residual-add GEMM epilogue can now write the fp16 DPT tap planes directly, so the separate split_planes pass over the decoder output is no longer needed at tap layers. In the DPT head, the bilinear upsample of each refinement output is deferred and folded into the next RCU conv epilogue, which reads four source pixels and interpolates the second residual on the fly. This avoids materialising the upsampled fp32 tensors and the extra kernel launches. In exchange the epilogue does more gathered residual loads and carries more registers, and fp16 range checking is added for the tap writes.

```diff
diff --git a/include/rf.h b/include/rf.h
--- a/include/rf.h
+++ b/include/rf.h
@@ -57,6 +57,9 @@
 int rf_gemm_add_prenorm(const void* a, int64_t lda, const void* w, int64_t ldw, float* x, int64_t ldx, int m, int n,
                         int k, const float* norm_w, void* xg, int64_t ldxg, float* ss, int operand_dtype,
                         void* workspace, int64_t ws_bytes, void* stream);
+int rf_gemm_add_tap(const void* a, int64_t lda, const void* w, int64_t ldw, float* x, int64_t ldx, int m, int n, int k,
+                    const float* norm_w, void* xg, int64_t ldxg, float* ss, void* plane, int p_ld, int operand_dtype,
+                    void* workspace, int64_t ws_bytes, void* stream);
 int rf_gemm_rownorm(const void* a, int64_t lda, const void* w, int64_t ldw, void* c, int64_t ldc, int m, int n,
                     int k, int epilogue, const float* ss, int norm_dim, float eps, float* seg_ss, int seg_w,
                     int n_seg, int operand_dtype, void* workspace, int64_t ws_bytes, void* stream);
@@ -187,6 +190,10 @@
                   int kw, int stride, int pad, const float* bias, const float* res1, const float* res2, float* out,
                   void* p_out, int p_ld, int flags, const float* w_fin, const float* b_fin, int n_fin, float elu_alpha,
                   void* workspace, int64_t ws_bytes, void* stream);
+int rf_conv2d_f16_up(const void* in, int n_img, int hi, int wi, int cin_pad, const void* w, int cout, int cout_pad,
+                     int kh, int kw, int stride, int pad, const float* bias, const float* res1, const float* res2,
+                     int res2_hi, int res2_wi, float* out, void* p_out, int p_ld, int flags, void* workspace,
+                     int64_t ws_bytes, void* stream);
 typedef struct {
     const void* in;
     const void* w;
@@ -309,6 +316,7 @@
     int qk_fused;
     const void* kv_all;
     int64_t ld_kv_all;
+    int tap_fused;
 } rf_decoder_desc;
 
 int rf_decoder_forward(float* x, int64_t ldx, const rf_decoder_desc* desc, void* stream);
diff --git a/renderformer_amd/_lib.py b/renderformer_amd/_lib.py
--- a/renderformer_amd/_lib.py
+++ b/renderformer_amd/_lib.py
@@ -37,6 +37,7 @@
     "rf_rmsnorm": [_P, _L, _P, _F, _P, _L, _I, _I, _P],
     "rf_prenorm": [_P, _L, _P, _P, _L, _P, _I, _I, _I, _P],
     "rf_gemm_add_prenorm": [_P, _L, _P, _L, _P, _L, _I, _I, _I, _P, _P, _L, _P, _I, _P, _L, _P],
+    "rf_gemm_add_tap": [_P, _L, _P, _L, _P, _L, _I, _I, _I, _P, _P, _L, _P, _P, _I, _I, _P, _L, _P],
     "rf_gemm_rownorm": [_P, _L, _P, _L, _P, _L, _I, _I, _I, _I, _P, _I, _F, _P, _I, _I, _I, _P, _L, _P],
     "rf_gemm_qk_rope": [_P, _L, _P, _L, _P, _L, _I, _I, _I, _P, _I, _F, _P, _I, _I, _P, _P, _L, _I, _P, _I, _F, _I,
                         _P, _L, _P],
@@ -72,6 +73,7 @@
     "rf_deconv2d_bf16x3": [_P, _P, _I, _I, _I, _I, _P, _P, _I, _I, _P, _P, _P, _P, _I, _P, _L, _P],
     "rf_conv2d_f16": [_P, _I, _I, _I, _I, _P, _I, _I, _I, _I, _I, _I, _P, _P, _P, _P, _P, _I, _I, _P, _P, _I, _F,
                       _P, _L, _P],
+    "rf_conv2d_f16_up": [_P, _I, _I, _I, _I, _P, _I, _I, _I, _I, _I, _I, _P, _P, _P, _I, _I, _P, _P, _I, _I, _P, _L, _P],
     "rf_deconv2d_f16": [_P, _I, _I, _I, _I, _P, _I, _I, _P, _P, _P, _I, _P, _L, _P],
     "rf_split_planes": [_P, _L, _I, _L, _P, _P, _I, _I, _P],
     "rf_upsample_bilinear": [_P, _I, _I, _I, _I, _P, _I, _I, _P, _P, _I, _P],
@@ -133,7 +135,8 @@
                 ("n_cross", _I), ("cross_bounds", _P), ("cross_grid", _I), ("swin", _I), ("n_images", _I),
                 ("grid_h", _I), ("grid_w", _I), ("window", _I), ("shift", _I), ("self_problems", _P), ("n_self", _I),
                 ("taps", _P), ("n_taps", _I), ("workspace", _P), ("gemm_ws", _P), ("gemm_ws_bytes", _L),
-                ("attn_ws", _P), ("timer_cross", _I), ("qk_fused", _I), ("kv_all", _P), ("ld_kv_all", _L)]
+                ("attn_ws", _P), ("timer_cross", _I), ("qk_fused", _I), ("kv_all", _P), ("ld_kv_all", _L),
+                ("tap_fused", _I)]
 
 
 class HipLibraryError(RuntimeError):
diff --git a/renderformer_amd/csrc/common.h b/renderformer_amd/csrc/common.h
--- a/renderformer_amd/csrc/common.h
+++ b/renderformer_amd/csrc/common.h
@@ -47,6 +47,26 @@
 }
 
 RF_DEV float f16_bits_to_f32(uint16_t b) { return (float)__builtin_bit_cast(_Float16, b); }
+
+RF_DEV void resize_axis(float s, int o, int n, int& i0, int& i1, float& l0, float& l1) {
+    const float of = (float)o;
+    i0 = (int)(s * of);
+    i1 = i0 + (i0 < n - 1 ? 1 : 0);
+    l1 = __builtin_fmaf(s, of, -(float)i0);
+    l0 = 1.0f - l1;
+}
+RF_DEV float bilerp_xy(float a, float b, float d, float e, float lx0, float lx1, float ly0, float ly1) {
+    const float top = __builtin_fmaf(lx0, a, lx1 * b), bot = __builtin_fmaf(lx0, d, lx1 * e);
+    return __builtin_fmaf(ly1, bot, ly0 * top);
+}
+RF_DEV float bilerp_zw(float a, float b, float d, float e, float lx0, float lx1, float ly0, float ly1) {
+    const float top = __builtin_fmaf(lx1, b, lx0 * a), bot = __builtin_fmaf(lx1, e, lx0 * d);
+    return __builtin_fmaf(ly0, top, ly1 * bot);
+}
+RF_DEV float4 bilerp4(float4 a, float4 b, float4 d, float4 e, float lx0, float lx1, float ly0, float ly1) {
+    return make_float4(bilerp_xy(a.x, b.x, d.x, e.x, lx0, lx1, ly0, ly1), bilerp_xy(a.y, b.y, d.y, e.y, lx0, lx1, ly0, ly1),
+                       bilerp_zw(a.z, b.z, d.z, e.z, lx0, lx1, ly0, ly1), bilerp_zw(a.w, b.w, d.w, e.w, lx0, lx1, ly0, ly1));
+}
 
 RF_DEV float wave_sum(float v) {
 #pragma unroll
diff --git a/renderformer_amd/csrc/conv.hip b/renderformer_amd/csrc/conv.hip
--- a/renderformer_amd/csrc/conv.hip
+++ b/renderformer_amd/csrc/conv.hip
@@ -85,11 +85,10 @@
     const int img = row / ho, oy = row - img * ho;
     const int ox = i / c8n;
     const int cc = (i - ox * c8n) * 8;
-    const float fy = sh * (float)oy, fx = sw * (float)ox;
-    const int y0 = (int)fy, x0 = (int)fx;
-    const int y1 = y0 + (y0 < hi - 1 ? 1 : 0), x1 = x0 + (x0 < wi - 1 ? 1 : 0);
-    const float ly1 = fy - (float)y0, lx1 = fx - (float)x0;
-    const float ly0 = 1.0f - ly1, lx0 = 1.0f - lx1;
+    int y0, y1, x0, x1;
+    float ly0, ly1, lx0, lx1;
+    resize_axis(sh, oy, hi, y0, y1, ly0, ly1);
+    resize_axis(sw, ox, wi, x0, x1, lx0, lx1);
     const float* base = in + (int64_t)img * hi * wi * c + cc;
     const float4* pa = reinterpret_cast<const float4*>(base + (int64_t)(y0 * wi + x0) * c);
     const float4* pb = reinterpret_cast<const float4*>(base + (int64_t)(y0 * wi + x1) * c);
@@ -104,12 +103,7 @@
         e[h] = pe[h];
     }
 #pragma unroll
-    for (int h = 0; h < 2; ++h) {
-        r[h].x = ly0 * (lx0 * a[h].x + lx1 * b[h].x) + ly1 * (lx0 * d[h].x + lx1 * e[h].x);
-        r[h].y = ly0 * (lx0 * a[h].y + lx1 * b[h].y) + ly1 * (lx0 * d[h].y + lx1 * e[h].y);
-        r[h].z = ly0 * (lx0 * a[h].z + lx1 * b[h].z) + ly1 * (lx0 * d[h].z + lx1 * e[h].z);
-        r[h].w = ly0 * (lx0 * a[h].w + lx1 * b[h].w) + ly1 * (lx0 * d[h].w + lx1 * e[h].w);
-    }
+    for (int h = 0; h < 2; ++h) r[h] = bilerp4(a[h], b[h], d[h], e[h], lx0, lx1, ly0, ly1);
     const int64_t pix = (int64_t)row * wo + ox;
     if (out) {
         float4* o = reinterpret_cast<float4*>(out + pix * c + cc);
diff --git a/renderformer_amd/csrc/gemm.hip b/renderformer_amd/csrc/gemm.hip
--- a/renderformer_amd/csrc/gemm.hip
+++ b/renderformer_amd/csrc/gemm.hip
@@ -47,6 +47,8 @@
     const float* bias;
     const float* res1;
     const float* res2;
+    int r2h, r2w;
+    float r2sh, r2sw;
     bf16_t* p_hi;
     bf16_t* p_lo;
     int p_ld;
@@ -436,7 +438,7 @@
     }
 }
 
-template <class C, int EPI, int TW2D = 0, bool FINAL = true>
+template <class C, int EPI, int TW2D = 0, bool FINAL = true, bool UP = false>
 RF_DEV void engine_epilogue(const EngineArgs& p, int m0, int n0, const f32x4 (&acc)[C::TI][C::TJ],
                             char* area = nullptr) {
     constexpr int TI = C::TI, TJ = C::TJ;
@@ -538,15 +540,16 @@
             }
             return;
         }
-        const int kk = p.deconv;
+        const int kk = UP ? 0 : p.deconv;
         const int nreal = kk ? p.cout * kk * kk : p.cout;
-        const bool border = (p.flags & RF_CONV_BORDER_BIAS) && !kk;
+        const bool border = !UP && (p.flags & RF_CONV_BORDER_BIAS) && !kk;
         float* __restrict__ outp = reinterpret_cast<float*>(p.c);
         const float* __restrict__ res1 = p.res1;
         const float* __restrict__ res2 = p.res2;
         const float* __restrict__ bias = p.bias;
         struct PixOp {
-            float4 r1[TJ], r2[TJ], b[TJ];
+            float4 r1[TJ], r2[UP ? 4 * TJ : TJ], b[TJ];
+            float ly0, ly1, lx0, lx1;
             int64_t pix[TJ];
             int co[TJ];
         };
@@ -560,11 +563,22 @@
         auto fetch = [&](int i, PixOp& o) {
             const int m = frow(i);
             int img = 0, y = 0, x = 0;
-            if (kk || border) {
+            if (kk || border || UP) {
                 x = m % p.wo;
                 const int t = m / p.wo;
                 y = t % p.ho;
                 img = t / p.ho;
+            }
+            int64_t s00 = 0, s01 = 0, s10 = 0, s11 = 0;
+            if constexpr (UP) {
+                int sy0, sy1, sx0, sx1;
+                resize_axis(p.r2sh, y, p.r2h, sy0, sy1, o.ly0, o.ly1);
+                resize_axis(p.r2sw, x, p.r2w, sx0, sx1, o.lx0, o.lx1);
+                const int64_t ib = (int64_t)img * p.r2h * p.r2w;
+                s00 = (ib + sy0 * p.r2w + sx0) * p.cout;
+                s01 = (ib + sy0 * p.r2w + sx1) * p.cout;
+                s10 = (ib + sy1 * p.r2w + sx0) * p.cout;
+                s11 = (ib + sy1 * p.r2w + sx1) * p.cout;
             }
             const float* brow = bias;
             if (border && brow)
@@ -583,10 +597,16 @@
                 o.co[j] = co;
                 o.r1[j] = float4{0.f, 0.f, 0.f, 0.f};
                 o.r2[j] = float4{0.f, 0.f, 0.f, 0.f};
+                if constexpr (UP) o.r2[TJ + j] = o.r2[2 * TJ + j] = o.r2[3 * TJ + j] = float4{0.f, 0.f, 0.f, 0.f};
                 o.b[j] = bconst[j];
                 if (m < p.m && col < nreal) {
                     if (res1) o.r1[j] = *reinterpret_cast<const float4*>(res1 + pix * p.cout + co);
-                    if (res2) o.r2[j] = *reinterpret_cast<const float4*>(res2 + pix * p.cout + co);
+                    if constexpr (UP) {
+                        o.r2[j] = *reinterpret_cast<const float4*>(res2 + s00 + co);
+                        o.r2[TJ + j] = *reinterpret_cast<const float4*>(res2 + s01 + co);
+                        o.r2[2 * TJ + j] = *reinterpret_cast<const float4*>(res2 + s10 + co);
+                        o.r2[3 * TJ + j] = *reinterpret_cast<const float4*>(res2 + s11 + co);
+                    } else if (res2) o.r2[j] = *reinterpret_cast<const float4*>(res2 + pix * p.cout + co);
                     if (brow && (border || kk)) o.b[j] = *reinterpret_cast<const float4*>(brow + co);
                 }
             }
@@ -611,7 +631,15 @@
                 const int co = o.co[j];
                 const float bb[4] = {o.b[j].x, o.b[j].y, o.b[j].z, o.b[j].w};
                 const float rr1[4] = {o.r1[j].x, o.r1[j].y, o.r1[j].z, o.r1[j].w};
-                const float rr2[4] = {o.r2[j].x, o.r2[j].y, o.r2[j].z, o.r2[j].w};
+                float rr2[4] = {o.r2[j].x, o.r2[j].y, o.r2[j].z, o.r2[j].w};
+                if constexpr (UP) {
+                    const float4 q = bilerp4(o.r2[j], o.r2[TJ + j], o.r2[2 * TJ + j], o.r2[3 * TJ + j], o.lx0, o.lx1,
+                                             o.ly0, o.ly1);
+                    rr2[0] = q.x;
+                    rr2[1] = q.y;
+                    rr2[2] = q.z;
+                    rr2[3] = q.w;
+                }
                 float v[4] = {acc[i][j][0], acc[i][j][1], acc[i][j][2], acc[i][j][3]};
 #pragma unroll
                 for (int e = 0; e < 4; ++e) {
@@ -662,6 +690,7 @@
         float ssr[TI];
 #pragma unroll
         for (int i = 0; i < TI; ++i) ssr[i] = 0.f;
+        float tmax = 0.f;
         const char* const gl = area + C::BM * PN_SLOTS * 4 + PN_RED<C, EPI>;
         const float* const pl = reinterpret_cast<const float*>(gl + C::BN * 4);
         float frq[EPI == E_ROPE ? TJ : 1][2];
@@ -733,6 +762,13 @@
                     }
                 } else {
                     *reinterpret_cast<float4*>(reinterpret_cast<float*>(p.c) + o) = make_float4(v[0], v[1], v[2], v[3]);
+                    if constexpr (EPI == E_ADD) {
+                        if (p.p_hi) {
+                            tmax = amax3(amax3(tmax, v[0], v[1]), v[2], v[3]);
+                            *reinterpret_cast<uint2*>(p.p_hi + (int64_t)row * p.p_ld + col) =
+                                make_uint2(pack_f16x2(v[0], v[1]), pack_f16x2(v[2], v[3]));
+                        }
+                    }
                     if (pre) {
                         const f32x4 g = lds_ld_f4(area + (col - n0) * 4);
                         const float y0 = v[0] * g[0], y1 = v[1] * g[1], y2 = v[2] * g[2], y3 = v[3] * g[3];
@@ -747,6 +783,8 @@
         }
         if constexpr (EPI == E_BF16)
             if (p.range && !f16_in_range(amax)) report_f16_range(p.range, RF_RANGE_GEMM);
+        if constexpr (EPI == E_ADD)
+            if (p.p_hi && p.range && !f16_in_range(tmax)) report_f16_range(p.range, RF_RANGE_CONV);
         if constexpr (EPI == E_ADD || EPI == E_BF16 || EPI == E_ROPE) {
             if (pre && p.xg_f16 && p.range && !f16_in_range(amax)) report_f16_range(p.range, RF_RANGE_RMSNORM);
             if (pre || segq) {
@@ -1776,7 +1814,7 @@
     }
 }
 
-template <class C, int EPI, int NTERM, bool GATHER, bool SK>
+template <class C, int EPI, int NTERM, bool GATHER, bool SK, bool UP = false>
 __global__ __launch_bounds__(C::THREADS, 2) void engine_kernel(EngineArgs p) {
     constexpr int BM = C::BM, BN = C::BN, TI = C::TI, TJ = C::TJ;
     constexpr int MAIN = C::STAGES * stage_bytes<C, NTERM>();
@@ -1796,7 +1834,7 @@
         const int m0 = tm * BM, n0 = tn * BN;
         pn_issue<C, EPI>(p, area, m0, n0);
         engine_mainloop<C, NTERM, GATHER, EPI == E_ADD>(p, smem, m0, n0, 0, p.k / (BK * C::KH), acc);
-        engine_epilogue<C, EPI>(p, m0, n0, acc, area);
+        engine_epilogue<C, EPI, 0, true, UP>(p, m0, n0, acc, area);
     } else {
         const int iters = p.k / (BK * C::KH);
         const int64_t ntiles64 = (int64_t)tiles_m * (p.n / BN);
@@ -1862,7 +1900,7 @@
                             }
                     }
                 }
-                engine_epilogue<C, EPI>(p, m0, n0, acc, area);
+                engine_epilogue<C, EPI, 0, true, UP>(p, m0, n0, acc, area);
             }
             it += kl - kf;
         }
@@ -2248,7 +2286,7 @@
                          TJ = h3::TJ;
 };
 
-template <int DBG = 0>
+template <int DBG = 0, bool UP = false>
 __global__ __launch_bounds__(512, 1) void halo3_kernel(EngineArgs p) {
     using namespace h2;
     __shared__ __attribute__((aligned(16))) char smem[h3::LDS];
@@ -2374,7 +2412,7 @@
         for (int i = 0; i < TI; ++i) asm volatile("" ::"v"(acc[i][0]), "v"(acc[i][1]));
         return;
     }
-    engine_epilogue<H3Tile, E_CONV, TW, false>(p, (img * p.ho + y0) * p.wo + x0, n0, acc);
+    engine_epilogue<H3Tile, E_CONV, TW, false, UP>(p, (img * p.ho + y0) * p.wo + x0, n0, acc);
 }
 
 namespace c32 {
@@ -2693,12 +2731,12 @@
     return gm;
 }
 
-template <class C, int EPI, int NTERM, bool GATHER = false>
+template <class C, int EPI, int NTERM, bool GATHER = false, bool UP = false>
 int launch(EngineArgs a, void* stream, const char* what) {
     const int tiles_m = (a.m + C::BM - 1) / C::BM, tiles_n = a.n / C::BN;
     const int nwg = tiles_n * tiles_m;
     a.group_m = pick_group_m(tiles_m, tiles_n, C::BM, C::BN, (nwg + 7) / 8, GATHER ? 0 : (int64_t)a.m * a.k * 2);
-    RF_LAUNCH((engine_kernel<C, EPI, NTERM, GATHER, false>), dim3(nwg), dim3(C::THREADS), 0, (hipStream_t)stream,
+    RF_LAUNCH((engine_kernel<C, EPI, NTERM, GATHER, false, UP>), dim3(nwg), dim3(C::THREADS), 0, (hipStream_t)stream,
                        a);
     return rf::check_launch(what);
 }
@@ -2737,11 +2775,11 @@
 constexpr int64_t SK_PART_FLOATS = (int64_t)256 * 256 * 256;
 constexpr int64_t SK_WS_BYTES = SK_PART_FLOATS * 4 + SK_MAX_GRID * 4;
 
-template <class C, int EPI, int NTERM = 1, bool GATHER = false>
+template <class C, int EPI, int NTERM = 1, bool GATHER = false, bool UP = false>
 int launch_sk(EngineArgs a, int grid, void* stream, const char* what) {
     const int tiles_m = (a.m + C::BM - 1) / C::BM, tiles_n = a.n / C::BN;
     a.group_m = pick_group_m(tiles_m, tiles_n, C::BM, C::BN, ((int64_t)tiles_m * tiles_n + 7) / 8);
-    RF_LAUNCH((engine_kernel<C, EPI, NTERM, GATHER, true>), dim3(grid), dim3(C::THREADS), 0,
+    RF_LAUNCH((engine_kernel<C, EPI, NTERM, GATHER, true, UP>), dim3(grid), dim3(C::THREADS), 0,
                        (hipStream_t)stream, a);
     return rf::check_launch(what);
 }
@@ -3403,7 +3441,7 @@
     p.bias = bias;
     p.gate = gate;
     p.out_f16 = out_f16;
-    p.range = (out_f16 || (p.xg && p.xg_f16)) ? rf::range_word() : nullptr;
+    p.range = (out_f16 || (p.xg && p.xg_f16) || p.p_hi) ? rf::range_word() : nullptr;
     const char* what = f16 ? "rf_gemm_f16" : "rf_gemm_bf16";
     const bool ws_ok = workspace && ws_bytes >= SK_WS_BYTES;
 #ifdef RF_STUDY
@@ -3472,6 +3510,34 @@
     nio.xg_f16 = f16;
     return gemm_bf16(a, lda, w, ldw, x, ldx, nullptr, m, n, k, RF_EPI_ADD_F32, workspace, ws_bytes, stream, nullptr,
                      f16, &nio);
+}
+
+extern "C" int rf_gemm_add_tap(const void* a, int64_t lda, const void* w, int64_t ldw, float* x, int64_t ldx, int m,
+                               int n, int k, const float* norm_w, void* xg, int64_t ldxg, float* ss, void* plane,
+                               int p_ld, int operand_dtype, void* workspace, int64_t ws_bytes, void* stream) {
+    RF_REQUIRE(x && plane, "rf_gemm_add_tap: null pointer");
+    RF_REQUIRE(operand_dtype == RF_DT_F16 || operand_dtype == RF_DT_BF16, "rf_gemm_add_tap: operand_dtype");
+    RF_REQUIRE(p_ld >= n && p_ld % 4 == 0 && ((uintptr_t)plane & 7) == 0, "rf_gemm_add_tap: plane rows (p_ld >= N, 8-B)");
+    const bool f16 = operand_dtype == RF_DT_F16;
+    EngineArgs nio{};
+    nio.p_hi = (bf16_t*)plane;
+    nio.p_ld = p_ld;
+    if (norm_w) {
+        RF_REQUIRE(xg && ss, "rf_gemm_add_tap: norm_w needs xg and ss");
+        RF_REQUIRE(ldxg >= n && ldxg % 4 == 0 && ((uintptr_t)xg & 7) == 0, "rf_gemm_add_tap: xg rows (ldxg >= N, 8-B)");
+        RF_REQUIRE(((uintptr_t)ss & 15) == 0 && ((uintptr_t)norm_w & 15) == 0, "rf_gemm_add_tap: ss / norm_w 16-B aligned");
+        if (n <= PN_SLOTS * 128) {
+            nio.xg = (bf16_t*)xg;
+            nio.ldxg = ldxg;
+            nio.norm_g = norm_w;
+            nio.ss_out = ss;
+            nio.xg_f16 = f16;
+        }
+    }
+    const int rc = gemm_bf16(a, lda, w, ldw, x, ldx, nullptr, m, n, k, RF_EPI_ADD_F32, workspace, ws_bytes, stream,
+                             nullptr, f16, &nio);
+    if (rc != RF_OK || !norm_w || nio.xg) return rc;
+    return rf_prenorm(x, ldx, norm_w, xg, ldxg, ss, m, n, operand_dtype, stream);
 }
 
 extern "C" int rf_gemm_rownorm(const void* a, int64_t lda, const void* w, int64_t ldw, void* c, int64_t ldc, int m,
@@ -3661,6 +3727,10 @@
 
 static int launch_halo3(EngineArgs a, void* stream, const char* what) {
     const int nwg = (a.m / 512) * (a.n / 128);
+    if (a.r2h) {
+        RF_LAUNCH((halo3_kernel<0, true>), dim3(nwg), dim3(512), 0, (hipStream_t)stream, a);
+        return rf::check_launch(what);
+    }
     const int dbg = rf::env_int("RF_H3_DBG", 0);
 #ifndef RF_STUDY
     if (dbg) return rf::study_only("rf_conv: RF_H3_DBG (halo3 ablation builds, garbage results)");
@@ -3772,6 +3842,19 @@
     return big ? launch<T256x128, E_CONV, NT, false>(p, stream, what) : launch<T128, E_CONV, NT, false>(p, stream, what);
 }
 
+static int conv_f16_up(EngineArgs& p, int64_t sk_grid_n, int tile, void* workspace, void* stream, const char* what) {
+    if (!sk_grid_n && halo3_ok(p)) return launch_halo3(p, stream, what);
+    if (sk_grid_n) {
+        if (const int rc = sk_setup(p, workspace, stream)) return rc;
+        return launch_sk<T128w8, E_CONV, P_F16, true, true>(p, (int)sk_grid_n, stream, what);
+    }
+    const int t = tile ? tile : conv_tile_env();
+    if (p.n % 128 || t == CT_64 || t == CT_64SK) return launch<T64c, E_CONV, P_F16, true, true>(p, stream, what);
+    const int64_t tiles = (int64_t)((p.m + 127) / 128) * (p.n / 128);
+    if (t == CT_128 || (t != CT_128w8 && tiles > 512)) return launch<T128, E_CONV, P_F16, true, true>(p, stream, what);
+    return launch<T128w8, E_CONV, P_F16, true, true>(p, stream, what);
+}
+
 static int conv_common(EngineArgs& p, int nterm, bool gather, const void* w_hi, const void* w_lo, int cout, int cout_pad, float* out,
                        const float* bias, const float* res1, const float* res2, void* p_hi, void* p_lo, int p_ld,
                        int flags, const float* w_fin, const float* b_fin, int n_fin, float elu_alpha, void* workspace,
@@ -3787,6 +3870,10 @@
                     p.pad == 1 && p.ho == p.hi && p.wo == p.wi && p.deconv == 0 && p.ho >= 2 && p.wo >= 2),
                "%s: RF_CONV_BORDER_BIAS needs a 3x3 stride-1 pad-1 convolution of an image of at least 2 x 2 pixels "
                "with its 9-row bias", what);
+    const bool up = p.r2h > 0;
+    RF_REQUIRE(!up || (nterm == P_F16 && gather && res2 && !(flags & (RF_CONV_FINAL | RF_CONV_BORDER_BIAS)) &&
+                       !p.deconv && cout_pad % 64 == 0),
+               "%s: the resized res2 needs a non-final fp16 convolution with res2 and a plain bias", what);
     static void* z = nullptr;
     if (!z && hipGetSymbolAddress(&z, HIP_SYMBOL(g_zero_row)) != hipSuccess) {
         z = nullptr;
@@ -3824,6 +3911,7 @@
         const int64_t grid = std::min<int64_t>(512, tiles * (p.k / BK) / 12);
         if (grid > tiles) {
             if (const int rc = sk_setup(p, workspace, stream)) return rc;
+            if (up) return launch_sk<T64c, E_CONV, P_F16, true, true>(p, (int)grid, stream, what);
             return gather ? launch_sk<T64c, E_CONV, P_F16, true>(p, (int)grid, stream, what)
                           : launch_sk<T64c, E_CONV, P_F16, false>(p, (int)grid, stream, what);
         }
@@ -3835,6 +3923,7 @@
         const int64_t grid = std::min<int64_t>(256, work / 8);
         if (tiles < 192 && grid > tiles) skg = grid;
     }
+    if (up) return conv_f16_up(p, skg, ct == CT_64 ? CT_64 : CT_AUTO, workspace, stream, what);
     return nterm == P_F16 ? conv_dispatch<P_F16>(p, gather, big, skg, workspace, stream, what, ct == CT_64 ? CT_64 : CT_AUTO)
                           : conv_dispatch<3>(p, gather, big, skg, workspace, stream, what);
 }
@@ -3869,11 +3958,10 @@
                        b_fin, n_fin, elu_alpha, workspace, ws_bytes, stream, "rf_conv2d_bf16x3");
 }
 
-extern "C" int rf_conv2d_f16(const void* in, int n_img, int hi, int wi, int cin_pad, const void* w, int cout,
-                             int cout_pad, int kh, int kw, int stride, int pad, const float* bias, const float* res1,
-                             const float* res2, float* out, void* p_out, int p_ld, int flags, const float* w_fin,
-                             const float* b_fin, int n_fin, float elu_alpha, void* workspace, int64_t ws_bytes,
-                             void* stream) {
+static int conv2d_f16(const void* in, int n_img, int hi, int wi, int cin_pad, const void* w, int cout, int cout_pad,
+                      int kh, int kw, int stride, int pad, const float* bias, const float* res1, const float* res2,
+                      int res2_hi, int res2_wi, float* out, void* p_out, int p_ld, int flags, const float* w_fin,
+                      const float* b_fin, int n_fin, float elu_alpha, void* workspace, int64_t ws_bytes, void* stream) {
     RF_REQUIRE(in, "rf_conv2d_f16: null input");
     RF_REQUIRE(cin_pad % BK == 0, "rf_conv2d_f16: cin_pad %d must be a multiple of %d", cin_pad, BK);
     RF_REQUIRE((cout_pad % 128 == 0 || cout_pad == 64) && cout_pad >= cout,
@@ -3894,8 +3982,34 @@
     p.k = kh * kw * cin_pad;
     RF_REQUIRE(p.k < 65536, "conv: kh*kw*cin_pad = %d must be < 65536", p.k);
     p.ldw = p.k;
+    if (res2_hi > 0) {
+        p.r2h = res2_hi;
+        p.r2w = res2_wi;
+        p.r2sh = p.ho > 1 ? (float)(res2_hi - 1) / (float)(p.ho - 1) : 0.f;
+        p.r2sw = p.wo > 1 ? (float)(res2_wi - 1) / (float)(p.wo - 1) : 0.f;
+    }
     return conv_common(p, P_F16, true, w, nullptr, cout, cout_pad, out, bias, res1, res2, p_out, nullptr, p_ld, flags,
                        w_fin, b_fin, n_fin, elu_alpha, workspace, ws_bytes, stream, "rf_conv2d_f16");
+}
+
+extern "C" int rf_conv2d_f16(const void* in, int n_img, int hi, int wi, int cin_pad, const void* w, int cout,
+                             int cout_pad, int kh, int kw, int stride, int pad, const float* bias, const float* res1,
+                             const float* res2, float* out, void* p_out, int p_ld, int flags, const float* w_fin,
+                             const float* b_fin, int n_fin, float elu_alpha, void* workspace, int64_t ws_bytes,
+                             void* stream) {
+    return conv2d_f16(in, n_img, hi, wi, cin_pad, w, cout, cout_pad, kh, kw, stride, pad, bias, res1, res2, 0, 0, out,
+                      p_out, p_ld, flags, w_fin, b_fin, n_fin, elu_alpha, workspace, ws_bytes, stream);
+}
+
+extern "C" int rf_conv2d_f16_up(const void* in, int n_img, int hi, int wi, int cin_pad, const void* w, int cout,
+                                int cout_pad, int kh, int kw, int stride, int pad, const float* bias, const float* res1,
+                                const float* res2, int res2_hi, int res2_wi, float* out, void* p_out, int p_ld,
+                                int flags, void* workspace, int64_t ws_bytes, void* stream) {
+    RF_REQUIRE(res2 && res2_hi >= 1 && res2_wi >= 1 && (int64_t)res2_hi * res2_wi < (1 << 30),
+               "rf_conv2d_f16_up: res2 source of res2_hi x res2_wi pixels");
+    RF_REQUIRE(((uintptr_t)res2 & 15) == 0, "rf_conv2d_f16_up: res2 must be 16-B aligned");
+    return conv2d_f16(in, n_img, hi, wi, cin_pad, w, cout, cout_pad, kh, kw, stride, pad, bias, res1, res2, res2_hi,
+                      res2_wi, out, p_out, p_ld, flags, nullptr, nullptr, 0, 0.f, workspace, ws_bytes, stream);
 }
 
 static const char* group_member(EngineArgs& p, const rf_conv_desc& d, const void* zero) {
diff --git a/renderformer_amd/csrc/stage.cpp b/renderformer_amd/csrc/stage.cpp
--- a/renderformer_amd/csrc/stage.cpp
+++ b/renderformer_amd/csrc/stage.cpp
@@ -318,15 +318,18 @@
                                         stream));
         }
         RF_CALL(rf_gemm_rownorm(h, D, L.w13, D, g, F, T2, 2 * F, D, epi_swiglu, ss, D, d->eps, nullptr, 0, 0, dt, gws, gwb, stream));
-        if (i + 1 < NL)
-            RF_CALL(rf_gemm_add_prenorm(g, F, L.w2, F, x, ldx, T2, D, F, d->layers[i + 1].query_norm, h, D, ss, dt, gws,
-                                        gwb, stream));
+        const rf_decoder_tap* t = tap < d->n_taps && d->taps[tap].layer == i ? &d->taps[tap++] : nullptr;
+        const float* next_norm = i + 1 < NL ? d->layers[i + 1].query_norm : nullptr;
+        if (t && d->tap_fused && !t->p_lo && t->p_ld % 4 == 0 && ((uintptr_t)t->p_hi & 7) == 0) {
+            RF_CALL(rf_gemm_add_tap(g, F, L.w2, F, x, ldx, T2, D, F, next_norm, h, D, ss, t->p_hi, t->p_ld, dt, gws, gwb,
+                                    stream));
+            continue;
+        }
+        if (next_norm)
+            RF_CALL(rf_gemm_add_prenorm(g, F, L.w2, F, x, ldx, T2, D, F, next_norm, h, D, ss, dt, gws, gwb, stream));
         else
             RF_CALL(gemm(g, F, L.w2, F, x, ldx, nullptr, T2, D, F, RF_EPI_ADD_F32, gws, gwb, stream));
-        if (tap < d->n_taps && d->taps[tap].layer == i) {
-            const rf_decoder_tap& t = d->taps[tap++];
-            RF_CALL(rf_split_planes(x, T2, D, ldx, t.p_hi, t.p_lo, t.p_ld, 0, stream));
-        }
+        if (t) RF_CALL(rf_split_planes(x, T2, D, ldx, t->p_hi, t->p_lo, t->p_ld, 0, stream));
     }
     return RF_OK;
 }
diff --git a/renderformer_amd/dpt.py b/renderformer_amd/dpt.py
--- a/renderformer_amd/dpt.py
+++ b/renderformer_amd/dpt.py
@@ -170,7 +170,7 @@
 
     def __call__(self, x: Planes, stride=1, pad=None, res1=None, res2=None, out_f32=False,
                  planes_ld: Optional[int] = None, planes_silu=False, final=None, final_flags=0,
-                 border_bias: Optional[torch.Tensor] = None):
+                 border_bias: Optional[torch.Tensor] = None, res2_up: Optional[torch.Tensor] = None):
         n, h, w, ld = x.shape
         if ld != self.cin_pad or x.c != self.cin:
             raise ValueError(f"conv input planes must have {self.cin} channels padded to {self.cin_pad}, got "
@@ -205,6 +205,12 @@
         for r in (res1, res2):
             if r is not None and (tuple(r.shape) != (n, ho, wo, self.cout) or not r.is_contiguous()):
                 raise ValueError("residual must match the conv output")
+        if res2_up is not None:
+            if not (self.f16 and not self.k) or res2 is not None:
+                raise ValueError("res2_up needs an fp16 convolution and no res2")
+            if (res2_up.dim() != 4 or res2_up.shape[0] != n or res2_up.shape[3] != self.cout or
+                    not res2_up.is_contiguous() or res2_up.dtype != torch.float32):
+                raise ValueError("res2_up must be contiguous fp32 [n, h, w, cout]")
         flags = PLANE_SILU if planes_silu else 0
         bias = self.b
         if border_bias is not None:
@@ -214,6 +220,10 @@
         if self.f16 and self.k:
             call("rf_deconv2d_f16", ptr(x.hi), n, h, w, ld, ptr(self.w_hi), self.cout, self.k, ptr(self.b), ptr(out),
                  ptr(pl.hi if pl else None), planes_ld or 0, ptr(ws), ws.numel(), stream())
+        elif self.f16 and res2_up is not None:
+            call("rf_conv2d_f16_up", ptr(x.hi), n, h, w, ld, ptr(self.w_hi), self.cout, self.cout_pad, self.kh,
+                 self.kw, stride, pad, ptr(bias), ptr(res1), ptr(res2_up), res2_up.shape[1], res2_up.shape[2],
+                 ptr(out), ptr(pl.hi if pl else None), planes_ld or 0, flags, ptr(ws), ws.numel(), stream())
         elif self.f16:
             call("rf_conv2d_f16", ptr(x.hi), n, h, w, ld, ptr(self.w_hi), self.cout, self.cout_pad, self.kh, self.kw,
                  stride, pad, ptr(bias), ptr(res1), ptr(res2), ptr(out), ptr(pl.hi if pl else None), planes_ld or 0,
@@ -231,6 +241,15 @@
 
 
 PRECISIONS = ("f16", "bf16x3")
+
+
+@dataclass
+class _Resize:
+    src: torch.Tensor
+    size: tuple
+
+    def materialise(self) -> torch.Tensor:
+        return upsample(self.src, *self.size)[0]
 
 
 class DPTHead:
@@ -265,6 +284,9 @@
         self.group_proj = (f16 and os.environ.get("RF_DPT_GROUP", "1") != "0" and len(self.projects) <= 4 and
                            all(c.kh == 1 and c.kw == 1 and not c.k and c.cout_pad % 128 == 0 for c in self.projects))
         self.fold = f16 and os.environ.get("RF_DPT_FOLD", "1") != "0"
+        self.res2_levels = set()
+        if f16 and os.environ.get("RF_DPT_RES2_FUSE", "1") != "0":
+            self.res2_levels = {int(c) for c in os.environ.get("RF_DPT_RES2_LEVELS", "123") if c in "123"}
         if self.fold:
             w, b = fold_affine_1x1(g("scratch.output_conv1.weight"), g("scratch.output_conv1.bias"),
                                    g("scratch.refinenet1.out_conv.weight"), g("scratch.refinenet1.out_conv.bias"))
@@ -273,10 +295,15 @@
 
     def _rcu(self, convs, x32, xs: Planes, extra=None, want_f32=False, next_silu=True, next_ld=None):
         _, t = convs[0](xs, planes_ld=convs[1].cin_pad, planes_silu=True)
+        if isinstance(extra, _Resize):
+            return convs[1](t, res1=x32, res2_up=extra.src, out_f32=want_f32, planes_ld=next_ld,
+                            planes_silu=next_silu)
         return convs[1](t, res1=x32, res2=extra, out_f32=want_f32, planes_ld=next_ld, planes_silu=next_silu)
 
     def _fuse(self, r, x0, x1, x1s, size, last=False):
         units, out_conv = self.refine[r]
+        if isinstance(x0, _Resize) and (x1 is None or r not in self.res2_levels):
+            x0 = x0.materialise()
         if x1 is None:
             out, outs = x0, split_planes(x0, self.feat_ld, silu=True, f16=self.f16)
         else:
@@ -287,7 +314,7 @@
         y32, _ = out_conv(y, out_f32=True)
         if last:
             return upsample(y32, *size, out_f32=False, planes_ld=self.out1.cin_pad, f16=self.f16)[1]
-        return upsample(y32, *size)[0]
+        return _Resize(y32, tuple(size))
 
     def tap_planes(self, i: int, t: torch.Tensor, n_img: int, hp: int, wp: int) -> Planes:
         return split_planes(t.view(n_img, hp, wp, t.shape[-1]), self.projects[i].cin_pad, f16=self.f16)
@@ -319,7 +346,7 @@
         units4, oc4 = self.refine[4]
         _, y = self._rcu(units4[2], rn[3], rns[3], next_silu=False, next_ld=oc4.cin_pad)
         y32, _ = oc4(y, out_f32=True)
-        p4 = upsample(y32, *size(rn[2]))[0]
+        p4 = _Resize(y32, size(rn[2]))
         p3 = self._fuse(3, p4, rn[2], rns[2], size(rn[1]))
         p2 = self._fuse(2, p3, rn[1], rns[1], size(rn[0]))
         p1 = self._fuse(1, p2, rn[0], rns[0], (2 * rn[0].shape[1], 2 * rn[0].shape[2]), last=True)
diff --git a/renderformer_amd/model.py b/renderformer_amd/model.py
--- a/renderformer_amd/model.py
+++ b/renderformer_amd/model.py
@@ -663,10 +663,15 @@
                     ops.attention(qs, ks, vs, att, plan.prob_self, R, H, max_k_len=R, q_prescaled=True)
                 add_proj(att, L.ws_out, getattr(L, "ws_out8", None), L.ffn_norm, name="self_out")
             norm_proj(L.ffn_norm, L.w13, getattr(L, "w13_8", None), g, ops.EPI_SWIGLU, tag="gemm_w13_stage2", name="w13")
-            add_proj(g, L.w2, getattr(L, "w2_8", None), W.dec[i + 1].query_norm if i + 1 < n_dec else None,
-                     tag="gemm_w2_stage2", name="w2")
-            if i in outl:
-                taps.append(W.dpt.tap_planes(len(taps), x, P, plan.hp, plan.wp))
+            next_norm = W.dec[i + 1].query_norm if i + 1 < n_dec else None
+            if i in outl and defer and W.dpt.f16 and ops.tap_fused():
+                pl = W.dpt.empty_tap_planes(len(taps), P, plan.hp, plan.wp, D, dev)
+                ops.gemm_add_tap(g, L.w2, x, pl.hi.view(T2, -1), next_norm, h, ss, tag="gemm_w2_stage2")
+                taps.append(pl)
+            else:
+                add_proj(g, L.w2, getattr(L, "w2_8", None), next_norm, tag="gemm_w2_stage2", name="w2")
+                if i in outl:
+                    taps.append(W.dpt.tap_planes(len(taps), x, P, plan.hp, plan.wp))
             cap = self._capture
             if cap is not None and cap["dec"] is not None:
                 rows = torch.cat([v * R + cap["dec"] for v in cap["views"]])
diff --git a/renderformer_amd/ops.py b/renderformer_amd/ops.py
--- a/renderformer_amd/ops.py
+++ b/renderformer_amd/ops.py
@@ -233,6 +233,37 @@
     _t0(tag)
     call("rf_gemm_add_prenorm", ptr(a), a.stride(0), ptr(w), w.stride(0), ptr(x), x.stride(0), m, n, k, ptr(norm_w),
          ptr(xg), xg.stride(0), ptr(ss), _dt(a), ptr(ws), ws.numel(), stream())
+    return x
+
+
+def tap_fused() -> bool:
+    return os.environ.get("RF_DPT_TAP_FUSE", "1") != "0"
+
+
+def gemm_add_tap(a: torch.Tensor, w: torch.Tensor, x: torch.Tensor, plane: torch.Tensor,
+                 norm_w: Optional[torch.Tensor] = None, xg: Optional[torch.Tensor] = None,
+                 ss: Optional[torch.Tensor] = None, tag: Optional[str] = None) -> torch.Tensor:
+    _check(a.dtype in HALF and w.dtype == a.dtype, f"gemm_add_tap: a / w must share bf16 or fp16 ({a.dtype}, {w.dtype})")
+    for t, n in ((a, "a"), (w, "w")):
+        _dev(t, t.dtype, n)
+    _dev(x, torch.float32, "x")
+    _dev(plane, torch.float16, "plane")
+    m, k = a.shape
+    n, k2 = w.shape
+    _check(k == k2 and x.shape == (m, n), "gemm_add_tap: shape mismatch")
+    _check(plane.dim() == 2 and plane.shape[0] == m and plane.shape[1] >= n and plane.stride(1) == 1,
+           "gemm_add_tap: plane must be [M, >= N] rows")
+    if norm_w is not None:
+        _check(xg is not None and ss is not None and xg.dtype == a.dtype and xg.shape == (m, n) and
+               norm_w.numel() == n, "gemm_add_tap: norm_w needs xg [M, N] of a's dtype and ss")
+        _dev(xg, xg.dtype, "xg")
+        _dev(ss, torch.float32, "ss")
+        _check(ss.shape[0] >= m and ss.shape[1] == PRENORM_SLOTS and ss.is_contiguous(), "gemm_add_tap: ss shape")
+    ws = _gemm_workspace(a.device)
+    _t0(tag)
+    call("rf_gemm_add_tap", ptr(a), a.stride(0), ptr(w), w.stride(0), ptr(x), x.stride(0), m, n, k, ptr(norm_w),
+         ptr(xg) if norm_w is not None else 0, xg.stride(0) if norm_w is not None else 0,
+         ptr(ss) if norm_w is not None else 0, ptr(plane), plane.stride(0), _dt(a), ptr(ws), ws.numel(), stream())
     return x
 
 
@@ -607,6 +638,7 @@
     d.workspace = ptr(ws)
     d.timer_cross = int(_timer_takes(tag, n_layers))
     d.qk_fused = int(bool(cross.get("qk_fused")))
+    d.tap_fused = int(tap_fused())
     call("rf_decoder_forward", ptr(x), x.stride(0), ctypes.addressof(d), stream())
     return x
 
```

Result: no change. 93.66, median of 4 (+0.3%).
